# cosdata/cosdata

Hardware: AMD Instinct MI355X
Metric: QPS at recall@10≥0.95, 1024-dim dense cosine, 1/2/4/8 MI355X (higher is better)
Workload: dtype u8

## Files before the change

cosdata_amd/_lib.py:

```python
from __future__ import annotations

import ctypes as C
import os
import subprocess

_PKG = os.path.dirname(os.path.abspath(__file__))
SO_PATH = os.path.join(_PKG, "libcosdata_hip.so")
CSRC = os.path.join(_PKG, "csrc")

OK, ERR_STORAGE_MISMATCH, ERR_CALCULATION, ERR_INVALID, ERR_UNIMPLEMENTED, ERR_HIP, ERR_NOT_READY, ERR_NO_DEVICE = range(8)
STATUS_NAMES = {
    0: "OK", 1: "StorageMismatch", 2: "CalculationError", 3: "Invalid", 4: "Unimplemented", 5: "HipError",
    6: "NotReady", 7: "NoDevice",
}
ABI_VERSION = 1


class CosdataError(RuntimeError):

    def __init__(self, status: int, message: str):
        super().__init__(f"[{STATUS_NAMES.get(status, status)}] {message}")
        self.status = status


class CosParams(C.Structure):
    _fields_ = [
        ("struct_size", C.c_uint32), ("abi_version", C.c_uint32), ("dim", C.c_uint32), ("metric", C.c_uint32),
        ("storage", C.c_uint32), ("resolution", C.c_uint32), ("range_lo", C.c_float), ("range_hi", C.c_float),
        ("num_layers", C.c_uint32), ("neighbors_count", C.c_uint32), ("level0_neighbors_count", C.c_uint32),
        ("ef_construction", C.c_uint32), ("ef_search", C.c_uint32), ("shortlist_size", C.c_uint32),
        ("visited_mode", C.c_uint32), ("device", C.c_int32), ("id_base", C.c_uint32), ("reserved", C.c_uint32),
        ("seed", C.c_uint64),
    ]


class CosSearchStats(C.Structure):
    _fields_ = [
        ("evals", C.c_uint64), ("expansions", C.c_uint64), ("adj_bytes", C.c_uint64), ("rerank_rows", C.c_uint64),
        ("walk_ms", C.c_float), ("finalize_ms", C.c_float), ("prep_ms", C.c_float), ("reserved", C.c_uint32),
    ]


class CosWalkSplit(C.Structure):
    _fields_ = [
        ("struct_size", C.c_uint32), ("queries", C.c_uint32), ("table_level_min", C.c_uint32), ("table_cols", C.c_uint32),
        ("cut_after_level", C.c_uint32), ("reserved", C.c_uint32),
        ("table_ms", C.c_float), ("upper_ms", C.c_float), ("sort_ms", C.c_float), ("lower_ms", C.c_float),
        ("table_int8_ops", C.c_double), ("table_evals", C.c_uint64),
        ("upper_evals", C.c_uint64), ("upper_expansions", C.c_uint64), ("upper_adj_bytes", C.c_uint64),
        ("lower_evals", C.c_uint64), ("lower_expansions", C.c_uint64), ("lower_adj_bytes", C.c_uint64),
    ]


class CosTimingSummary(C.Structure):
    _fields_ = [("launches", C.c_uint32), ("prep_ms_sum", C.c_float), ("walk_ms_sum", C.c_float), ("finalize_ms_sum", C.c_float),
                ("walk_ms_min", C.c_float), ("walk_ms_max", C.c_float)]


class CosCoalescingStats(C.Structure):
    _fields_ = [("launches", C.c_uint64), ("queries", C.c_uint64), ("requests", C.c_uint64), ("closed_full", C.c_uint64),
                ("closed_quiet", C.c_uint64), ("closed_deadline", C.c_uint64), ("solo_calls", C.c_uint64)]


class CosSparseStats(C.Structure):
    _fields_ = [("kernel_ms", C.c_float), ("blocks", C.c_uint32), ("postings_visited", C.c_uint64), ("posting_bytes", C.c_uint64)]


class CosFlatStats(C.Structure):
    _fields_ = [("gemm_ms", C.c_float), ("gemm_launches", C.c_uint32), ("int8_ops", C.c_double), ("code_bytes", C.c_double)]


class CosBM25Stats(C.Structure):
    _fields_ = [("struct_size", C.c_uint32), ("documents_count", C.c_uint32), ("n_terms", C.c_uint32), ("largest_doc_id", C.c_uint32),
                ("dir_rows", C.c_uint32), ("dir_tiles", C.c_uint32), ("reserved", C.c_uint32),
                ("postings", C.c_uint64), ("tombstones", C.c_uint64), ("device_bytes", C.c_uint64)]


class CosSparseIndexStats(C.Structure):
    _fields_ = [("struct_size", C.c_uint32), ("n_vectors", C.c_uint32), ("n_dims", C.c_uint32), ("dir_rows", C.c_uint32),
                ("dir_tiles", C.c_uint32), ("packed", C.c_uint32), ("have_raw", C.c_uint32), ("reserved", C.c_uint32),
                ("postings", C.c_uint64), ("removed", C.c_uint64), ("raw_pairs", C.c_uint64), ("device_bytes", C.c_uint64)]


def build(force: bool = False, verbose: bool = False) -> str:
    srcs = [os.path.join(CSRC, f) for f in os.listdir(CSRC) if f.endswith((".hip", ".h"))]
    srcs.append(os.path.join(_PKG, "..", "include", "cosdata_hip.h"))
    stale = force or not os.path.exists(SO_PATH) or any(os.path.getmtime(s) > os.path.getmtime(SO_PATH) for s in srcs)
    if force:
        subprocess.check_call(["make", "-C", CSRC, "-s", "clean"])
    if stale:
        cmd = ["make", "-C", CSRC, "-j", str(max(2, min(16, 2 * (os.cpu_count() or 1))))]
        if not verbose:
            cmd.append("-s")
        subprocess.check_call(cmd)
    return SO_PATH


_lib = None

ABI_SYMBOLS = [
    "cos_index_create", "cos_index_destroy", "cos_last_error_string", "cos_device_count",
    "cos_index_upload_vectors", "cos_index_set_root", "cos_index_upload_graph_level", "cos_index_level_count",
    "cos_index_download_graph_level", "cos_index_download_codes", "cos_index_download_root", "cos_index_build", "cos_index_append", "cos_index_delete", "cos_index_restore_link_state", "cos_index_release_link_state", "cos_index_enable_metadata", "cos_index_upload_meta_nodes", "cos_index_upload_meta_graph_level", "cos_index_build_meta", "cos_index_meta_level_count", "cos_index_download_meta_graph_level", "cos_search_filtered_batch",
    "cos_ann_search_filtered_batch", "cos_index_load_reference_dir", "cos_reference_dir_level_counts", "cos_reference_dir_read_level",
    "cos_search_batch", "cos_search_batch_device", "cos_ann_search_batch", "cos_index_set_coalescing", "cos_index_coalescing_stats", "cos_index_set_ef_search",
    "cos_index_set_visited_mode", "cos_index_set_latency_mode", "cos_index_set_latency_waves", "cos_index_set_walk_order", "cos_index_walk_order_cuts", "cos_index_set_walk_table", "cos_index_walk_table_info", "cos_index_last_walk_split", "cos_index_enable_timing", "cos_index_last_stats", "cos_index_timing_summary", "cos_quantize_batch",
    "cos_code_bytes", "cos_sample_values_range", "cos_distance_batch", "cos_bruteforce_topk", "cos_flat_search_batch", "cos_bm25_create", "cos_bm25_destroy",
    "cos_bm25_insert", "cos_bm25_delete", "cos_bm25_stats", "cos_bm25_download",
    "cos_bm25_search_batch", "cos_bm25_search_batch_device", "cos_rrf_fuse_batch", "cos_hybrid_search_batch", "cos_text_process", "cos_text_count_tokens", "cos_bm25_term_frequency", "cos_xxhash32", "cos_stem_english", "cos_sparse_create", "cos_sparse_build_csr", "cos_sparse_create_from_vectors", "cos_sparse_destroy", "cos_sparse_search_batch", "cos_sparse_last_stats", "cos_sparse_layout",
    "cos_sparse_set_max_candidates", "cos_sparse_max_candidates",
    "cos_sparse_insert", "cos_sparse_delete", "cos_sparse_stats", "cos_sparse_download", "cos_merge_topk_device", "cos_merge_topk_packed_device", "cos_hbm_probe",
    "cos_shardset_unique_id", "cos_shardset_create", "cos_shardset_destroy", "cos_shardset_search_batch", "cos_shardset_exchange_device",
    "cos_tuning_set", "cos_tuning_clear", "cos_tuning_get",
]


def lib():
    global _lib
    if _lib is not None:
        return _lib
    if not os.path.exists(SO_PATH):
        raise CosdataError(ERR_NO_DEVICE, f"{SO_PATH} is missing: build it with `python -c 'import __graft_entry__ as g; g.build()'` "
                                          "(the HIP extension is mandatory; there is no CPU path)")
    try:
        import torch
    except ImportError:
        pass
    L = C.CDLL(SO_PATH)
    vp, i32, u32, f32 = C.c_void_p, C.c_int32, C.c_uint32, C.c_float
    sig = {
        "cos_index_create": [C.POINTER(CosParams), C.POINTER(vp)],
        "cos_index_destroy": [vp],
        "cos_device_count": [C.POINTER(i32)],
        "cos_index_upload_vectors": [vp, vp, u32, u32],
        "cos_index_set_root": [vp, vp],
        "cos_index_upload_graph_level": [vp, u32, u32, vp, vp],
        "cos_index_level_count": [vp, u32, C.POINTER(u32)],
        "cos_index_download_graph_level": [vp, u32, vp, vp],
        "cos_index_download_codes": [vp, vp, vp],
        "cos_index_download_root": [vp, vp],
        "cos_index_build": [vp, u32],
        "cos_index_append": [vp, vp, u32, u32, u32],
        "cos_index_release_link_state": [vp],
        "cos_index_restore_link_state": [vp],
        "cos_index_delete": [vp, vp, u32],
        "cos_index_load_reference_dir": [vp, C.c_char_p, u32, u32],
        "cos_index_enable_metadata": [vp, u32, u32],
        "cos_index_upload_meta_nodes": [vp, u32, vp, vp],
        "cos_index_upload_meta_graph_level": [vp, u32, u32, vp, vp],
        "cos_search_filtered_batch": [vp, vp, u32, vp, vp, u32, vp, vp, vp, vp],
        "cos_ann_search_filtered_batch": [vp, vp, u32, vp, vp, vp, vp, vp, vp],
        "cos_reference_dir_level_counts": [C.c_char_p, u32, u32, u32, vp],
        "cos_reference_dir_read_level": [C.c_char_p, u32, u32, u32, u32, vp, vp],
        "cos_search_batch": [vp, vp, u32, u32, vp, vp, vp, vp],
        "cos_search_batch_device": [vp, vp, u32, u32, vp, vp, vp, vp, vp],
        "cos_ann_search_batch": [vp, vp, u32, vp, vp, vp, vp],
        "cos_index_set_ef_search": [vp, u32],
        "cos_index_set_coalescing": [vp, u32, u32],
        "cos_index_coalescing_stats": [vp, C.POINTER(CosCoalescingStats)],
        "cos_index_set_visited_mode": [vp, u32],
        "cos_index_build_meta": [vp, u32, vp, vp, vp, u32],
        "cos_index_meta_level_count": [vp, u32, C.POINTER(u32)],
        "cos_index_download_meta_graph_level": [vp, u32, vp, vp],
        "cos_index_set_latency_mode": [vp, u32],
        "cos_index_set_latency_waves": [vp, u32],
        "cos_index_set_walk_order": [vp, u32],
        "cos_index_walk_order_cuts": [vp, C.POINTER(u32), u32, C.POINTER(u32)],
        "cos_index_enable_timing": [vp, i32],
        "cos_index_last_stats": [vp, vp, C.POINTER(CosSearchStats)],
        "cos_index_set_walk_table": [vp, u32, u32],
        "cos_index_walk_table_info": [vp, C.POINTER(u32), C.POINTER(u32)],
        "cos_index_last_walk_split": [vp, vp, C.POINTER(CosWalkSplit)],
        "cos_index_timing_summary": [vp, vp, C.POINTER(CosTimingSummary)],
        "cos_quantize_batch": [u32, u32, u32, f32, f32, vp, u32, vp, vp],
        "cos_sample_values_range": [vp, u32, u32, f32, C.POINTER(f32), C.POINTER(f32)],
        "cos_distance_batch": [u32, u32, u32, u32, vp, vp, u32, vp, vp, u32, vp, vp, u32, vp, vp],
        "cos_bruteforce_topk": [vp, vp, u32, u32, vp, vp],
        "cos_flat_search_batch": [vp, vp, u32, u32, vp, vp, vp, C.POINTER(CosFlatStats)],
        "cos_bm25_create": [i32, vp, vp, u32, vp, vp, u32, C.POINTER(vp)],
        "cos_bm25_destroy": [vp],
        "cos_bm25_insert": [vp, vp, vp, u32, vp, vp],
        "cos_bm25_delete": [vp, vp, vp, u32, vp],
        "cos_bm25_stats": [vp, C.POINTER(CosBM25Stats)],
        "cos_bm25_download": [vp, C.POINTER(u32), C.POINTER(C.c_uint64), vp, vp, vp, vp, vp],
        "cos_bm25_search_batch": [vp, vp, vp, u32, u32, vp, vp, vp],
        "cos_bm25_search_batch_device": [vp, vp, vp, u32, u32, vp, vp, vp, vp],
        "cos_rrf_fuse_batch": [vp, vp, u32, vp, vp, u32, u32, f32, u32, vp, vp, vp],
        "cos_hybrid_search_batch": [vp, vp, vp, vp, vp, u32, u32, f32, vp, vp, vp],
        "cos_sparse_create": [i32, u32, f32, vp, u32, vp, vp, u32, vp, vp, vp, C.POINTER(vp)],
        "cos_sparse_build_csr": [u32, f32, u32, vp, vp, vp, vp, vp, vp, C.POINTER(u32)],
        "cos_sparse_create_from_vectors": [i32, u32, f32, u32, vp, vp, vp, i32, C.POINTER(vp)],
        "cos_sparse_destroy": [vp],
        "cos_sparse_search_batch": [vp, vp, vp, vp, u32, u32, f32, u32, vp, vp, vp],
        "cos_sparse_last_stats": [vp, vp],
        "cos_sparse_layout": [vp, C.POINTER(u32)],
        "cos_sparse_set_max_candidates": [vp, u32],
        "cos_sparse_max_candidates": [vp, C.POINTER(u32)],
        "cos_sparse_insert": [vp, u32, vp, vp, vp, C.POINTER(u32)],
        "cos_sparse_delete": [vp, vp, vp, u32, vp, vp, C.POINTER(C.c_uint64)],
        "cos_sparse_stats": [vp, C.POINTER(CosSparseIndexStats)],
        "cos_sparse_download": [vp, C.POINTER(u32), C.POINTER(C.c_uint64), vp, vp, vp],
        "cos_merge_topk_device": [vp, vp, vp, u32, u32, u32, vp, vp, vp, i32, vp],
        "cos_merge_topk_packed_device": [vp, u32, u32, u32, vp, vp, vp, i32, vp],
        "cos_hbm_probe": [i32, u32, C.c_uint64, u32, u32, C.POINTER(C.c_double)],
        "cos_shardset_unique_id": [vp],
        "cos_shardset_create": [vp, u32, u32, u32, vp, C.POINTER(vp)],
        "cos_shardset_destroy": [vp],
        "cos_shardset_search_batch": [vp, vp, u32, u32, vp, vp, vp],
        "cos_shardset_exchange_device": [vp, vp, u32, u32, vp, vp, vp, vp, vp],
        "cos_tuning_set": [C.c_char_p, C.c_int64],
        "cos_tuning_clear": [C.c_char_p],
        "cos_tuning_get": [C.c_char_p, C.POINTER(C.c_int64), C.POINTER(i32)],
    }
    for name, args in sig.items():
        fn = getattr(L, name)
        fn.restype = i32
        fn.argtypes = args
    L.cos_last_error_string.restype = C.c_char_p
    L.cos_last_error_string.argtypes = []
    L.cos_stem_english.restype = C.c_size_t
    L.cos_stem_english.argtypes = [vp, C.c_char_p, C.c_size_t, C.c_char_p, C.c_size_t]
    L.cos_text_process.restype = i32
    L.cos_text_process.argtypes = [C.c_char_p, C.c_size_t, u32, f32, f32, f32, vp, vp, vp, vp, u32, C.POINTER(u32)]
    L.cos_text_count_tokens.restype = u32
    L.cos_text_count_tokens.argtypes = [C.c_char_p, C.c_size_t, u32]
    L.cos_bm25_term_frequency.restype = f32
    L.cos_bm25_term_frequency.argtypes = [u32, u32, f32, f32, f32]
    L.cos_xxhash32.restype = u32
    L.cos_xxhash32.argtypes = [C.c_char_p, C.c_size_t, u32]
    L.cos_code_bytes.restype = C.c_size_t
    L.cos_code_bytes.argtypes = [u32, u32, u32]
    _lib = L
    return L


def check(rc: int):
    if rc != OK:
        raise CosdataError(rc, lib().cos_last_error_string().decode("utf-8", "replace"))


def tuning_set(name: str, value: int):
    check(lib().cos_tuning_set(name.encode(), int(value)))


def tuning_clear(name: str | None = None):
    check(lib().cos_tuning_clear(name.encode() if name is not None else None))


def tuning_get(name: str):
    v, isset = C.c_int64(), C.c_int32()
    check(lib().cos_tuning_get(name.encode(), C.byref(v), C.byref(isset)))
    return int(v.value) if isset.value else None


# ... 25 lines not shown
```

cosdata_amd/csrc/engine.hip:

```cpp
#include <hip/hip_runtime.h>

#include <algorithm>
#include <cstdarg>
#include <cstdio>
#include <cstdlib>
#include <chrono>
#include <cmath>
#include <condition_variable>
#include <cstring>
#include <map>
#include <mutex>
#include <string>
#include <thread>
#include <vector>

#include "engine_internal.h"

using namespace cosdev;

static thread_local std::string g_err;
int32_t cos_fail(int32_t code, const char *fmt, ...) {
    char buf[512];
    va_list ap;
    va_start(ap, fmt);
    vsnprintf(buf, sizeof(buf), fmt, ap);
    va_end(ap);
    g_err = buf;
    return code;
}

extern "C" const char *cos_last_error_string(void) { return g_err.c_str(); }

extern "C" int32_t cos_device_count(int32_t *out) {
    if (!out) return cos_fail(COS_ERR_INVALID, "null argument");
    int n = 0;
    hipError_t e = hipGetDeviceCount(&n);
    if (e != hipSuccess) { *out = 0; return cos_fail(COS_ERR_NO_DEVICE, "hipGetDeviceCount: %s", hipGetErrorString(e)); }
    *out = n;
    return COS_OK;
}

static u32 pow2ceil(u32 v) { u32 p = 1; while (p < v) p <<= 1; return p; }

int32_t cos_set_device(const cos_index *ix) {
    HIP_TRY(hipSetDevice(ix->p.device));
    return COS_OK;
}

static bool graph_ready(const cos_index *ix) {
    if (!ix->have_vectors || !ix->have_root) return false;
    for (auto &l : ix->lv) if (l.n == 0) return false;
    return true;
}

IndexDev cos_make_index_dev(const cos_index *ix) {
    IndexDev d;
    memset(&d, 0, sizeof(d));
    d.codes = ix->d_codes;
    d.mags = ix->d_mags;
    d.raw = ix->d_raw;
    d.raw_mags = ix->d_raw_mags;
    d.row_stride = ix->row_stride;
    d.raw_stride = ix->p.dim;
    d.n = ix->n;
    d.dim = ix->p.dim;
    d.metric = ix->p.metric;
    d.storage = ix->p.storage;
    d.num_layers = ix->p.num_layers;
    d.shortlist = ix->p.shortlist_size;
    d.visited_mode = ix->p.visited_mode;
    d.nchunks = ix->nchunks;
    d.G = ix->G;
    d.id_base = ix->p.id_base;
    d.id_stride = ix->id_stride;
    d.mbits = ix->meta.d_mbits;
    d.mmags = ix->meta.d_mmags;
    d.mdim = ix->meta.mdim;
    for (u32 l = 0; l <= ix->p.num_layers; l++) {
        const LevelHost &h = ix->lv[l];
        d.lv[l].adj_vec = h.d_adj_vec;
        d.lv[l].adj_node = l == 0 ? h.d_adj_vec : h.d_adj_node;
        d.lv[l].node_vec = l == 0 ? nullptr : h.d_node_vec;
        d.lv[l].child = l == 0 ? nullptr : h.d_child;
        d.lv[l].n = h.n;
        d.lv[l].M = h.M;
        d.lv[l].root_idx = h.n ? h.n - 1 : 0;
        d.lv[l].adj_mag = (ix->adj_mag_valid && cosdev::tune_or(cosdev::TUNE_WALK_ADJ_MAG, 1) != 0) ? h.d_adj_mag : nullptr;
        d.lv[l].mag_stride = std::min(h.M, ix->p.shortlist_size);
    }
    return d;
}

extern "C" int32_t cos_index_create(const cos_params *p, cos_index **out) {
    if (!p || !out) return cos_fail(COS_ERR_INVALID, "null argument");
    *out = nullptr;
    if (p->struct_size != sizeof(cos_params) || p->abi_version != COS_ABI_VERSION)
        return cos_fail(COS_ERR_INVALID, "cos_params size/version mismatch (%u/%u, expected %zu/%u)", p->struct_size, p->abi_version,
                    sizeof(cos_params), COS_ABI_VERSION);
    if (p->dim == 0) return cos_fail(COS_ERR_INVALID, "dim == 0");
// ... 485 lines not shown
    const u64 log_cap = (u64)ef * M + 2;
    u32 max_nodes = 0;
    for (const LevelHost &l : ix->lv) max_nodes = std::max(max_nodes, l.n);
    const u32 words = (max_nodes + 31) / 32 + 1;
    if (log_cap > 0xFFFFFFFFull) return cos_fail(COS_ERR_INVALID, "ef too large");
    const size_t need_bits = (size_t)B * words, need_log = (size_t)B * log_cap;
    if (need_bits > vt.bits.cap || need_log > vt.log.cap) {
        HIP_TRY(hipStreamSynchronize(st));
        if (need_bits > vt.bits.cap) vt.zeroed = false;
        HIP_TRY(vt.bits.grow(need_bits));
        HIP_TRY(vt.log.grow(need_log));
    }
    if (!vt.zeroed) {
        HIP_TRY(hipMemsetAsync(vt.bits, 0, vt.bits.cap * 4, st));
        vt.zeroed = true;
    }
    wa.vis_bits = vt.bits;
    wa.vis_log = vt.log;
    wa.vis_words_per_query = words;
    wa.vis_log_cap = (u32)log_cap;
    return COS_OK;
}

static int32_t ensure_order_rank(cos_index *ix) {
    if (ix->order_rank_valid) return COS_OK;
    for (u32 l = 0; l < cosdev::MAX_LEVELS; l++) {
        ix->d_order_rank[l].reset();
        ix->order_rank_n[l] = 0;
    }
    ix->order_levels.clear();
    const u32 Ltop = ix->p.num_layers;
    auto usable = [&](u32 l) { return l >= 1 && l <= Ltop && ix->lv[l].n > 1 && ix->lv[l].n <= (1u << 20) && ix->lv[l].d_adj_node; };
    std::vector<u32> want;
    if (const long long mask = cosdev::tune(cosdev::TUNE_WALK_SPLIT_LEVELS); mask != cosdev::TUNE_UNSET) {
        for (u32 l = Ltop; l >= 1; l--)
            if ((mask >> l) & 1) want.push_back(l);
    } else {
        for (u32 l = 1; l <= Ltop; l++)
            if (usable(l) && (size_t)ix->lv[l].n * ix->row_stride <= ((size_t)64 << 20)) { want.push_back(l); break; }
    }
    u32 prev = Ltop + 1;
    for (u32 l : want) {
        if (!usable(l) || l >= prev) continue;
        ix->order_levels.push_back(l);
        prev = l;
    }
    if (!ix->order_levels.empty()) HIP_TRY(hipDeviceSynchronize());
    for (u32 kl : ix->order_levels) {
        const LevelHost &H = ix->lv[kl];
        const u32 n = H.n, M = H.M;
        std::vector<u32> adj((size_t)n * M), rank(n, 0u), stack;
        HIP_TRY(hipMemcpy(adj.data(), H.d_adj_node, adj.size() * 4, hipMemcpyDeviceToHost));
        std::vector<uint8_t> seen(n, 0);
        u32 next = 0;
        auto dfs_from = [&](u32 start) {
            stack.push_back(start);
            while (!stack.empty()) {
                const u32 v = stack.back();
                stack.pop_back();
                if (seen[v]) continue;
                seen[v] = 1;
                rank[v] = next++;
                const u32 *row = &adj[(size_t)v * M];
                for (u32 j = M; j-- > 0;) {
                    const u32 u = row[j];
                    if (u != cosdev::ROW_EMPTY && u < n && !seen[u]) stack.push_back(u);
                }
            }
        };
        dfs_from(n - 1);
        for (u32 v = 0; v < n; v++) if (!seen[v]) dfs_from(v);
        HIP_TRY(ix->d_order_rank[kl].alloc(n));
        HIP_TRY(hipMemcpy(ix->d_order_rank[kl], rank.data(), (size_t)n * 4, hipMemcpyHostToDevice));
        ix->order_rank_n[kl] = n;
    }
    ix->order_rank_valid = true;
    return COS_OK;
}

static void clear_current_table(cos_index *ix) {
    ix->d_tcodes = nullptr;
    ix->d_tmags = nullptr;
    ix->d_tcsums = nullptr;
    ix->table_cols = 0;
    ix->table_level_min = 0;
    ix->table_stride = 0;
}
static u32 walk_table_max_cols(const cos_index *ix) {
    const long long env = cosdev::tune_or(cosdev::TUNE_WALK_TABLE_COLS, -1);
    return env >= 0 ? (u32)std::min<long long>(env, 1ll << 20) : ix->walk_table_max_cols;
}
static u32 walk_table_min_B(const cos_index *ix) {
    const long long env = cosdev::tune_or(cosdev::TUNE_WALK_TABLE_MIN_B, -1);
    return env >= 0 ? (u32)std::min<long long>(env, 0xFFFFFFFFll) : ix->walk_table_min_B;
}
cosdev::WalkPlanIn cos_walk_plan_in(const cos_index *ix, u32 B, u32 ef) {
    cosdev::WalkPlanIn in{};
    in.eng = ix->eng;
    in.storage = ix->p.storage;
    in.nchunks = ix->nchunks;
    in.G = ix->G;
    in.num_layers = ix->p.num_layers;
    for (u32 l = 0; l <= ix->p.num_layers; l++) in.M[l] = ix->lv[l].M;
    in.shortlist = ix->p.shortlist_size;
    in.visited_mode = ix->p.visited_mode;
    in.mdim = ix->meta.mdim;
    in.B = B;
    in.ef = ef;
    in.chain = true;
    const long long lat = cosdev::tune_or(cosdev::TUNE_WALK_LAT, -1), lat4 = cosdev::tune_or(cosdev::TUNE_WALK_LAT4, -1);
    in.lat_max_B = lat >= 0 ? (u32)std::min(lat, 0xFFFFFFFFll) : ix->lat_max_B;
    in.lat4_max_B = lat4 >= 0 ? (u32)std::min(lat4, 0xFFFFFFFFll) : ix->lat4_max_B;
    in.small_table_tk = cosdev::tune_or(cosdev::TUNE_WALK_SMALL_TABLE_TK, 1) != 0;
    in.adj_mag_mode = (u32)cosdev::tune_or(cosdev::TUNE_WALK_ADJ_MAG, 1);
    in.table_min_B = walk_table_min_B(ix);
    in.order_min_B = ix->walk_order_min_B;
    in.chain_min_B = ix->chain_min_B;
    in.side_min_B = ix->walk_side_min_B;
    in.table_after_sort = cosdev::tune_or(cosdev::TUNE_WALK_TABLE_AFTER_SORT, 1);
    in.table_supported = cosdev::level_table_eng_supported(ix->eng, ix->row_stride);
    in.adj_mag_valid = ix->adj_mag_valid;
    return in;
}
static int32_t ensure_level_table(cos_index *ix) {
    const u32 max_cols = walk_table_max_cols(ix);
    const bool automatic = max_cols == COS_WALK_TABLE_AUTO;
    const u32 efs = ix->p.ef_search, Mup = ix->p.neighbors_count;
    const u64 c_rule = (u64)cosdev::tune_or(cosdev::TUNE_WALK_TABLE_RULE_C, 2u * efs <= 3u * Mup ? 10 : (efs <= 2u * Mup ? 8 : 6));
    const u64 per_level = automatic ? std::min<u64>(c_rule * ix->p.ef_search * ix->p.neighbors_count, 1u << 20) : (u64)(1u << 20);
    const u64 total_cap = automatic ? (u64)(1u << 20) : (u64)max_cols;
    const u64 key = automatic ? (0x8000000000000000ull | per_level) : (u64)max_cols;
    if (ix->level_table_valid && ix->table_built_for_key == key) return COS_OK;
    if (!ix->level_table_valid) {
        HIP_TRY(hipDeviceSynchronize());
        ix->table_sets.clear();
    }
    ix->level_table_valid = true;
    ix->table_built_for_key = key;
    clear_current_table(ix);
    for (const auto &t : ix->table_sets)
        if (t.key == key) {
            ix->table_level_min = t.level_min;
            ix->table_cols = t.cols;
            ix->table_stride = t.stride;
            memcpy(ix->table_col0, t.col0, sizeof(t.col0));
            ix->d_tcodes = t.tcodes;
            ix->d_tmags = t.tmags;
            ix->d_tcsums = t.tcsums;
            return COS_OK;
        }
    if (!cosdev::level_table_eng_supported(ix->eng, ix->row_stride) || max_cols == 0) return COS_OK;
    const u32 Ltop = ix->p.num_layers;
    u32 cols = 0, lmin = 0;
    for (u32 l = Ltop; l >= 1; l--) {
        if (!ix->lv[l].d_node_vec || ix->lv[l].n == 0 || ix->lv[l].n > per_level || (u64)cols + ix->lv[l].n > total_cap) break;
        cols += ix->lv[l].n;
        lmin = l;
    }
    if (lmin == 0) return COS_OK;
    HIP_TRY(hipDeviceSynchronize());
    cos_index::TableSet t;
    auto build = [&]() -> hipError_t {
        hipError_t e = t.tcodes.alloc((size_t)cols * ix->row_stride);
        if (e == hipSuccess) e = t.tmags.alloc(cols);
        if (e == hipSuccess) e = t.tcsums.alloc(cols);
        u32 c0 = 0;
        for (u32 l = Ltop; l >= lmin && e == hipSuccess; l--) {
            ix->table_col0[l] = c0;
            e = cosdev::launch_level_table_gather(ix->d_codes, ix->d_mags, ix->row_stride, ix->lv[l].d_node_vec, ix->lv[l].n, c0, t.tcodes, t.tmags, nullptr);
            c0 += ix->lv[l].n;
        }
        if (e == hipSuccess) e = cosdev::launch_code_sums(t.tcodes, ix->row_stride, cols, t.tcsums, nullptr);
        if (e == hipSuccess) e = hipDeviceSynchronize();
        return e;
    };
    if (const hipError_t e = build(); e != hipSuccess) {
        (void)hipDeviceSynchronize();
        if (e == hipErrorOutOfMemory) {
            (void)hipGetLastError();
            return COS_OK;
        }
        ix->level_table_valid = false;
        HIP_TRY(e);
    }
    ix->d_tcodes = t.tcodes;
    ix->d_tmags = t.tmags;
    ix->d_tcsums = t.tcsums;
    ix->table_cols = cols;
    ix->table_level_min = lmin;
    ix->table_stride = ((u64)cols + 31) / 32 * 32;
    t.key = key;
    t.level_min = lmin;
    t.cols = cols;
    t.stride = ix->table_stride;
    memcpy(t.col0, ix->table_col0, sizeof(t.col0));
    ix->table_sets.push_back(std::move(t));
    return COS_OK;
}

extern "C" int32_t cos_index_set_walk_table(cos_index *ix, uint32_t max_cols, uint32_t min_queries) {
    if (!ix) return cos_fail(COS_ERR_INVALID, "null argument");
    if (max_cols > (1u << 20) && max_cols != COS_WALK_TABLE_AUTO) return cos_fail(COS_ERR_INVALID, "max_cols must be <= 2^20 (or COS_WALK_TABLE_AUTO)");
    std::lock_guard<std::mutex> g(ix->mu);
    ix->walk_table_max_cols = max_cols;
    ix->walk_table_min_B = min_queries;
    return COS_OK;
}

extern "C" int32_t cos_index_walk_table_info(cos_index *ix, uint32_t *out_level_min, uint32_t *out_cols) {
    if (!ix || !out_level_min || !out_cols) return cos_fail(COS_ERR_INVALID, "null argument");
    *out_level_min = *out_cols = 0;
    if (!graph_ready(ix)) return cos_fail(COS_ERR_NOT_READY, "index needs vectors, root and every graph level");
    int32_t rc = cos_set_device(ix);
    if (rc) return rc;
    std::lock_guard<std::mutex> g(ix->mu);
    if (walk_table_min_B(ix) == 0) return COS_OK;
    if ((rc = ensure_level_table(ix))) return rc;
    *out_level_min = ix->table_level_min;
    *out_cols = ix->table_cols;
    return COS_OK;
}

static int32_t ensure_adj_mags(cos_index *ix) {
    if (ix->adj_mag_valid) return COS_OK;
    if (!graph_ready(ix) || ix->meta.mdim != 0u) return COS_OK;
    if (cosdev::walk_rows_over_64_slots(cos_walk_plan_in(ix, 0, 0))) return COS_OK;
    HIP_TRY(hipDeviceSynchronize());
    for (u32 l = 0; l <= ix->p.num_layers; l++) {
        ix->lv[l].d_adj_mag.reset();
    }
    for (u32 l = 0; l <= ix->p.num_layers; l++) {
        LevelHost &H = ix->lv[l];
        const u32 slots = std::min(H.M, ix->p.shortlist_size);
        const hipError_t e = H.d_adj_mag.alloc((size_t)H.n * slots);
        if (e == hipErrorOutOfMemory) {
            (void)hipGetLastError();
            for (u32 k = 0; k < l; k++) ix->lv[k].d_adj_mag.reset();
            return COS_OK;
        }
        HIP_TRY(e);
        HIP_TRY(cosdev::launch_fill_adj_mag(H.d_adj_vec, ix->d_mags, H.d_adj_mag, H.n, H.M, slots, ix->own_stream));
    }
    HIP_TRY(hipStreamSynchronize(ix->own_stream));
    ix->adj_mag_valid = true;
    return COS_OK;
}

int32_t cos_prepare_walk_plans(cos_index *ix) {
    std::lock_guard<std::mutex> g(ix->mu);
    if (int32_t rc = ensure_adj_mags(ix)) return rc;
    if (ix->walk_order_min_B)
        if (int32_t rc = ensure_order_rank(ix)) return rc;
    if (walk_table_min_B(ix))
        if (int32_t rc = ensure_level_table(ix)) return rc;
    return COS_OK;
}

extern "C" int32_t cos_index_walk_order_cuts(cos_index *ix, uint32_t *out_levels, uint32_t cap, uint32_t *out_n) {
    if (!ix || !out_n || (cap && !out_levels)) return cos_fail(COS_ERR_INVALID, "null argument");
    *out_n = 0;
    if (!graph_ready(ix)) return cos_fail(COS_ERR_NOT_READY, "index needs vectors, root and every graph level");
    int32_t rc = cos_set_device(ix);
    if (rc) return rc;
    std::lock_guard<std::mutex> g(ix->mu);
    if ((rc = ensure_order_rank(ix))) return rc;
    for (u32 l : ix->order_levels) {
        if (*out_n < cap) out_levels[*out_n] = l;
        (*out_n)++;
    }
    return COS_OK;
}

struct SearchLaunch {
    cosdev::WalkPlan plan;
    u32 ef = 0, visited_mode = 0;
    bool timed = false;
    u64 tab_stride = 0;
    u32 tab_col0[cosdev::MAX_LEVELS] = {};
    const uint8_t *tcodes = nullptr;
    const float *tmags = nullptr;
    const u32 *tcsums = nullptr;
    u32 n_keys = 0, key_level[cosdev::MAX_LEVELS], key_n[cosdev::MAX_LEVELS];
    const u32 *order_rank[cosdev::MAX_LEVELS];
};

static int32_t get_workspace(cos_index *ix, void *key, hipStream_t st, u32 B, u32 top_k, bool host_api, Workspace **out, SearchLaunch *L,
                             bool chain = true) {
    std::lock_guard<std::mutex> g(ix->mu);
    std::unique_ptr<Workspace> &slot = ix->ws[key];
    if (!slot) slot.reset(new Workspace());
    Workspace *w = slot.get();
    const u32 L1 = ix->p.num_layers + 1;
    if (B > w->capB) {
        u32 cap = std::max(B, 64u);
        HIP_TRY(hipStreamSynchronize(st));
        w->capB = 0;
        w->cap_topk = 0;
        HIP_TRY(w->q_codes.alloc((size_t)cap * ix->row_stride));
        HIP_TRY(w->q_mags.alloc(cap));
        HIP_TRY(w->q_raw_mags.alloc(cap));
        HIP_TRY(w->walk_ids.alloc((size_t)cap * L1 * KEEP_SEARCH));
        HIP_TRY(w->walk_sims.alloc((size_t)cap * L1 * KEEP_SEARCH));
        HIP_TRY(w->walk_counts.alloc((size_t)cap * L1));
        HIP_TRY(w->walk_status.alloc(cap));
        HIP_TRY(w->stats.alloc((size_t)cap * 4));
        HIP_TRY(w->stats2.alloc((size_t)cap * 4));
        HIP_TRY(w->qsums.alloc(cap));
        if (ix->eng == ENG_Q2) HIP_TRY(w->qdig.alloc((size_t)cap * (ix->row_stride / 16) * 64));
        HIP_TRY(w->fin_flags.alloc((size_t)cap + 1));
        HIP_TRY(w->rerank_rows.alloc(cap));
        HIP_TRY(w->d_queries.alloc((size_t)cap * ix->p.dim));
        HIP_TRY(w->d_out_counts.alloc(cap));
        HIP_TRY(w->d_out_status.alloc(cap));
        w->capB = cap;
    }
    L->ef = ix->p.ef_search;
    L->visited_mode = ix->p.visited_mode;
    L->timed = ix->timing;
    cosdev::WalkPlanIn in = cos_walk_plan_in(ix, B, L->ef);
    in.chain = chain;
    const cosdev::WalkPlan want = cosdev::walk_plan(in);
    cosdev::WalkHave have{};
    if (want.refill_adj_mag) {
        if (int32_t rc = ensure_adj_mags(ix)) return rc;
        in.adj_mag_valid = ix->adj_mag_valid;
    }
    if (want.prepare_order) {
        if (w->order.cap < w->capB) {
            HIP_TRY(hipStreamSynchronize(st));
            HIP_TRY(cosdev::walk_order_reserve(w->order, w->capB));
        }
        if (int32_t rc = ensure_order_rank(ix)) return rc;
        have.order_buffers = w->order.cap >= B;
        have.n_order_keys = (u32)ix->order_levels.size();
        have.order_level0 = have.n_order_keys ? ix->order_levels[0] : 0u;
    }
    if (want.prepare_table) {
        if (int32_t rc = ensure_level_table(ix)) return rc;
        const size_t need = (size_t)w->capB * ix->table_stride;
        if (need > w->tab.cap) {
            const size_t budget = (size_t)cosdev::tune_or(cosdev::TUNE_WALK_TABLE_MAX_BYTES, (long long)48 << 30);
            HIP_TRY(hipStreamSynchronize(st));
            ix->table_bytes_total -= w->tab.cap * 4;
            w->tab.reset();
            if (ix->table_bytes_total + need * 4 <= budget) {
                if (const hipError_t e = w->tab.alloc(need); e == hipSuccess)
                    ix->table_bytes_total += need * 4;
                else if (e == hipErrorOutOfMemory)
                    (void)hipGetLastError();
                else
                    HIP_TRY(e);
            }
        }
        have.table_level_min = ix->level_table_valid ? ix->table_level_min : 0u;
        have.table_cols = ix->table_cols;
        have.table_buffer = w->tab && (size_t)B * ix->table_stride <= w->tab.cap;
    }
    L->plan = cosdev::walk_plan(in, &have);
    if (L->plan.use_table) {
        L->tab_stride = ix->table_stride;
        memcpy(L->tab_col0, ix->table_col0, sizeof(L->tab_col0));
        L->tcodes = ix->d_tcodes;
        L->tmags = ix->d_tmags;
        L->tcsums = ix->d_tcsums;
    }
    if (L->plan.ordered)
        for (u32 l : ix->order_levels) {
            L->key_level[L->n_keys] = l;
            L->key_n[L->n_keys] = ix->order_rank_n[l];
            L->order_rank[L->n_keys++] = ix->d_order_rank[l];
        }
    if (host_api && (size_t)top_k * w->capB > (size_t)w->cap_topk * w->capB) {
        w->cap_topk = 0;
        HIP_TRY(w->d_out_ids.alloc((size_t)w->capB * top_k));
        HIP_TRY(w->d_out_scores.alloc((size_t)w->capB * top_k));
        w->cap_topk = top_k;
    }
    if (w->ev.empty()) {
        w->ev.assign((size_t)Workspace::EV_RING * Workspace::EV_PER, nullptr);
        for (auto &e : w->ev) HIP_TRY(hipEventCreate(&e));
    }
    if (!w->walk_done) HIP_TRY(hipEventCreateWithFlags(&w->walk_done, hipEventDisableTiming));
    if (!w->walk_fin) HIP_TRY(hipEventCreateWithFlags(&w->walk_fin, hipEventDisableTiming));
    if (!w->last_range) HIP_TRY(hipEventCreateWithFlags(&w->last_range, hipEventDisableTiming));
    *out = w;
    return COS_OK;
}

static int32_t run_search(cos_index *ix, Workspace *w, const SearchLaunch &L, const float *d_queries, u32 B, u32 top_k, u32 *d_out_ids,
                          float *d_out_scores, u32 *d_out_counts, int32_t *d_out_status, bool do_finalize, hipStream_t st,
                          hipStream_t st_fin = nullptr, hipEvent_t walk_ev = nullptr) {
    const cosdev::WalkPlan &plan = L.plan;
    const bool timed = L.timed, ordered = plan.ordered, chained = plan.chained;
    const u32 ef = L.ef, n_keys = L.n_keys;
    IndexDev dev = cos_make_index_dev(ix);
    dev.visited_mode = L.visited_mode;
    for (u32 l = 0; l <= dev.num_layers; l++)
        if (!((plan.use_adj_mag >> l) & 1u)) dev.lv[l].adj_mag = nullptr;
    WalkArgs wa;
    memset(&wa, 0, sizeof(wa));
    if (dev.visited_mode == COS_VISITED_EXACT) {
        int32_t rc = vis_tab_prepare(w->vis, ix, B, ef, st, wa);
        if (rc) return rc;
    }
    hipEvent_t *ev = &w->ev[(size_t)(w->ev_count % Workspace::EV_RING) * Workspace::EV_PER];
    if (timed) HIP_TRY(hipEventRecord(ev[0], st));
    HIP_TRY(launch_quantize_rows(ix->eng, d_queries, ix->p.dim, B, ix->p.dim, ix->p.range_lo, ix->p.range_hi, w->q_codes, ix->row_stride,
                                 w->q_mags, w->q_raw_mags, st));
    if (plan.use_table) {
        if (plan.table_waits_for_sort) {
            std::lock_guard<std::mutex> g(ix->chain_mu);
            if (ix->chain_last_range_ev && ix->chain_last_range_ev != w->last_range) HIP_TRY(hipStreamWaitEvent(st, ix->chain_last_range_ev, 0));
        }
        if (timed) HIP_TRY(hipEventRecord(ev[4], st));
        HIP_TRY(cosdev::launch_level_table(ix->eng, w->q_codes, w->q_mags, w->qsums, w->qdig, B, L.tcodes, L.tmags, L.tcsums, ix->row_stride, plan.table_cols,
                                           w->tab, L.tab_stride, ix->n_cus, st));
        if (timed) HIP_TRY(hipEventRecord(ev[5], st));
    }
    if (timed) HIP_TRY(hipEventRecord(ev[1], st));
    wa.qcodes = w->q_codes;
    wa.qmags = w->q_mags;
    wa.B = B;
    wa.ef = ef;
    wa.keep = KEEP_SEARCH;
    wa.out_ids = w->walk_ids;
    wa.out_sims = w->walk_sims;
    wa.out_counts = w->walk_counts;
    wa.out_status = w->walk_status;
    wa.out_stats = w->stats;
    wa.out_stats2 = w->stats2;
    HIP_TRY(hipMemsetAsync(w->stats2, 0, (size_t)B * 32, st));
    if (plan.use_table) {
        wa.tab = w->tab;
        wa.tab_mags = L.tmags;
        wa.tab_stride = L.tab_stride;
        wa.tab_level_min = plan.table_level_min;
        memcpy(wa.tab_col0, L.tab_col0, sizeof(L.tab_col0));
    }
    hipStream_t sw = st;
    if (plan.side_stream) {
        if (!w->walk_stream) {
            int lo = 0, hi = 0;
            HIP_TRY(hipDeviceGetStreamPriorityRange(&lo, &hi));
            HIP_TRY(hipStreamCreateWithPriority(&w->walk_stream, hipStreamNonBlocking, lo));
            HIP_TRY(hipEventCreateWithFlags(&w->prep_done, hipEventDisableTiming));
        }
        sw = w->walk_stream;
        HIP_TRY(hipEventRecord(w->prep_done, st));
        HIP_TRY(hipStreamWaitEvent(sw, w->prep_done, 0));
    }
    auto walk = [&](hipStream_t s) -> int32_t {
        if (!ordered) {
            if (chained) HIP_TRY(hipEventRecord(w->last_range, s));
            HIP_TRY(launch_walk(ix->eng, dev, wa, plan.kernel, s));
            return COS_OK;
        }
        wa.phase = 1;
        wa.entry0 = w->order.entry0;
        wa.order_key = w->order.order_key;
        wa.order_iota = w->order.iota;
        u32 first = dev.num_layers;
        for (u32 i = 0; i <= n_keys; i++) {
            const bool last = i == n_keys;
            wa.level_first = first;
            wa.level_last = last ? 0u : L.key_level[i];
            wa.key_n = last ? 0u : L.key_n[i];
            wa.order_rank = last ? nullptr : L.order_rank[i];
            if (last && chained) HIP_TRY(hipEventRecord(w->last_range, s));
            HIP_TRY(launch_walk(ix->eng, dev, wa, plan.kernel, s));
            if (last) break;
            if (timed && i == 0) HIP_TRY(hipEventRecord(ev[6], s));
            HIP_TRY(cosdev::launch_walk_order(w->order, B, L.key_n[i], ix->num_xcd, s));
            if (timed && i == 0) HIP_TRY(hipEventRecord(ev[7], s));
            wa.q_order = w->order.q_order;
            first = L.key_level[i] - 1;
        }
        return COS_OK;
    };
    if (chained) {
        std::lock_guard<std::mutex> g(ix->chain_mu);
        if (ix->chain_ev && ix->chain_ev != w->walk_done) HIP_TRY(hipStreamWaitEvent(sw, ix->chain_ev, 0));
        if (timed) HIP_TRY(hipEventRecord(ev[1], sw));
        if (int32_t rc = walk(sw)) return rc;
        HIP_TRY(hipEventRecord(w->walk_done, sw));
        ix->chain_ev = w->walk_done;
        ix->chain_last_range_ev = w->last_range;
    } else {
        if (timed && sw != st) HIP_TRY(hipEventRecord(ev[1], sw));
        if (int32_t rc = walk(sw)) return rc;
    }
    if (timed) HIP_TRY(hipEventRecord(ev[2], sw));
    hipStream_t sf = st_fin ? st_fin : st;
    if (sf != sw) {
        hipEvent_t we = walk_ev ? walk_ev : w->walk_fin;
        HIP_TRY(hipEventRecord(we, sw));
        HIP_TRY(hipStreamWaitEvent(sf, we, 0));
    }
    if (do_finalize) {
        HIP_TRY(launch_finalize(dev, d_queries, ix->p.dim, w->q_raw_mags, w->walk_ids, w->walk_sims, w->walk_counts, w->walk_status, B, top_k,
                                d_out_ids, d_out_scores, d_out_counts, d_out_status, w->rerank_rows, sf, ordered ? w->order.q_order : nullptr, w->fin_flags));
    }
    if (timed) { HIP_TRY(hipEventRecord(ev[3], sf)); w->ev_count++; }
    w->lastB = B;
    w->timed = timed;
    w->last_plan = plan;
    { std::lock_guard<std::mutex> g(ix->mu); ix->last_ws = w; }
    return COS_OK;
}

static int32_t check_search_args(cos_index *ix, const void *q, u32 B, u32 top_k) {
    if (!ix || !q) return cos_fail(COS_ERR_INVALID, "null argument");
    if (!graph_ready(ix)) return cos_fail(COS_ERR_NOT_READY, "index needs vectors, root and every graph level before search");
    if (top_k == 0 || top_k > 1024) return cos_fail(COS_ERR_INVALID, "top_k must be in [1, 1024]");
    if (B == 0) return cos_fail(COS_ERR_INVALID, "empty batch");
    return cos_set_device(ix);
}

extern "C" int32_t cos_search_batch_device(cos_index *ix, const float *d_queries, uint32_t B, uint32_t top_k, uint32_t *d_out_ids,
                                           float *d_out_scores, uint32_t *d_out_counts, int32_t *d_out_status, void *stream) {
    int32_t rc = check_search_args(ix, d_queries, B, top_k);
    if (rc) return rc;
    if (!d_out_ids || !d_out_scores || !d_out_counts || !d_out_status) return cos_fail(COS_ERR_INVALID, "null output");
    Workspace *w;
    SearchLaunch L;
    rc = get_workspace(ix, stream, (hipStream_t)stream, B, top_k, false, &w, &L);
    if (rc) return rc;
    return run_search(ix, w, L, d_queries, B, top_k, d_out_ids, d_out_scores, d_out_counts, d_out_status, true, (hipStream_t)stream);
}

struct PipeLease {
    cos_index *ix;
    HostPipe *hp = nullptr;
    explicit PipeLease(cos_index *ix_) : ix(ix_) {}
    PipeLease(const PipeLease &) = delete;
    PipeLease &operator=(const PipeLease &) = delete;
    int32_t acquire() {
        std::unique_lock<std::mutex> lk(ix->pipe_mu);
        for (;;) {
            if (!ix->pipes_free.empty()) { hp = ix->pipes_free.back(); ix->pipes_free.pop_back(); break; }
            if (ix->pipes_all.size() < COS_MAX_HOST_PIPES) {
                std::unique_ptr<HostPipe> n(new HostPipe());
                hipError_t e = hipStreamCreateWithFlags(&n->s[0], hipStreamNonBlocking);
                if (e != hipSuccess) return cos_fail(COS_ERR_HIP, "hipStreamCreateWithFlags: %s", hipGetErrorString(e));
                hp = n.get();
                ix->pipes_all.push_back(std::move(n));
                break;
            }
            ix->pipe_cv.wait(lk);
        }
        ix->host_calls_active.fetch_add(1);
        return COS_OK;
    }
    ~PipeLease() {
        if (!hp) return;
        ix->host_calls_active.fetch_sub(1);
        { std::lock_guard<std::mutex> g(ix->pipe_mu); ix->pipes_free.push_back(hp); }
        ix->pipe_cv.notify_one();
    }
};

static int32_t report_status(const int32_t *status, u32 B) {
    for (u32 b = 0; b < B; b++)
        if (status[b] != COS_OK) return cos_fail(status[b], "query %u failed with status %d (zero-norm vector -> DistanceError::CalculationError)", b, status[b]);
    return COS_OK;
}

static int32_t search_host_simple(cos_index *ix, HostPipe *hp, const float *queries, uint32_t B, uint32_t top_k, uint32_t *out_ids, float *out_scores,
                                  uint32_t *out_counts, int32_t *out_status) {
    hipStream_t st = hp->s[0];
    Workspace *w;
    SearchLaunch L;
    int32_t rc = get_workspace(ix, (void *)st, st, B, top_k, true, &w, &L);
    if (rc) return rc;
    HIP_TRY(hipMemcpyAsync(w->d_queries, queries, (size_t)B * ix->p.dim * 4, hipMemcpyHostToDevice, st));
    rc = run_search(ix, w, L, w->d_queries, B, top_k, w->d_out_ids, w->d_out_scores, w->d_out_counts, w->d_out_status, true, st);
    if (rc) { (void)hipDeviceSynchronize(); return rc; }
    std::vector<int32_t> status(B);
    hipError_t e = hipMemcpyAsync(out_ids, w->d_out_ids, (size_t)B * top_k * 4, hipMemcpyDeviceToHost, st);
    if (e == hipSuccess) e = hipMemcpyAsync(out_scores, w->d_out_scores, (size_t)B * top_k * 4, hipMemcpyDeviceToHost, st);
    if (e == hipSuccess) e = hipMemcpyAsync(out_counts, w->d_out_counts, (size_t)B * 4, hipMemcpyDeviceToHost, st);
    if (e == hipSuccess) e = hipMemcpyAsync(status.data(), w->d_out_status, (size_t)B * 4, hipMemcpyDeviceToHost, st);
    const hipError_t es = hipStreamSynchronize(st);
    HIP_TRY(e);
    HIP_TRY(es);
    if (out_status) memcpy(out_status, status.data(), (size_t)B * 4);
    return report_status(status.data(), B);
// ... 284 lines not shown
    int32_t rc = check_search_args(ix, queries, B, 1);
    if (rc) return rc;
    if (!out_ids || !out_sims || !out_counts) return cos_fail(COS_ERR_INVALID, "null output");
    PipeLease lease(ix);
    rc = lease.acquire();
    if (rc) return rc;
    hipStream_t st = lease.hp->s[0];
    Workspace *w;
    SearchLaunch L;
    rc = get_workspace(ix, (void *)st, st, B, 1, true, &w, &L);
    if (rc) return rc;
    const u32 L1 = ix->p.num_layers + 1;
    HIP_TRY(hipMemcpyAsync(w->d_queries, queries, (size_t)B * ix->p.dim * 4, hipMemcpyHostToDevice, st));
    rc = run_search(ix, w, L, w->d_queries, B, 1, nullptr, nullptr, nullptr, nullptr, false, st);
    if (rc) return rc;
    std::vector<int32_t> status(B);
    HIP_TRY(hipMemcpyAsync(out_ids, w->walk_ids, (size_t)B * L1 * KEEP_SEARCH * 4, hipMemcpyDeviceToHost, st));
    HIP_TRY(hipMemcpyAsync(out_sims, w->walk_sims, (size_t)B * L1 * KEEP_SEARCH * 4, hipMemcpyDeviceToHost, st));
    HIP_TRY(hipMemcpyAsync(out_counts, w->walk_counts, (size_t)B * L1 * 4, hipMemcpyDeviceToHost, st));
    HIP_TRY(hipMemcpyAsync(status.data(), w->walk_status, (size_t)B * 4, hipMemcpyDeviceToHost, st));
    HIP_TRY(hipStreamSynchronize(st));
    if (out_status) memcpy(out_status, status.data(), (size_t)B * 4);
    for (u32 b = 0; b < B; b++)
        if (status[b] != COS_OK) return cos_fail(status[b], "query %u failed with status %d", b, status[b]);
    return COS_OK;
}

static Workspace *find_workspace(cos_index *ix, void *stream, bool null_is_last) {
    std::lock_guard<std::mutex> g(ix->mu);
    if (!stream && null_is_last) return ix->last_ws;
    auto it = ix->ws.find(stream);
    return it != ix->ws.end() ? it->second.get() : nullptr;
}
static int32_t sum_launch_stats(const u64 *d_stats, u32 B, u64 sum[4]) {
    std::vector<u64> st((size_t)B * 4);
    HIP_TRY(hipMemcpy(st.data(), d_stats, st.size() * 8, hipMemcpyDeviceToHost));
    sum[0] = sum[1] = sum[2] = sum[3] = 0;
    for (u32 b = 0; b < B; b++)
        for (int k = 0; k < 4; k++) sum[k] += st[(size_t)b * 4 + k];
    return COS_OK;
}

extern "C" int32_t cos_index_last_stats(cos_index *ix, void *stream, cos_search_stats *out) {
    if (!ix || !out) return cos_fail(COS_ERR_INVALID, "null argument");
    memset(out, 0, sizeof(*out));
    int32_t rc = cos_set_device(ix);
    if (rc) return rc;
    Workspace *w = find_workspace(ix, stream, true);
    if (!w || w->lastB == 0) return cos_fail(COS_ERR_NOT_READY, "no batch has run on this stream");
    if (w->timed && w->ev_count) {
        hipEvent_t *ev = &w->ev[(size_t)((w->ev_count - 1) % Workspace::EV_RING) * Workspace::EV_PER];
        HIP_TRY(hipEventSynchronize(ev[3]));
        HIP_TRY(hipEventElapsedTime(&out->prep_ms, ev[0], ev[1]));
        HIP_TRY(hipEventElapsedTime(&out->walk_ms, ev[1], ev[2]));
        HIP_TRY(hipEventElapsedTime(&out->finalize_ms, ev[2], ev[3]));
    } else {
        HIP_TRY(hipDeviceSynchronize());
    }
    u64 st[4];
    if ((rc = sum_launch_stats(w->stats, w->lastB, st))) return rc;
    out->evals = st[0];
    out->expansions = st[1];
    out->adj_bytes = st[2];
    out->reserved = (uint32_t)st[3];
    std::vector<u64> rr(w->lastB);
    HIP_TRY(hipMemcpy(rr.data(), w->rerank_rows, rr.size() * 8, hipMemcpyDeviceToHost));
    for (u32 b = 0; b < w->lastB; b++) out->rerank_rows += rr[b];
    return COS_OK;
}

extern "C" int32_t cos_index_last_walk_split(cos_index *ix, void *stream, cos_walk_split *out) {
    if (!ix || !out) return cos_fail(COS_ERR_INVALID, "null argument");
    if (out->struct_size != sizeof(cos_walk_split)) return cos_fail(COS_ERR_INVALID, "cos_walk_split.struct_size mismatch");
    memset(out, 0, sizeof(*out));
    out->struct_size = sizeof(cos_walk_split);
    int32_t rc = cos_set_device(ix);
    if (rc) return rc;
    Workspace *w = find_workspace(ix, stream, true);
    if (!w || w->lastB == 0) return cos_fail(COS_ERR_NOT_READY, "no batch has run on this stream");
    const cosdev::WalkPlan &plan = w->last_plan;
    out->queries = w->lastB;
    out->table_level_min = plan.table_level_min;
    out->table_cols = plan.table_cols;
    out->cut_after_level = plan.cut_after_level;
    if (w->timed && w->ev_count) {
        hipEvent_t *ev = &w->ev[(size_t)((w->ev_count - 1) % Workspace::EV_RING) * Workspace::EV_PER];
        HIP_TRY(hipEventSynchronize(ev[3]));
        if (plan.use_table) HIP_TRY(hipEventElapsedTime(&out->table_ms, ev[4], ev[5]));
        if (plan.ordered) {
            HIP_TRY(hipEventElapsedTime(&out->upper_ms, ev[1], ev[6]));
            HIP_TRY(hipEventElapsedTime(&out->sort_ms, ev[6], ev[7]));
            HIP_TRY(hipEventElapsedTime(&out->lower_ms, ev[7], ev[2]));
        } else
            HIP_TRY(hipEventElapsedTime(&out->lower_ms, ev[1], ev[2]));
    } else {
        HIP_TRY(hipDeviceSynchronize());
    }
    const u32 kdims = (u32)((ix->row_stride + 63) / 64 * 64);
    out->table_int8_ops = 2.0 * (double)w->lastB * (double)out->table_cols * (double)kdims;
    u64 st[4], s2[4];
    if ((rc = sum_launch_stats(w->stats, w->lastB, st)) || (rc = sum_launch_stats(w->stats2, w->lastB, s2))) return rc;
    out->lower_evals = s2[0];
    out->lower_expansions = s2[1];
    out->lower_adj_bytes = s2[2];
    out->table_evals = s2[3];
    out->upper_evals = st[0] - s2[0];
    out->upper_expansions = st[1] - s2[1];
    out->upper_adj_bytes = st[2] - s2[2];
    return COS_OK;
}

extern "C" int32_t cos_index_timing_summary(cos_index *ix, void *stream, cos_timing_summary *out) {
    if (!ix || !out) return cos_fail(COS_ERR_INVALID, "null argument");
    memset(out, 0, sizeof(*out));
    int32_t rc = cos_set_device(ix);
    if (rc) return rc;
    Workspace *w = find_workspace(ix, stream, false);
    if (!w || w->ev_count == 0) return cos_fail(COS_ERR_NOT_READY, "no timed batch has run on this stream");
    const u32 n = std::min(w->ev_count, Workspace::EV_RING);
    out->launches = n;
    out->walk_ms_min = 1e30f;
    for (u32 i = 0; i < n; i++) {
        hipEvent_t *ev = &w->ev[(size_t)((w->ev_count - 1 - i) % Workspace::EV_RING) * Workspace::EV_PER];
        float a = 0, b = 0, c = 0;
        HIP_TRY(hipEventSynchronize(ev[3]));
        HIP_TRY(hipEventElapsedTime(&a, ev[0], ev[1]));
        HIP_TRY(hipEventElapsedTime(&b, ev[1], ev[2]));
        HIP_TRY(hipEventElapsedTime(&c, ev[2], ev[3]));
        out->prep_ms_sum += a;
        out->walk_ms_sum += b;
        out->finalize_ms_sum += c;
        out->walk_ms_min = std::min(out->walk_ms_min, b);
        out->walk_ms_max = std::max(out->walk_ms_max, b);
    }
    return COS_OK;
}

static constexpr u32 PSEUDO_LO = 0xFFFFFEFEu, PSEUDO_HI = 0xFFFFFFFDu;

extern "C" int32_t cos_index_enable_metadata(cos_index *ix, uint32_t mdim, uint32_t max_replicas_per_node) {
    if (!ix || mdim == 0 || mdim > 64 || max_replicas_per_node == 0) return cos_fail(COS_ERR_INVALID, "metadata dimensions must be in [1, 64] and max_replicas_per_node >= 1");
    if (!ix->have_vectors) return cos_fail(COS_ERR_NOT_READY, "upload vectors before enabling the metadata component");
    if (ix->p.ef_construction > cosdev::WALK_FAST_MAX_EF || std::min(ix->p.neighbors_count, ix->p.shortlist_size) > 64u ||
        std::min(ix->p.level0_neighbors_count, ix->p.shortlist_size) > 64u ||
        (ix->nchunks != 0u && (ix->nchunks + ix->G - 1u) / ix->G > (ix->eng == ENG_U8 ? 2u : 1u)))
        return cos_fail(COS_ERR_UNIMPLEMENTED, "metadata collections: ef_construction <= %u, at most 64 scanned neighbour slots per node, u8 rows of at most 2048 / SubByte rows of at most 64 x 16 bytes", cosdev::WALK_FAST_MAX_EF);
    if ((u64)ix->n * max_replicas_per_node >= PSEUDO_LO) return cos_fail(COS_ERR_INVALID, "replica ids would run into the reserved id range");
    if (ix->p.id_base % max_replicas_per_node != 0)
        return cos_fail(COS_ERR_INVALID, "id_base %u of a metadata collection's shard must be a multiple of max_replicas_per_node %u (first embedding x replicas)", ix->p.id_base, max_replicas_per_node);
    if ((u64)ix->p.id_base + (u64)ix->n * max_replicas_per_node >= PSEUDO_LO) return cos_fail(COS_ERR_INVALID, "replica ids would run into the reserved id range");
    for (auto &l : ix->lv)
        if (l.n) return cos_fail(COS_ERR_INVALID, "enable the metadata component before uploading / building the base graph: it changes the id of every vector (row x max_replicas)");
    int32_t rc = cos_set_device(ix);
    if (rc) return rc;
    ix->id_stride = max_replicas_per_node;
    ix->meta.mdim = mdim;
    ix->meta.lv.resize(ix->p.num_layers + 1);
    for (u32 l = 0; l <= ix->p.num_layers; l++) ix->meta.lv[l].M = l == 0 ? ix->p.level0_neighbors_count : ix->p.neighbors_count;
    DevBuf z;
    HIP_TRY(z.alloc(((size_t)ix->p.dim + 1) * 4));
    HIP_TRY(hipMemsetAsync(z.p, 0, ((size_t)ix->p.dim + 1) * 4, ix->own_stream));
    HIP_TRY(launch_quantize_rows(ix->eng, z.as<float>(), ix->p.dim, 1, ix->p.dim, ix->p.range_lo, ix->p.range_hi,
                                 ix->d_codes + ((size_t)ix->n + 1) * ix->row_stride, ix->row_stride, ix->d_mags + ix->n + 1, z.as<float>() + ix->p.dim, ix->own_stream));
    HIP_TRY(hipStreamSynchronize(ix->own_stream));
    return COS_OK;
}

extern "C" int32_t cos_index_upload_meta_nodes(cos_index *ix, uint32_t n_nodes, const uint32_t *node_ids, const int32_t *mbits) {
    if (!ix || !node_ids || !mbits || n_nodes == 0) return cos_fail(COS_ERR_INVALID, "null/empty node table");
    if (!ix->meta.mdim || !ix->have_vectors) return cos_fail(COS_ERR_NOT_READY, "cos_index_enable_metadata first");
    int32_t rc = cos_set_device(ix);
    if (rc) return rc;
    const u32 md = ix->meta.mdim;
    for (u32 i = 0; i < n_nodes; i++) {
        if (i && node_ids[i] <= node_ids[i - 1]) return cos_fail(COS_ERR_INVALID, "node ids must be strictly ascending");
        const bool pseudo = node_ids[i] >= PSEUDO_LO && node_ids[i] <= PSEUDO_HI;
        if (!pseudo && node_ids[i] / ix->id_stride >= ix->n) return cos_fail(COS_ERR_INVALID, "replica id %u has no resident vector", node_ids[i]);
    }
    std::vector<float> mags(n_nodes);
    for (u32 i = 0; i < n_nodes; i++) {
        float acc = -0.0f;
        for (u32 j = 0; j < md; j++) { const float x = (float)mbits[(size_t)i * md + j]; acc = acc + x * x; }
// ... 228 lines not shown
```

cosdata_amd/csrc/engine_internal.h:

```cpp
#pragma once
#include <hip/hip_runtime.h>

#include <atomic>
#include <condition_variable>
#include <map>
#include <memory>
#include <mutex>
#include <string>
#include <thread>
#include <vector>

#include "../../include/cosdata_hip.h"
#include "engine_types.h"
#include "tuning.h"
#include "link_types.h"
#include "dev_mem.h"
#include "walk_plan.h"

namespace cosdev {
hipError_t launch_fill_i32(int32_t *p, u64 n, int32_t v, hipStream_t st);
hipError_t launch_edge_pairs(const u32 *adj_vec, const u32 *node_vec, u32 node0, u32 cn, u32 M, u32 *px, u32 *py, hipStream_t st);
hipError_t launch_edge_keys(const u32 *adj_vec, const float *sims, const int32_t *st_in, u32 node0, u32 cn, u32 M, u32 metric, int32_t *key, int32_t *fail, hipStream_t st);
hipError_t launch_low_cache(const u32 *adj_vec, const int32_t *key, u32 n, u32 M, int32_t kmin, int32_t kmax, uint8_t *low_idx, int32_t *low_key, hipStream_t st);
hipError_t launch_unlink(const LinkArgs &a, const u32 *dn, u32 *status, hipStream_t st);
hipError_t launch_index_pair_distances(int eng, const uint8_t *codes, const float *mags, u64 row_stride, u32 nchunks, u32 dim, u32 metric, const u32 *d_pair_x,
                                       const u32 *d_pair_y, u32 n_pairs, float *d_out, int32_t *d_status, hipStream_t st);
hipError_t launch_grow_rows(const u32 *src, u32 *dst, u32 old_n, u32 new_n, u32 M, u32 remap_from, u32 remap_to, u32 fill, hipStream_t st);
hipError_t launch_grow_bytes(const uint8_t *src, uint8_t *dst, u32 old_n, u32 new_n, hipStream_t st);
hipError_t launch_fill_adj_mag(const u32 *adj_vec, const float *mags, float *adj_mag, u32 n, u32 M, u32 slots, hipStream_t st);
hipError_t launch_link_round(const LinkArgs &a, u32 maxM, const u32 *pend, const u32 *pcount, u32 *next, u32 *next_count, u32 *evq, u32 *evq_count,
                             u32 count_ub, u32 round, hipStream_t st);
hipError_t launch_quantize_rows(int eng, const float *x, u64 x_stride, u32 n, u32 dim, float lo, float hi, uint8_t *codes,
                                u64 row_stride, float *mags, float *raw_mags, hipStream_t st);
hipError_t launch_walk(int eng, const IndexDev &ix, const WalkArgs &wa, WalkKernel kernel, hipStream_t st);
static_assert(WALK_PLAN_MAX_LEVELS == MAX_LEVELS && WALK_PLAN_ENG_U8 == ENG_U8 && WALK_PLAN_ENG_Q2 == ENG_Q2 && WALK_PLAN_FAST_MAX_EF == WALK_FAST_MAX_EF &&
              COS_STORAGE_U8 == 0u && COS_VISITED_REF == 0u, "walk_plan.h restates these");
hipError_t launch_walk_meta(int eng, const IndexDev &ix, const WalkArgs &wa, hipStream_t st);
hipError_t launch_walk_meta_index(int eng, const IndexDev &ix, const WalkArgs &wa, hipStream_t st);
hipError_t launch_finalize(const IndexDev &ix, const float *queries, u64 q_stride, const float *q_raw_mags, const u32 *walk_ids,
                           const float *walk_sims, const u32 *walk_counts, const int32_t *walk_status, u32 B, u32 top_k,
                           u32 *out_ids, float *out_scores, u32 *out_counts, int32_t *out_status, u64 *out_rerank_rows,
                           hipStream_t st, const u32 *q_order = nullptr, u32 *slow_list = nullptr);
struct WalkOrder {
    u32 cap = 0;
    DevArr<u32> entry0;
    DevArr<u32> order_key;
    DevArr<u32> keys_sorted;
    DevArr<u32> iota, vals_sorted, q_order;
    DevBuf tmp;
};
hipError_t walk_order_reserve(WalkOrder &o, u32 B);
hipError_t launch_walk_order(WalkOrder &o, u32 B, u32 key_max, u32 num_xcd, hipStream_t st);
hipError_t launch_level_table_gather(const uint8_t *codes, const float *mags, u64 row_stride, const u32 *node_vec, u32 n, u32 col0,
                                     uint8_t *tcodes, float *tmags, hipStream_t st);
hipError_t launch_code_sums(const uint8_t *codes, u64 row_stride, u32 n, u32 *sums, hipStream_t st);
hipError_t launch_level_table(int eng, const uint8_t *qcodes, const float *qmags, u32 *qsums, uint8_t *qdig, u32 B, const uint8_t *tcodes, const float *tmags,
                              const u32 *tcsums, u64 row_stride, u32 ncols, float *tab, u64 tab_stride, u32 n_cus, hipStream_t st);
bool level_table_eng_supported(int eng, u64 row_stride);
int32_t quantize_ref_layout(uint32_t storage, uint32_t res, uint32_t dim, const float *x, uint32_t n, void *codes, float *mags);
int32_t distance_ref_layout(uint32_t metric, uint32_t storage, uint32_t res, uint32_t dim, const void *x_codes, const float *x_mags, uint32_t nx,
                            const void *y_codes, const float *y_mags, uint32_t ny, const uint32_t *pair_x, const uint32_t *pair_y, uint32_t n_pairs,
                            float *out, int32_t *status);
}

using cosdev::u32;
using cosdev::u64;

int32_t cos_fail(int32_t code, const char *fmt, ...);
#define HIP_TRY(expr)                                                                                  \
    do {                                                                                               \
        hipError_t _e = (expr);                                                                        \
        if (_e != hipSuccess) return cos_fail(COS_ERR_HIP, "%s: %s (%s:%d)", #expr, hipGetErrorString(_e), __FILE__, __LINE__); \
    } while (0)

struct LevelHost {
    std::vector<u32> node_ids;
    std::vector<u32> nbr_ids;
    DevArr<u32> d_adj_vec, d_adj_node, d_node_vec, d_child;
    DevArr<u32> d_node_id, d_node_meta;
    DevArr<float> d_adj_mag;
    u32 n = 0, M = 0;
    u32 root_idx = 0;
    bool host_valid = false;
    void release() {
        d_adj_vec.reset(); d_adj_node.reset(); d_node_vec.reset(); d_child.reset();
        d_node_id.reset(); d_node_meta.reset(); d_adj_mag.reset();
        n = 0;
        node_ids.clear();
        nbr_ids.clear();
        host_valid = false;
    }
};

struct LinkState {
    DevBuf key[cosdev::MAX_LEVELS], low_idx[cosdev::MAX_LEVELS], low_key[cosdev::MAX_LEVELS], owner[cosdev::MAX_LEVELS];
    uint64_t rng = 0;
    u32 n_built = 0;
    bool valid = false;
    void release() {
        for (int l = 0; l < cosdev::MAX_LEVELS; l++) { key[l].reset(); low_idx[l].reset(); low_key[l].reset(); owner[l].reset(); }
        valid = false;
    }
};

struct VisTab {
    DevArr<u32> bits, log;
    bool zeroed = false;
};
int32_t vis_tab_prepare(VisTab &vt, const cos_index *ix, u32 B, u32 ef, hipStream_t st, cosdev::WalkArgs &wa);

struct Workspace {
    u32 capB = 0, cap_topk = 0;
    DevArr<uint8_t> q_codes;
    DevArr<float> q_mags, q_raw_mags;
    DevArr<u32> walk_ids, walk_counts;
    DevArr<float> walk_sims;
    DevArr<int32_t> walk_status;
    DevArr<u64> stats;
    DevArr<u64> stats2;
    DevArr<float> tab;
    DevArr<u32> qsums;
    DevArr<uint8_t> qdig;
    DevArr<u32> fin_flags;
    DevArr<u64> rerank_rows;
    VisTab vis;
    cosdev::WalkOrder order;
    DevArr<float> d_queries;
    DevArr<u32> d_out_ids, d_out_counts;
    DevArr<float> d_out_scores;
    DevArr<int32_t> d_out_status;
    DevArr<u32> f_buf;
    static constexpr u32 EV_RING = 128;
    static constexpr u32 EV_PER = 8;
    std::vector<hipEvent_t> ev;
    u32 ev_count = 0;
    hipEvent_t walk_done = nullptr;
    hipEvent_t last_range = nullptr;
    hipStream_t walk_stream = nullptr;
    hipEvent_t prep_done = nullptr, walk_fin = nullptr;
    u32 lastB = 0;
    bool timed = false;
    cosdev::WalkPlan last_plan{};
    Workspace() = default;
    Workspace(const Workspace &) = delete;
    ~Workspace() {
        for (hipEvent_t e : {walk_done, walk_fin, last_range, prep_done}) if (e) (void)hipEventDestroy(e);
        for (hipEvent_t e : ev) if (e) (void)hipEventDestroy(e);
        if (walk_stream) (void)hipStreamDestroy(walk_stream);
    }
};

struct MetaGraph {
    u32 mdim = 0;
    std::vector<u32> node_ids;
    DevArr<int32_t> d_mbits;
    DevArr<float> d_mmags;
    std::vector<LevelHost> lv;
};

struct HostPipe {
    static constexpr u32 MAX_CHUNKS = 4;
    hipStream_t s[2] = {nullptr, nullptr}, sc = nullptr, sf = nullptr;
    hipEvent_t ev_in[MAX_CHUNKS] = {}, ev_walk[MAX_CHUNKS] = {};
    char wkey[MAX_CHUNKS] = {};
    DevArr<float> d_q;
    DevArr<u32> d_ids, d_counts;
    DevArr<float> d_scores;
    DevArr<int32_t> d_status;
    HostPipe() = default;
    HostPipe(const HostPipe &) = delete;
    ~HostPipe() {
        for (hipEvent_t e : ev_in) if (e) (void)hipEventDestroy(e);
        for (hipEvent_t e : ev_walk) if (e) (void)hipEventDestroy(e);
        for (hipStream_t st : {s[0], s[1], sc, sf}) if (st) (void)hipStreamDestroy(st);
    }
};
static constexpr u32 COS_MAX_HOST_PIPES = 32;

struct cos_index {
    cos_params p;
    int eng = -1;
    u32 n = 0;
    bool have_vectors = false, have_root = false;
    const float *d_raw = nullptr;
    DevArr<float> raw_own;
    DevArr<float> d_raw_mags;
    DevArr<uint8_t> d_codes;
    DevArr<float> d_mags;
    u64 row_stride = 0;
    u32 nchunks = 0, G = 1;
    std::vector<float> root_raw;
    std::vector<LevelHost> lv;
    u32 id_stride = 1;
    MetaGraph meta;
    hipStream_t own_stream = nullptr;
    std::mutex mu;
    std::map<void *, std::unique_ptr<Workspace>> ws;
    std::mutex pipe_mu;
    std::condition_variable pipe_cv;
    std::vector<std::unique_ptr<HostPipe>> pipes_all;
    std::vector<HostPipe *> pipes_free;
    std::atomic<int> host_calls_active{0};
    Workspace *last_ws = nullptr;
    std::mutex co_mu;
    std::condition_variable co_cv;
    std::vector<struct CoSlot *> co_slots;
    struct CoSlot *co_open = nullptr;
    u32 co_max_queries = 0, co_window_us = 0;
    u32 co_inflight = 0;
    cos_coalescing_stats co_stats{};
    bool timing = false;
    std::mutex chain_mu;
    hipEvent_t chain_ev = nullptr;
    hipEvent_t chain_last_range_ev = nullptr;
    u32 chain_min_B = 16384;
    u32 walk_order_min_B = COS_WALK_ORDER_DEFAULT_MIN_B;
    u32 n_cus = 256;
    u32 num_xcd = 8;
    DevArr<u32> d_order_rank[cosdev::MAX_LEVELS];
    u32 order_rank_n[cosdev::MAX_LEVELS] = {};
    std::vector<u32> order_levels;
    bool order_rank_valid = false;
    u32 walk_table_max_cols = COS_WALK_TABLE_AUTO, walk_table_min_B = COS_WALK_TABLE_DEFAULT_MIN_B;
    size_t table_bytes_total = 0;
    bool adj_mag_valid = false;
    LinkState link;
    bool level_table_valid = false;
    u32 table_level_min = 0, table_cols = 0;
    u64 table_built_for_key = 0;
    u64 table_stride = 0;
    u32 table_col0[cosdev::MAX_LEVELS] = {};
    const uint8_t *d_tcodes = nullptr;
    const float *d_tmags = nullptr;
    const u32 *d_tcsums = nullptr;
    struct TableSet { u64 key; u32 level_min, cols; u64 stride; u32 col0[cosdev::MAX_LEVELS]; DevArr<uint8_t> tcodes; DevArr<float> tmags; DevArr<u32> tcsums; };
    std::vector<TableSet> table_sets;
    u32 walk_side_min_B = 4096;
    u32 lat_max_B = COS_LATENCY_MODE_DEFAULT_MAX_B;
    u32 lat4_max_B = COS_LATENCY_WAVES_DEFAULT_MAX_B;
    struct FlatWs *flat_ws = nullptr;
};


struct FlatWs;
void cos_flat_ws_release(cos_index *ix);
void cos_coalesce_release(cos_index *ix);
cosdev::IndexDev cos_make_index_dev(const cos_index *ix);
cosdev::IndexDev cos_make_meta_dev(const cos_index *ix);
int32_t cos_set_device(const cos_index *ix);
cosdev::WalkPlanIn cos_walk_plan_in(const cos_index *ix, u32 B, u32 ef);
int32_t cos_prepare_walk_plans(cos_index *ix);
void cos_meta_free_levels(cos_index *ix);
```

cosdata_amd/csrc/engine_types.h:

```cpp
#pragma once
#include <stdint.h>
#include "device_common.h"

namespace cosdev {

struct LevelDev {
    const u32 *adj_vec;
    const u32 *adj_node;
    const u32 *node_vec;
    const u32 *child;
    u32 n;
    u32 M;
    u32 root_idx;
    const float *adj_mag;
    u32 mag_stride;
    const u32 *node_id;
    const u32 *node_meta;
};

struct IndexDev {
    const uint8_t *codes;
    const float *mags;
    const float *raw;
    const float *raw_mags;
    u64 row_stride;
    u64 raw_stride;
    u32 n;
    u32 dim;
    u32 metric;
    u32 storage;
    u32 num_layers;
    u32 shortlist;
    u32 visited_mode;
    u32 nchunks;
    u32 G;
    u32 id_base;
    u32 id_stride;
    const int32_t *mbits;
    const float *mmags;
    u32 mdim;
    LevelDev lv[MAX_LEVELS];
};

struct WalkArgs {
    const uint8_t *qcodes;
    const float *qmags;
    const u32 *q_rows;
    const u32 *self_ids;
    u32 *vis_bits;
    u32 *vis_log;
    u32 vis_words_per_query;
    u32 vis_log_cap;
    u32 B;
    u32 ef;
    u32 keep;
    u32 *out_ids;
    float *out_sims;
    u32 *out_nodes;
    u32 *out_counts;
    int32_t *out_status;
    const int32_t *f_dims;
    const float *f_mags;
    const u32 *f_off;
    u64 *out_stats;
    u64 *out_stats2;
    const float *tab;
    const float *tab_mags;
    u64 tab_stride;
    u32 tab_level_min;
    u32 tab_col0[MAX_LEVELS];
    u32 no_self_seed;
    u32 smem_mmax;
    u32 smem_win_bytes;
    u32 merge_min;
    u32 phase;
    u32 level_first, level_last;
    u32 key_n;
    const u32 *order_rank;
    const u32 *q_order;
    u32 *entry0;
    u32 *order_key;
    u32 *order_iota;
};

constexpr u32 WALK_FAST_MAX_EF = 1024u;
constexpr u32 WALK_GENERAL_MAX_EF = 16384u;

}
```

cosdata_amd/csrc/kernels_flat.hip:

```cpp
#include <hip/hip_runtime.h>

#include <algorithm>
#include <cstdlib>
#include <cstring>
#include <type_traits>
#include <vector>

#include "dot_engines.h"
#include "engine_internal.h"
#include "flat_scan.h"
#include "topk_select.h"

using namespace cosdev;

namespace {

typedef float f32x16 __attribute__((ext_vector_type(16)));

constexpr int BM = 128, BN = 128, BK = 32, LDT = BK + 4;
constexpr int SEL = 64;
constexpr size_t GEMM_SMEM = 2ull * (BM + BN) * LDT * sizeof(float);

template <bool VEC, bool FUSED>
__global__ __launch_bounds__(256) void flat_gemm_f32(const float *__restrict__ Q, u64 q_stride, const float *__restrict__ qmags, u32 B,
// ... 751 lines not shown
                if (use_fused) FLAT_LAUNCH_PF(ENG_U8, true); else FLAT_LAUNCH_PF(ENG_U8, false);
            } else {
                if (use_fused) FLAT_LAUNCH_PF(ENG_Q2, true); else FLAT_LAUNCH_PF(ENG_Q2, false);
            }
#undef FLAT_LAUNCH_PF
#undef FLAT_LAUNCH
#undef FLAT_ARGS
            e = hipGetLastError();
            if (e == hipSuccess) e = hipEventRecord(ev1, st);
            if (e == hipSuccess) {
                if (use_fused && R == 1) {
                    hipLaunchKernelGGL(flat_select_append, dim3(B), dim3(64), 0, st, (const u64 *)d_app, d_appcnt, APP_CAP, B, d_pool, d_thr, d_zero + 1);
                    e = hipGetLastError();
                } else if (use_fused)
                    e = launch_flat_append_wide(R, d_app, d_appcnt, APP_CAP, B, d_pool, d_thr, d_zero + 1, st);
                else if (R == 1)
                    e = launch_select(d_scores, s_stride, B, n0, nc, d_part, S, d_pool, st, d_thr);
                else
                    e = launch_flat_select_wide(R, d_scores, s_stride, B, n0, nc, d_part, S, d_pool, d_thr, st);
            }
            launches++;
            streamed += (double)nc * (double)ix->row_stride * (double)((B + CM - 1) / CM);
            n0 += nc;
            seen += nc;
        }
        const size_t nk = (size_t)B * top_k, out_words = 2 * nk + B + 2;
        if (e == hipSuccess) e = W->out.grow(out_words);
        if (e == hipSuccess) e = W->h_out.grow(out_words);
        if (e != hipSuccess) break;
        if (R == 1) {
            hipLaunchKernelGGL(flat_rerank_top5k, dim3(B), dim3(64), (((size_t)dim * 4 + 15) & ~(size_t)15), st, d_q, (u64)dim, d_qrm, B, ix->d_raw, (u64)dim,
                               ix->d_raw_mags, dim, d_pool, 5 * top_k, top_k, ix->p.id_base, d_oi, d_os, d_oc);
        } else {
            e = launch_flat_rerank_wide(R, false, d_q, (u64)dim, d_qrm, B, ix->d_raw, (u64)dim, ix->d_raw_mags, dim, d_pool, 5 * top_k, top_k, ix->p.id_base,
                                        d_oi, d_os, d_oc, st);
            if (e != hipSuccess) break;
        }
        hipLaunchKernelGGL(flat_pack_out_kernel, dim3((u32)((std::max<size_t>(nk, B) + 255) / 256)), dim3(256), 0, st, d_oi, d_os, d_oc, d_zero, B, top_k, W->out.p);
        e = hipGetLastError();
        if (e == hipSuccess) e = hipMemcpyAsync(W->h_out, W->out.p, out_words * 4, hipMemcpyDeviceToHost, st);
        if (e == hipSuccess) e = hipStreamSynchronize(st);
        if (e != hipSuccess) break;
        const u32 *ho = W->h_out;
        zero = ho[2 * nk + B] != 0;
        const u32 hover = ho[2 * nk + B + 1];
        if (zero) break;
        if (fused && hover != 0) continue;
        memcpy(out_ids, ho, nk * 4);
        memcpy(out_scores, ho + nk, nk * 4);
        memcpy(out_counts, ho + 2 * nk, (size_t)B * 4);
        break;
    }
    if (e == hipSuccess && !zero) {
        for (size_t i = 0; i + 1 < n_ev && e == hipSuccess; i += 2) {
            float ms = 0.f;
            e = hipEventElapsedTime(&ms, W->evs[i], W->evs[i + 1]);
            gemm_ms += ms;
        }
    }
    if (stats) {
        stats->gemm_ms = gemm_ms;
        stats->gemm_launches = launches;
        stats->int8_ops = 2.0 * (double)B * (double)n * (double)kdims;
        stats->code_bytes = streamed;
    }
    HIP_TRY(e);
    if (zero) return cos_fail(COS_ERR_CALCULATION, "zero-norm query or stored vector: DistanceError::CalculationError (cosine.rs:228-232)");
    return COS_OK;
}

namespace {
__global__ __launch_bounds__(256) void level_table_gather_kernel(const uint8_t *__restrict__ codes, const float *__restrict__ mags, u64 row_stride,
                                                                 const u32 *__restrict__ node_vec, u32 n, u32 col0, uint8_t *__restrict__ tcodes,
                                                                 float *__restrict__ tmags) {
    const int lane = threadIdx.x & 63;
    const u32 node = blockIdx.x * 4 + (threadIdx.x >> 6);
    if (node >= n) return;
    const u32 row = node_vec[node];
    const uint4 *src = (const uint4 *)(codes + (u64)row * row_stride);
    uint4 *dst = (uint4 *)(tcodes + (u64)(col0 + node) * row_stride);
    for (u32 c = lane; c < (u32)(row_stride / 16); c += 64) dst[c] = src[c];
    if (lane == 0) tmags[col0 + node] = mags[row];
}
}

namespace cosdev {

hipError_t launch_level_table_gather(const uint8_t *codes, const float *mags, u64 row_stride, const u32 *node_vec, u32 n, u32 col0,
                                     uint8_t *tcodes, float *tmags, hipStream_t st) {
    if (n == 0) return hipSuccess;
    hipLaunchKernelGGL(level_table_gather_kernel, dim3((n + 3) / 4), dim3(256), 0, st, codes, mags, row_stride, node_vec, n, col0, tcodes, tmags);
    return hipGetLastError();
}

hipError_t launch_code_sums(const uint8_t *codes, u64 row_stride, u32 n, u32 *sums, hipStream_t st) {
    if (n == 0) return hipSuccess;
    hipLaunchKernelGGL(code_sums_kernel, dim3((n + 3) / 4), dim3(256), 0, st, codes, row_stride, n, sums);
    return hipGetLastError();
}

bool level_table_eng_supported(int eng, u64 row_stride) {
    return eng == ENG_U8 || (eng == ENG_Q2 && level_table_areg_supported(ENG_Q2, row_stride));
}

hipError_t launch_level_table(int eng, const uint8_t *qcodes, const float *qmags, u32 *qsums , uint8_t *qdig ,
                              u32 B, const uint8_t *tcodes, const float *tmags, const u32 *tcsums, u64 row_stride, u32 ncols, float *tab, u64 tab_stride,
                              u32 n_cus, hipStream_t st) {
    if (B == 0 || ncols == 0) return hipSuccess;
    const bool q2 = eng == ENG_Q2;
    const u32 kdims = q2 ? (u32)(row_stride / 16) * 64 : (u32)((row_stride + 63) / 64 * 64);
    hipError_t e = hipSuccess;
    if (!q2) e = launch_code_sums(qcodes, row_stride, B, qsums, st);
    if (e != hipSuccess) return e;
    if (level_table_areg_supported(eng, row_stride) && tune_or(TUNE_WALK_TABLE_GEMM, 1) != 0) {
        if (q2) {
            e = launch_flat_scan_expand_queries(qcodes, row_stride, B, kdims, qdig, st, false);
            if (e != hipSuccess) return e;
        }
        return launch_level_table_areg(eng, n_cus ? n_cus : 256u, st, q2 ? qdig : qcodes, (const u32 *)qsums, B, tcodes, tcsums, row_stride, ncols, tab, tab_stride);
    }
    const u32 metric = 1u;
    dim3 grid((ncols + CN - 1) / CN, (B + CM - 1) / CM);
    FusedOut fo{nullptr, nullptr, nullptr, 0u, nullptr};
    if (q2)
        hipLaunchKernelGGL((flat_codes_gemm_i8<ENG_Q2, false, 2>), grid, dim3(512), 0, st, qcodes, qmags, (const u32 *)qsums, B, tcodes, tmags, tcsums, row_stride, 0u,
                           ncols, kdims, metric, tab, tab_stride, fo);
    else
        hipLaunchKernelGGL((flat_codes_gemm_i8<ENG_U8, false, 2>), grid, dim3(512), 0, st, qcodes, qmags, (const u32 *)qsums, B, tcodes, tmags, tcsums, row_stride, 0u,
                           ncols, kdims, metric, tab, tab_stride, fo);
    return hipGetLastError();
}

}
```

cosdata_amd/csrc/kernels_walk.hip:

```cpp
#include <hip/hip_runtime.h>

#include <algorithm>
#include <cstdlib>

#include "engine_types.h"
#include "tuning.h"
#include "walk_common.h"
#include "walk_plan.h"

using namespace cosdev;

namespace {

template <int ENG>
__global__ __launch_bounds__(256) void quantize_rows_kernel(const float *__restrict__ x, u64 x_stride, u32 n, u32 dim, float lo,
                                                            float hi, uint8_t *__restrict__ codes, u64 row_stride,
                                                            float *__restrict__ mags, float *__restrict__ raw_mags) {
    const int lane = threadIdx.x & 63;
    const u32 row = blockIdx.x * (blockDim.x >> 6) + (threadIdx.x >> 6);
    if (row >= n) return;
    const float *xr = x + (u64)row * x_stride;
    uint8_t *cr = codes + (u64)row * row_stride;
    float rn = 0.0f;
    const bool need_seq = (raw_mags != nullptr) || (ENG != ENG_U8);
    if (need_seq) rn = seq_norm_wave(xr, dim, lane);
    if (raw_mags && lane == 0) raw_mags[row] = rn;
    if constexpr (ENG == ENG_U8) {
        u32 ss = 0;
        for (u32 i = lane; i < (u32)row_stride; i += 64) {
            uint8_t q = 0;
            if (i < dim) {
                float c = rust_min(rust_max(xr[i], lo), hi);
                float v = __fmul_rn(__fdiv_rn(__fsub_rn(c, lo), __fsub_rn(hi, lo)), 255.0f);
                q = rust_f32_as_u8(v);
            }
            cr[i] = q;
            ss += (u32)q * (u32)q;
        }
#pragma unroll
        for (int m = 32; m > 0; m >>= 1) ss += (u32)__shfl_xor((int)ss, m, 64);
        if (lane == 0) mags[row] = sqrtf((float)ss);
    } else if constexpr (ENG == ENG_Q2) {
        const u32 nch = (u32)(row_stride / 16);
        for (u32 c = 0; c < nch; c++) {
            u32 i = c * 64 + lane;
            u32 lvl = 0;
            if (i < dim) lvl = rust_f32_as_usize_low2(floorf(__fdiv_rn(__fadd_rn(xr[i], 1.0f), 0.5f)));
            u64 p0 = __ballot((lvl >> 1) & 1u);
            u64 p1 = __ballot(lvl & 1u);
            if (lane == 0) {
                *(u64 *)(cr + (u64)c * 16) = p0;
                *(u64 *)(cr + (u64)c * 16 + 8) = p1;
            }
        }
        if (lane == 0) mags[row] = rn;
    } else if constexpr (ENG == ENG_Q1) {
        const u32 nch = (u32)(row_stride / 16);
        for (u32 c = 0; c < 2 * nch; c++) {
            const u32 i = c * 64 + lane;
            u32 lvl = 0;
            if (i < dim) lvl = rust_f32_as_usize_low(floorf(__fdiv_rn(__fadd_rn(xr[i], 1.0f), 1.0f)), 1u);
            const u64 p0 = __ballot(lvl & 1u);
            if (lane == 0) *(u64 *)(cr + (u64)c * 8) = p0;
        }
        if (lane == 0) mags[row] = rn;
    } else if constexpr (ENG == ENG_Q3) {
        const u32 nch = (u32)(row_stride / 16);
        for (u32 c = 0; c < nch; c += 2) {
            const u32 i = c * 32 + lane;
            u32 lvl = 0;
            if (i < dim) lvl = rust_f32_as_usize_low(floorf(__fdiv_rn(__fadd_rn(xr[i], 1.0f), 0.25f)), 7u);
            const u64 p0 = __ballot((lvl >> 2) & 1u), p1 = __ballot((lvl >> 1) & 1u), p2 = __ballot(lvl & 1u);
            if (lane == 0) {
                *(uint4 *)(cr + (u64)c * 16) = make_uint4((u32)p0, (u32)p1, (u32)p2, 0u);
                if (c + 1 < nch) *(uint4 *)(cr + (u64)(c + 1) * 16) = make_uint4((u32)(p0 >> 32), (u32)(p1 >> 32), (u32)(p2 >> 32), 0u);
            }
        }
        if (lane == 0) mags[row] = rn;
    } else if constexpr (ENG == ENG_F16) {
        __half *ch = (__half *)cr;
        for (u32 i = lane; i < (u32)(row_stride / 2); i += 64) ch[i] = i < dim ? __float2half_rn(xr[i]) : __float2half_rn(0.0f);
        if (lane == 0) mags[row] = rn;
    } else {
        float *cf = (float *)cr;
        for (u32 i = lane; i < (u32)(row_stride / 4); i += 64) cf[i] = i < dim ? xr[i] : 0.0f;
        if (lane == 0) mags[row] = rn;
    }
}

#include "walk_kernel.inc"

struct FinalizeArgs {
    const float *queries;
    u64 q_stride;
    const float *q_raw_mags;
    const u32 *walk_ids;
    const float *walk_sims;
    const u32 *walk_counts;
    const int32_t *walk_status;
    u32 B, top_k;
    u32 *out_ids;
    float *out_scores;
    u32 *out_counts;
    int32_t *out_status;
    u64 *out_rerank_rows;
    const u32 *q_order;
    u32 *slow_list;
    u32 *slow_count;
};

template <int NWV>
__device__ __forceinline__ void finalize_sync() {
    if constexpr (NWV > 1) __syncthreads();
    else { __builtin_amdgcn_s_waitcnt(0); __builtin_amdgcn_wave_barrier(); }
}
template <int NWV>
__device__ __forceinline__ void rerank_wide(const IndexDev &ix, const float *qf, const u32 *cand, u32 ncand, float mag_query, u64 *keys, int lane, int wave) {
    for (u32 base = (u32)wave * 8u; base < ncand; base += 8u * (u32)NWV) {
        const u32 my = base + (u32)(lane >> 3);
        const u32 id = my < ncand ? cand[my] : 0u;
        const u32 rrow = id / ix.id_stride;
        const float dp = f32_oct_dot(ix.raw + (u64)rrow * ix.raw_stride, qf, ix.dim, lane & 7);
        const float cs = x86_div(dp, __fmul_rn(mag_query, ix.raw_mags[rrow]));
        if ((lane & 7) == 0 && my < ncand) keys[my] = pack_key(simkey(cs), id);
// ... 248 lines not shown
            const u64 key = pack_key(metric_key(metric, smv[u]), id);
            const u64 keep = ballot64((u32)lane < cc[u] && !drop && key >= T);
            const u32 nk = (u32)__popcll(keep);
            if (n + nk > (u32)FAST_CAP) { overflow = true; break; }
            if (__builtin_amdgcn_inverse_ballot_w64(keep)) surv[n + (u32)__popcll(keep & ((1ull << lane) - 1ull))] = key;
            n += nk;
        }
        if (overflow) break;
    }
    if (overflow) {
        if (lane == 0) fa.slow_list[atomicAdd(fa.slow_count, 1u)] = qi;
        if constexpr (NWV > 1) {
            if (lane == 0) cand[64] = 0xFFFFFFFFu;
            __syncthreads();
            __syncthreads();
        }
        return;
    }
    __builtin_amdgcn_s_waitcnt(0);
    __builtin_amdgcn_wave_barrier();
    u64 k[2];
#pragma unroll
    for (int r = 0; r < 2; r++) {
        const u32 e = (u32)lane * 2u + (u32)r;
        k[r] = e < n ? surv[e] : 0ull;
    }
    bitonic_sort_desc<2>(k, lane);
    const u64 prev_last = shfl_up1_u64(k[1]);
    const bool keep0 = k[0] != 0ull && (lane == 0 || k[0] != prev_last), keep1 = k[1] != 0ull && k[1] != k[0];
    const u32 mine = (keep0 ? 1u : 0u) + (keep1 ? 1u : 0u);
    u32 incl = mine;
#pragma unroll
    for (int d = 1; d < 64; d <<= 1) {
        const u32 t = (u32)__shfl_up((int)incl, d, 64);
        if (lane >= d) incl += t;
    }
    u32 pos = incl - mine;
    const u32 total = readlane_u32(incl, 63);
    const u32 ncand = total < want ? total : want;
    if (keep0) { if (pos < ncand) cand[pos] = (u32)k[0]; pos++; }
    if (keep1) { if (pos < ncand) cand[pos] = (u32)k[1]; }
    const u32 nout = ncand < fa.top_k ? ncand : fa.top_k;
    u64 res[1] = {0ull};
    if constexpr (NWV > 1) {
        if (lane == 0) cand[64] = ncand;
        __syncthreads();
        rerank_wide<NWV>(ix, qf, cand, ncand, mag_query, surv, lane, 0);
        __syncthreads();
        res[0] = (u32)lane < ncand ? surv[lane] : 0ull;
    } else {
    __builtin_amdgcn_s_waitcnt(0);
    __builtin_amdgcn_wave_barrier();

    const int pair = lane >> 1;
    for (u32 base = 0; base < ncand; base += 32) {
        const u32 my = base + (u32)pair;
        const u32 id = my < ncand ? cand[my] : 0u;
        const u32 rrow = id / ix.id_stride;
        const float dp = f32_pair_dot(ix.raw + (u64)rrow * ix.raw_stride, qf, ix.dim, lane & 1);
        const float cs = x86_div(dp, __fmul_rn(mag_query, ix.raw_mags[rrow]));
        const u64 key = my < ncand ? pack_key(simkey(cs), id) : 0ull;
        const int from = (2 * (lane - (int)base)) & 63;
        const u32 klo = (u32)__shfl((int)(u32)key, from, 64), khi = (u32)__shfl((int)(u32)(key >> 32), from, 64);
        if ((u32)lane >= base && (u32)lane < base + 32) res[0] = ((u64)khi << 32) | klo;
    }
    }
    bitonic_sort_desc<1>(res, lane);
    if ((u32)lane < nout) {
        fa.out_ids[(u64)qi * fa.top_k + lane] = (u32)res[0] + ix.id_base;
        fa.out_scores[(u64)qi * fa.top_k + lane] = simkey_inv((u32)(res[0] >> 32));
    }
    if (lane == 0) {
        fa.out_counts[qi] = nout;
        fa.out_status[qi] = COS_OK;
        if (fa.out_rerank_rows) fa.out_rerank_rows[qi] = ncand;
    }
}

}

namespace cosdev {

hipError_t launch_quantize_rows(int eng, const float *x, u64 x_stride, u32 n, u32 dim, float lo, float hi, uint8_t *codes,
                                u64 row_stride, float *mags, float *raw_mags, hipStream_t st) {
    if (n == 0) return hipSuccess;
    dim3 block(256), grid((n + 3) / 4);
    switch (eng) {
    case ENG_U8: hipLaunchKernelGGL(quantize_rows_kernel<ENG_U8>, grid, block, 0, st, x, x_stride, n, dim, lo, hi, codes, row_stride, mags, raw_mags); break;
    case ENG_Q2: hipLaunchKernelGGL(quantize_rows_kernel<ENG_Q2>, grid, block, 0, st, x, x_stride, n, dim, lo, hi, codes, row_stride, mags, raw_mags); break;
    case ENG_F32: hipLaunchKernelGGL(quantize_rows_kernel<ENG_F32>, grid, block, 0, st, x, x_stride, n, dim, lo, hi, codes, row_stride, mags, raw_mags); break;
    case ENG_F16: hipLaunchKernelGGL(quantize_rows_kernel<ENG_F16>, grid, block, 0, st, x, x_stride, n, dim, lo, hi, codes, row_stride, mags, raw_mags); break;
    case ENG_Q1: hipLaunchKernelGGL(quantize_rows_kernel<ENG_Q1>, grid, block, 0, st, x, x_stride, n, dim, lo, hi, codes, row_stride, mags, raw_mags); break;
    case ENG_Q3: hipLaunchKernelGGL(quantize_rows_kernel<ENG_Q3>, grid, block, 0, st, x, x_stride, n, dim, lo, hi, codes, row_stride, mags, raw_mags); break;
    default: return hipErrorInvalidValue;
    }
    return hipGetLastError();
}

size_t walk_smem_bytes(const IndexDev &ix, u32 ef, int eng, u32 mmax, u32 win_bytes) {
    size_t b = (size_t)mmax * 8 + (size_t)ef * 8 + 64 * 4 * 2 + (size_t)win_bytes;
    b = (b + 15) & ~(size_t)15;
    if (eng == ENG_F32) b += (size_t)ix.row_stride;
    if (eng == ENG_F16) b += ((size_t)ix.dim * 4 + 15) & ~(size_t)15;
    return b + 16;
}

static int walk_pb_policy(u32 B, u32 ef, bool upper_range_of_a_split_walk) {
    const int forced = (int)tune_or(TUNE_WALK_PB, 0), forced_upper = (int)tune_or(TUNE_WALK_PB_UPPER, 0);
    if (upper_range_of_a_split_walk && (forced_upper == 4 || forced_upper == 8)) return forced_upper;
    if (forced == 4 || forced == 8) return forced;
    if (upper_range_of_a_split_walk && ef > 64u) return 4;
    return ef > 256u ? 4 : 8;
}

static u32 walk_merge_min_policy(u32 ef) {
    const long long forced = tune_or(TUNE_WALK_MERGE_MIN, -1);
    if (forced >= 0) return (u32)std::min<long long>(forced, 65);
    return ef <= 64u ? 4u : 3u;
}

template <int ENG, int CH, bool G64>
static hipError_t launch_walk_r(const IndexDev &ix, const WalkArgs &wa_in, hipStream_t st) {
    WalkArgs wa = wa_in;
    wa.merge_min = wa.tab != nullptr ? walk_merge_min_policy(wa.ef) : 0u;
    const u32 lf = wa.phase ? wa.level_first : ix.num_layers, ll = wa.phase ? wa.level_last : 0u;
    u32 mmax = 1;
    for (u32 l = ll; l <= lf; l++) mmax = std::max(mmax, ix.lv[l].M);
    constexpr bool TABLE_ENG = ENG == ENG_U8 || ENG == ENG_Q2;
    const bool all_tab = TABLE_ENG && wa.tab != nullptr && ll >= wa.tab_level_min && tune_or(TUNE_WALK_UPPER_LDS_PAD, 0) >= 0;
    wa.smem_mmax = mmax;
    size_t pad = 0;
    if (wa.phase != 0u && wa.level_last >= 1u) pad = (size_t)std::max<long long>(0, std::min<long long>(tune_or(TUNE_WALK_UPPER_LDS_PAD, 0), 48 << 10));
    dim3 grid(wa.B), block(64);
    const bool exact = ix.visited_mode != 0;
    constexpr bool HAS_PB8 = ENG == ENG_U8 && G64 && CH == 1;
    const bool pb8 = HAS_PB8 && walk_pb_policy(wa.B, wa.ef, wa.phase != 0u && wa.level_last >= 1u) == 8;
#define WALK(R_)                                                                                                          \
    do {                                                                                                                  \
        wa.smem_win_bytes = (all_tab && (R_) <= 4) ? (u32)(((64 * (R_) + 1) * 8 + 15) & ~15) : (u32)(LA * 64 * 4 * 3);         \
        const size_t smem = walk_smem_bytes(ix, wa.ef, ENG, mmax, wa.smem_win_bytes) + pad;                                \
        if constexpr (HAS_PB8) {                                                                                          \
            if (pb8) {                                                                                                    \
                if (exact) hipLaunchKernelGGL((walk_kernel<ENG, CH, R_, G64, true, 8>), grid, block, smem, st, ix, wa);   \
                else hipLaunchKernelGGL((walk_kernel<ENG, CH, R_, G64, false, 8>), grid, block, smem, st, ix, wa);        \
                break;                                                                                                    \
            }                                                                                                             \
        }                                                                                                                 \
        if (exact) hipLaunchKernelGGL((walk_kernel<ENG, CH, R_, G64, true>), grid, block, smem, st, ix, wa);              \
        else hipLaunchKernelGGL((walk_kernel<ENG, CH, R_, G64, false>), grid, block, smem, st, ix, wa);                   \
    } while (0)
    if (wa.ef <= 64) WALK(1);
    else if (wa.ef <= 128 && tune_or(TUNE_WALK_R2, 1) != 0) WALK(2);
    else if (wa.ef <= 256) WALK(4);
    else if (wa.ef <= 512) WALK(8);
    else if (wa.ef <= 1024) WALK(16);
    else return hipErrorInvalidValue;
#undef WALK
    return hipGetLastError();
}

hipError_t launch_walk_lat(int eng, const IndexDev &ix, const WalkArgs &wa, hipStream_t st);
hipError_t launch_walk_lat4(int eng, const IndexDev &ix, const WalkArgs &wa, hipStream_t st);
hipError_t launch_walk_general(int eng, const IndexDev &ix, const WalkArgs &wa, hipStream_t st);

hipError_t launch_walk(int eng, const IndexDev &ix, const WalkArgs &wa, WalkKernel kernel, hipStream_t st) {
    if (wa.B == 0) return hipSuccess;
    if (kernel == WalkKernel::General) return launch_walk_general(eng, ix, wa, st);
    if (kernel == WalkKernel::Lat4) return launch_walk_lat4(eng, ix, wa, st);
    if (kernel == WalkKernel::Lat1) return launch_walk_lat(eng, ix, wa, st);
    const u32 ch = (eng == ENG_F32 || eng == ENG_F16) ? 1 : (ix.nchunks + ix.G - 1) / ix.G;
    switch (eng) {
    case ENG_U8:
        if (ch == 1) return ix.G == 64 ? launch_walk_r<ENG_U8, 1, true>(ix, wa, st) : launch_walk_r<ENG_U8, 1, false>(ix, wa, st);
        if (ch == 2) return launch_walk_r<ENG_U8, 2, true>(ix, wa, st);
        if (ch == 3) return launch_walk_r<ENG_U8, 3, true>(ix, wa, st);
        if (ch == 4) return launch_walk_r<ENG_U8, 4, true>(ix, wa, st);
// ... 61 lines not shown
```

cosdata_amd/csrc/kernels_walk_lat4.hip:

```cpp
#include <hip/hip_runtime.h>

#include <cstdlib>

#include "engine_types.h"
#include "tuning.h"
#include "walk_common.h"

using namespace cosdev;

namespace {

constexpr int NW = 4;
constexpr int GL4 = LAT_ROW_LANES;
constexpr int PBL4 = 8;
constexpr u32 FREE = 0xFFFFFFFFu;

template <int ENG, int CH, int R, int E>
__global__ __launch_bounds__(256) void walk_lat4_kernel(const IndexDev ix, const WalkArgs wa) {
    extern __shared__ __attribute__((aligned(16))) unsigned char smem_raw[];
    constexpr u32 CAP = 64u * R;
    constexpr u32 LA = (u32)(NW * E);
    const int tid = threadIdx.x, lane = tid & 63, wave = __builtin_amdgcn_readfirstlane(tid >> 6);
    const u32 qi = blockIdx.x;
    if (qi >= wa.B) return;

    const u32 Mmax = walk_mmax(ix);
    u64 *s_pool, *s_res, *s_win, *s_cl, *s_spec;
    u32 *s_vis, *s_first, *s_flag, *s_misc;
    {
        unsigned char *p = smem_raw;
        s_pool = (u64 *)p;  p += (size_t)2 * CAP * 8;
        s_res = (u64 *)p;   p += (size_t)wa.ef * 8;
        s_win = (u64 *)p;   p += (size_t)LA * 64 * 8;
        s_cl = (u64 *)p;    p += (size_t)NW * E * 64 * 8;
        s_spec = (u64 *)p;  p += (size_t)NW * E * 64 * 8;
        s_first = (u32 *)p; p += (size_t)64 * Mmax * 4;
        s_vis = (u32 *)p;   p += (size_t)2 * Mmax * 4;
        s_flag = (u32 *)p;  p += (size_t)LA * 4;
        s_misc = (u32 *)p;
    }
    u64 *my_cl = s_cl + (size_t)wave * E * 64, *my_spec = s_spec + (size_t)wave * E * 64;

    const u32 qrow = wa.q_rows ? wa.q_rows[qi] : qi;
    const u32 self_id = wa.self_ids ? wa.self_ids[qi] * ix.id_stride : COS_QUERY_ID;
    const uint8_t *qcode = wa.qcodes + (u64)qrow * ix.row_stride;
    const float qmag = wa.qmags[qrow];
    const u32 N = ix.n;
    const u32 L = ix.num_layers;
    const u32 metric = ix.metric;

    const int lig = lane & (GL4 - 1);
    const int grp = lane / GL4;
    const u64 lt_mask = (1ull << lane) - 1ull;
    uint4 qreg[CH];
#pragma unroll
    for (int c = 0; c < CH; c++) {
        const u32 chunk = (u32)lig + (u32)c * (u32)GL4;
        qreg[c] = chunk < ix.nchunks ? *(const uint4 *)(qcode + (u64)chunk * 16) : make_uint4(0, 0, 0, 0);
    }

    for (u32 i = tid; i < 64u * Mmax; i += 256) s_first[i] = FREE;

    u64 n_evals = 0, n_exp = 0, adj_bytes = 0, n_rounds = 0;
    int32_t status = COS_OK;
    u32 entry = ix.lv[L].root_idx;

    auto single_distance = [&](u32 row, float &sim_out) -> bool {
        const u32 acc = int_row_dot_group0<ENG, CH>(qreg, ix.codes + (u64)row * ix.row_stride, ix.nchunks, lig, grp, GL4);
        bool bad;
        sim_out = cosine_or_dot(metric, (float)acc, qmag, uniform_f32(ix.mags[row]), bad);
        return !bad;
    };

    for (int level = (int)L; level >= 0; level--) {
        const LevelDev lv = ix.lv[level];
        const u32 M = lv.M;
        const u32 slots = M < ix.shortlist ? M : ix.shortlist;
        const u32 bitmask = 64u * M - 1u;
        const u32 out_slot = L - (u32)level;
        u32 cur = 0;
        const bool tab_level = ENG == ENG_U8 && wa.tab != nullptr && (u32)level >= wa.tab_level_min;
        const float *tabq = wa.tab + (u64)qi * wa.tab_stride + wa.tab_col0[level];
        const float *tabm = wa.tab_mags + wa.tab_col0[level];

        vis_clear<256>(s_vis, M, tid);
        __syncthreads();
        u32 npool = 0, npop = 0;
        if (wave == 0) {
            const u32 erow = uniform_u32(lv.node_vec ? lv.node_vec[entry] : entry);
            float s0 = 0.0f;
            bool ok;
            if (tab_level) {
                bool bad;
                s0 = cosine_or_dot(metric, uniform_f32(tabq[entry]), qmag, uniform_f32(tabm[entry]), bad);
                ok = !bad;
            } else
                ok = single_distance(erow, s0);
            if (lane == 0) {
                vis_set_bit(s_vis, self_id & bitmask);
                vis_set_bit(s_vis, vis_bit_of(erow, N, ix.id_stride, bitmask));
                s_pool[0] = pack_key(metric_key(metric, s0), entry);
                s_misc[1] = ok ? 0u : 1u;
            }
        }
        n_evals++;
        __syncthreads();
        if (uniform_u32(s_misc[1])) { status = COS_ERR_CALCULATION; break; }
        npool = 1;

        bool failed = false;
        while (npool > 0 && npop < wa.ef) {
            n_rounds++;
            u32 kwin = npool < LA ? npool : LA;
            if (kwin > wa.ef - npop) kwin = wa.ef - npop;
            const u64 *pool = s_pool + (size_t)cur * CAP;
            u64 *pool_nx = s_pool + (size_t)(cur ^ 1u) * CAP;

            u32 av[E], an[E], wnode[E];
            u64 wkey[E];
            const u32 slot_l = (u32)lane < slots ? (u32)lane : slots - 1u;
#pragma unroll
            for (int i = 0; i < E; i++) {
                const u32 e = (u32)(i * NW + wave);
                wkey[i] = pool[e < kwin ? e : 0u];
                wnode[i] = uniform_u32((u32)wkey[i]);
                av[i] = lv.adj_vec[(u64)wnode[i] * M + slot_l];
            }
            if (level != 0) {
#pragma unroll
                for (int i = 0; i < E; i++) an[i] = lv.adj_node[(u64)wnode[i] * M + slot_l];
            }
            const u64 last_key = pool[kwin - 1u];
            bool cnd[E];
            u32 bitv[E];
            u32 T = 0;
#pragma unroll
            for (int i = 0; i < E; i++) {
                const u32 e = (u32)(i * NW + wave);
                const bool live = e < kwin && (u32)lane < slots;
                av[i] = live ? av[i] : ROW_EMPTY;
                an[i] = live ? (level == 0 ? av[i] : an[i]) : ROW_EMPTY;
                bitv[i] = vis_bit_of(av[i], N, ix.id_stride, bitmask);
                const u32 vword = s_vis[bitv[i] >> 5];
                cnd[i] = av[i] != ROW_EMPTY && !(vword & (1u << (bitv[i] & 31u)));
                if (cnd[i]) atomicMin(&s_first[bitv[i]], e * 64u + (u32)lane);
                const u64 cm = ballot64(cnd[i]);
                if (cnd[i]) my_cl[T + (u32)__popcll(cm & lt_mask)] = (u64)av[i] | ((u64)(u32)(i * 64 + lane) << 32);
                T += (u32)__popcll(cm);
            }
            __builtin_amdgcn_wave_barrier();
            if (tab_level) {
#pragma unroll
                for (int i = 0; i < E; i++) {
                    float sim = 0.0f, magv = 1.0f;
                    if (cnd[i]) { sim = tabq[an[i]]; magv = tabm[an[i]]; }
                    bool bad;
                    sim = cosine_or_dot(metric, sim, qmag, magv, bad);
                    if (cnd[i]) my_spec[i * 64 + lane] = (u64)metric_key(metric, sim) | (bad ? (1ull << 32) : 0ull);
                }
                T = 0;
            }
            spec_row_dots<ENG, CH, GL4, PBL4>(my_cl, my_spec, T, qreg, ix, qmag, lig, grp);
            __syncthreads();

            bool win[E];
            u64 key[E];
            u64 wmask[E];
#pragma unroll
            for (int i = 0; i < E; i++) {
                const u32 e = (u32)(i * NW + wave);
                win[i] = cnd[i] && s_first[bitv[i]] == e * 64u + (u32)lane;
                const u64 sp = win[i] ? my_spec[i * 64 + lane] : 0ull;
                key[i] = pack_key((u32)sp, an[i]);
                wmask[i] = ballot64(win[i]);
                if (e < kwin) {
                    const bool stale = e + 1u < kwin && (wmask[i] & ballot64(key[i] > last_key)) != 0ull;
                    const bool bad = (wmask[i] & ballot64((sp >> 32) != 0ull)) != 0ull;
                    if (lane == 0) s_flag[e] = (stale ? 1u : 0u) | (bad ? 2u : 0u) | ((u32)__popcll(wmask[i]) << 8);
                }
            }
            __syncthreads();

            u32 j = kwin - 1u, n_valid = 0, my_base[E];
            {
                const u32 f = (u32)lane < kwin ? s_flag[lane] : 0u;
                bool found = false;
#pragma unroll
                for (int i = 0; i < E; i++) my_base[i] = 0;
#pragma unroll
                for (int e = 0; e < (int)LA; e++) {
                    const u32 fe = readlane_u32(f, e);
                    if ((u32)e < kwin && !found) {
#pragma unroll
                        for (int i = 0; i < E; i++)
                            if ((u32)(i * NW + wave) == (u32)e) my_base[i] = n_valid;
                        n_valid += fe >> 8;
                        if (fe & 2u) failed = true;
                        if (fe & 1u) { j = (u32)e; found = true; }
                    }
                }
            }
            if (failed) break;
#pragma unroll
            for (int i = 0; i < E; i++) {
                const u32 e = (u32)(i * NW + wave);
                if (win[i] && e <= j) {
                    atomicOr(&s_vis[bitv[i] >> 5], 1u << (bitv[i] & 31u));
                    s_win[my_base[i] + (u32)__popcll(wmask[i] & lt_mask)] = key[i];
                }
                if (cnd[i]) s_first[bitv[i]] = FREE;
            }
            if ((u32)tid <= j) s_res[npop + (u32)tid] = pool[tid];
            const u64 pk = (u32)tid < npool ? pool[tid] : 0ull;
            if (n_valid) __syncthreads();

            if (n_valid == 0u) {
                if ((u32)tid > j && (u32)tid < npool) pool_nx[(u32)tid - (j + 1u)] = pk;
            } else if (n_valid <= 64u && npool <= 64u) {
                if (wave == 0) {
                    const u64 kw_l = (u32)lane < n_valid ? s_win[lane] : 0ull;
                    const bool live_p = (u32)lane > j && (u32)lane < npool;
                    u32 pos_p = (u32)lane - (j + 1u), pos_w = 0;
                    for (u32 w = 0; w < n_valid; w++) {
                        const u64 kw = readlane_u64(kw_l, (int)w);
                        pos_p += kw > pk ? 1u : 0u;
                        pos_w += kw > kw_l ? 1u : 0u;
                        const u32 above = (u32)__popcll(ballot64(live_p && pk > kw));
                        if ((u32)lane == w) pos_w += above;
                    }
                    if (live_p && pos_p < CAP) pool_nx[pos_p] = pk;
                    if ((u32)lane < n_valid && pos_w < CAP) pool_nx[pos_w] = kw_l;
                }
            } else {
            constexpr int WR = (int)((LA * 64u + 63u) / 64u);
            u64 wreg[WR];
#pragma unroll
            for (int r = 0; r < WR; r++) wreg[r] = ((u32)(r * 64 + lane) < n_valid) ? s_win[r * 64 + lane] : 0ull;
            u32 pos_p = (u32)tid - (j + 1u);
// ... 113 lines not shown
```

cosdata_amd/csrc/walk_common.h:

```cpp
#pragma once
#include "engine_types.h"
#include "dot_engines.h"
#include "topk_select.h"

namespace cosdev {

constexpr int32_t COS_OK = 0, COS_ERR_CALCULATION = 2, COS_ERR_UNIMPLEMENTED = 4;
constexpr u32 COS_QUERY_ID = 0xFFFFFFFEu;
constexpr u32 COS_ROOT_ID = 0xFFFFFFFFu;
constexpr int LAT_ROW_LANES = 16;

__host__ __device__ __forceinline__ u32 walk_mmax(const IndexDev &ix) {
    return ix.lv[0].M > ix.lv[ix.num_layers].M ? ix.lv[0].M : ix.lv[ix.num_layers].M;
}

__device__ __forceinline__ u32 vis_bit_of(u32 row, u32 N, u32 id_stride, u32 bitmask) {
    const u32 id = row == N ? COS_ROOT_ID : row * id_stride;
    return id & bitmask;
}
template <int NT>
__device__ __forceinline__ void vis_clear(u32 *vis, u32 M, int tid) {
    for (u32 w = tid; w < 2 * M; w += NT) vis[w] = 0;
}
__device__ __forceinline__ void vis_set_bit(u32 *vis, u32 bit) { vis[bit >> 5] |= 1u << (bit & 31); }
__device__ __forceinline__ u64 vis_alias_winners(u64 cmask, u32 bit, u64 lostmask) {
    u64 wmask = cmask & ~lostmask;
    while (lostmask) {
        const int l = __ffsll((long long)lostmask) - 1;
        const u64 g = cmask & ballot64(bit == readlane_u32(bit, l));
        wmask = (wmask & ~g) | (g & (0ull - g));
        lostmask &= ~g;
    }
    return wmask;
}

template <bool UNSCALED = false>
__device__ __forceinline__ float cosine_or_dot(u32 metric, float dotf, float qmag, float mag, bool &bad) {
    bad = false;
    if (metric != 0u) return dotf;
    const float den = __fmul_rn(qmag, mag);
    bad = den == 0.0f;
    return UNSCALED ? div_rn_unscaled(dotf, den) : __fdiv_rn(dotf, den);
}

template <int ENG, int CH>
__device__ __forceinline__ u32 int_row_dot_group0(const uint4 (&qreg)[CH], const uint8_t *row_ptr, u32 nchunks, int lig, int grp, int G) {
    u32 acc = 0;
    if (grp == 0) {
#pragma unroll
        for (int c = 0; c < CH; c++) {
            const u32 chunk = (u32)lig + (u32)c * (u32)G;
            if (chunk < nchunks) acc = chunk_dot<ENG>(qreg[c], *(const uint4 *)(row_ptr + (u64)chunk * 16), acc);
        }
    }
    acc = group_reduce_add_u32(acc, G);
    return readlane_u32(acc, 0);
}

template <int ENG, int CH, int GL, int PB>
__device__ __forceinline__ void spec_row_dots(const u64 *cl, u64 *spec, u32 T, const uint4 (&qreg)[CH], const IndexDev &ix, float qmag, int lig, int grp) {
    constexpr int RP = 64 / GL;
    for (u32 b0 = 0; b0 < T; b0 += RP * PB) {
        uint4 buf[PB][CH];
        float pmag[PB];
        u32 ppos[PB], prow[PB];
#pragma unroll
        for (int p = 0; p < PB; p++) {
            if (b0 + (u32)(p * RP) >= T) break;
            const u32 my = b0 + (u32)(p * RP + grp);
            const bool v = my < T;
            const u64 e = cl[v ? my : b0];
            prow[p] = (u32)e;
            ppos[p] = v ? (u32)(e >> 32) : 0xFFFFFFFFu;
        }
#pragma unroll
        for (int p = 0; p < PB; p++) {
            if (b0 + (u32)(p * RP) >= T) break;
            pmag[p] = ix.mags[prow[p]];
            const uint8_t *rp = ix.codes + (u64)prow[p] * ix.row_stride;
#pragma unroll
            for (int c = 0; c < CH; c++) {
                u32 chunk = (u32)lig + (u32)c * (u32)GL;
                if (c == CH - 1) chunk = chunk < ix.nchunks ? chunk : ix.nchunks - 1u;
                buf[p][c] = *(const uint4 *)(rp + (u64)chunk * 16);
            }
        }
#pragma unroll
        for (int p = 0; p < PB; p++) {
            if (b0 + (u32)(p * RP) >= T) break;
            u32 part[CH];
#pragma unroll
            for (int c = 0; c < CH; c++) part[c] = chunk_dot<ENG>(qreg[c], buf[p][c], 0u);
            u32 acc = part[0];
#pragma unroll
            for (int c = 1; c < CH; c++) acc += part[c];
            acc = group_reduce_add_u32(acc, GL);
            bool bad;
            const float sim = cosine_or_dot(ix.metric, (float)acc, qmag, pmag[p], bad);
            if (lig == 0 && ppos[p] != 0xFFFFFFFFu) spec[ppos[p]] = (u64)metric_key(ix.metric, sim) | (bad ? (1ull << 32) : 0ull);
        }
    }
}

template <int R>
__device__ __forceinline__ void sort_popped_list(u64 (&rk)[R], const u64 *res, u32 npop, int lane) {
#pragma unroll
    for (int r = 0; r < R; r++) {
        const u32 e = (u32)lane * R + r;
        rk[r] = e < npop ? res[e] : 0ull;
    }
    bitonic_sort_desc<R>(rk, lane);
}
__device__ __forceinline__ void write_level_entry(u64 key, u64 pos, const IndexDev &ix, const LevelDev &lv, const WalkArgs &wa) {
    const u32 nd = (u32)key;
    const u32 vrow = lv.node_vec ? lv.node_vec[nd] : nd;
    wa.out_ids[pos] = vrow == ix.n ? COS_ROOT_ID : vrow * ix.id_stride;
// ... 26 lines not shown
```

cosdata_amd/csrc/walk_kernel.inc:

```
constexpr int PB = 4;
constexpr int LA = 4;

struct WalkSmem {
    u32 *vis;
    u64 *res;
    u32 *wl_vec;
    u32 *wl_node;
    u32 *win_vec;
    u32 *win_node;
    float *win_mag;
    float *qf;
};

template <int ENG, int CH, int R, bool G64, bool EXACT, int PB64 = 4>
__global__ __launch_bounds__(64) __attribute__((amdgpu_waves_per_eu(CH >= 3 ? (R <= 4 ? (CH == 3 ? 4 : 3) : (CH == 3 ? 3 : 2)) : (R == 1 ? ((ENG == ENG_U8 && CH == 1 && G64 && !EXACT) ? 7 : 6) : (R <= 4 ? 5 : 4)), 8))) void walk_kernel(const IndexDev ix, const WalkArgs wa) {
    extern __shared__ __attribute__((aligned(16))) unsigned char smem_raw[];
    const int lane = threadIdx.x;
    if (blockIdx.x >= wa.B) return;
    const u32 qi = wa.q_order ? wa.q_order[blockIdx.x] : blockIdx.x;
    const bool resume = wa.phase != 0u && wa.level_first < ix.num_layers;
    if (resume && wa.out_status[qi] != COS_OK) return;

    const u32 Mmax = wa.smem_mmax;
    WalkSmem sm;
// ... 7 lines not shown
        sm.win_node = (u32 *)(p + LA * 64 * 4);
        sm.win_mag = (float *)(p + 2 * LA * 64 * 4);
        p += wa.smem_win_bytes;
        p = (unsigned char *)(((size_t)p + 15) & ~(size_t)15);
        sm.qf = (float *)p;
    }

    const u32 qrow = wa.q_rows ? wa.q_rows[qi] : qi;
    const u32 self_id = wa.self_ids ? wa.self_ids[qi] * ix.id_stride : COS_QUERY_ID;
    const uint8_t *qcode = wa.qcodes + (u64)qrow * ix.row_stride;
    const float qmag = wa.qmags[qrow];
    const u32 N = ix.n;
    const u32 L = ix.num_layers;
    const u32 metric = ix.metric;
    constexpr bool exact = EXACT;
    u32 *vis = exact ? wa.vis_bits + (u64)qi * wa.vis_words_per_query : sm.vis;
    u32 *vlog = exact ? wa.vis_log + (u64)qi * wa.vis_log_cap : nullptr;

    constexpr bool FLOAT_ENG = ENG == ENG_F32 || ENG == ENG_F16;
    constexpr bool TABLE_OK = ENG == ENG_U8 || ENG == ENG_Q2;
    const int G = (ENG == ENG_F32) ? 8 : (ENG == ENG_F16 ? 1 : (int)ix.G);
    const int lig = lane & (G - 1);
    const int grp = lane / G;
    const int RP = 64 / G;
    uint4 qreg[CH];
    if constexpr (!FLOAT_ENG) {
#pragma unroll
        for (int c = 0; c < CH; c++) {
            u32 chunk = (u32)lig + (u32)c * (u32)G;
            qreg[c] = chunk < ix.nchunks ? *(const uint4 *)(qcode + (u64)chunk * 16) : make_uint4(0, 0, 0, 0);
        }
    } else if constexpr (ENG == ENG_F16) {
        const __half *qh = (const __half *)qcode;
        for (u32 i = lane; i < ix.dim; i += 64) sm.qf[i] = __half2float(qh[i]);
        __builtin_amdgcn_s_waitcnt(0);
#pragma unroll
        for (int c = 0; c < CH; c++) qreg[c] = make_uint4(0, 0, 0, 0);
    } else {
        const float *qg = (const float *)qcode;
        for (u32 i = lane; i < (u32)(ix.row_stride / 4); i += 64) sm.qf[i] = qg[i];
        __builtin_amdgcn_s_waitcnt(0);
#pragma unroll
        for (int c = 0; c < CH; c++) qreg[c] = make_uint4(0, 0, 0, 0);
    }

    u32 loff64[CH];
#pragma unroll
    for (int c = 0; c < CH; c++) {
        const u32 chunk = (u32)lane + (u32)c * 64u;
        loff64[c] = (chunk < ix.nchunks ? chunk : 0u) * 16u;
    }

    u64 n_evals = 0, n_exp = 0, adj_bytes = 0, n_rounds = 0, n_tab = 0;
    const u32 merge_min = uniform_u32(wa.merge_min);
    int32_t status = COS_OK;
    u32 entry = uniform_u32(resume ? wa.entry0[qi] : ix.lv[L].root_idx);
    const int level_first = wa.phase ? (int)wa.level_first : (int)L, level_last = wa.phase ? (int)wa.level_last : 0;
    u32 order_key = wa.key_n;

    auto single_distance = [&](u32 row, float &sim_out) -> bool {
        float dotf;
        if constexpr (!FLOAT_ENG) {
            dotf = (float)int_row_dot_group0<ENG, CH>(qreg, ix.codes + (u64)row * ix.row_stride, ix.nchunks, lig, grp, G);
        } else if constexpr (ENG == ENG_F16) {
            float d = f16_lane_dot(ix.codes + (u64)row * ix.row_stride, sm.qf, ix.dim);
            dotf = __uint_as_float(readlane_u32(__float_as_uint(d), 0));
        } else {
            float d = f32_oct_dot((const float *)(ix.codes + (u64)row * ix.row_stride), sm.qf, ix.dim, lane & 7);
            dotf = __uint_as_float(readlane_u32(__float_as_uint(d), 0));
        }
        bool bad;
        sim_out = cosine_or_dot(metric, dotf, qmag, uniform_f32(ix.mags[row]), bad);
        return !bad;
    };

    for (int level = level_first; level >= level_last; level--) {
        const LevelDev lv = ix.lv[level];
        const u32 M = lv.M;
        const u32 slots = M < ix.shortlist ? M : ix.shortlist;
        const u32 bitmask = 64u * M - 1u;
        const u32 out_slot = L - (u32)level;
        u32 nlog = 0;
        const bool tab_level = TABLE_OK && wa.tab != nullptr && (u32)level >= wa.tab_level_min;
        const float *tabq = wa.tab + (u64)qi * wa.tab_stride + wa.tab_col0[level];
        const float *tabm = wa.tab_mags + wa.tab_col0[level];

        if (!exact) {
            vis_clear<64>(sm.vis, M, lane);
            if (lane == 0 && wa.no_self_seed == 0u) vis_set_bit(sm.vis, self_id & bitmask);
        }

        Pool<R> pool;
        pool.clear();
        u32 npool = 0, npop = 0;
        u32 res_lo = 0, res_hi = 0;

        {
            const u32 erow = uniform_u32(lv.node_vec ? lv.node_vec[entry] : entry);
            float s0;
            if (tab_level) {
                bool bad;
                s0 = cosine_or_dot(metric, uniform_f32(tabq[entry]), qmag, uniform_f32(tabm[entry]), bad);
                if (bad) { status = COS_ERR_CALCULATION; break; }
            } else if (!single_distance(erow, s0)) { status = COS_ERR_CALCULATION; break; }
            if (lane == 0) {
                if (!exact) vis_set_bit(sm.vis, vis_bit_of(erow, N, ix.id_stride, bitmask));
                else {
                    atomicOr(&vis[entry >> 5], 1u << (entry & 31));
                    vlog[0] = entry >> 5;
                }
            }
            pool.insert_at(pack_key(metric_key(metric, s0), entry), 0, lane);
            npool = 1;
            if (exact) nlog = 1;
        }

        u32 failed = 0;
        u32 lev_evals = 1;
        const u32 log2M = (u32)__ffs((int)M) - 1u;
        const u64 slotmask = slots >= 64u ? ~0ull : ((1ull << slots) - 1ull);
        auto level_rounds = [&](auto tabc, auto cosc, auto amagc) __attribute__((always_inline)) {
        constexpr bool TAB = decltype(tabc)::value;
        constexpr bool COSINE = decltype(cosc)::value;
        constexpr bool AMAG = decltype(amagc)::value && G64 && !FLOAT_ENG;
        const u32 metric_t = COSINE ? 0u : metric;
        while (npool > 0 && npop < wa.ef) {
            n_rounds++;
            u32 kwin = npool < (u32)LA ? npool : (u32)LA;
            if (kwin > wa.ef - npop) kwin = wa.ef - npop;
            u32 wv_[LA], wn_[LA];
            {
                const u32 slot_l = (u32)lane < slots ? (u32)lane : slots - 1u;
                auto fetch_stage = [&](auto bothc) {
                    constexpr bool BOTH = decltype(bothc)::value;
                    float wm_[LA];
                    static_for<0, LA>([&](auto ic) {
                        constexpr int i = decltype(ic)::value;
                        const u32 nd = pool.template peek_node<i>();
                        const u64 off = ((u64)nd << log2M) + slot_l;
                        wv_[i] = lv.adj_vec[off];
                        if constexpr (BOTH) wn_[i] = lv.adj_node[off];
                        if constexpr (!TAB && AMAG) wm_[i] = lv.adj_mag[(u64)nd * lv.mag_stride + slot_l];
                    });
                    if constexpr (!TAB) {
                        static_for<0, LA>([&](auto ic) {
                            constexpr int i = decltype(ic)::value;
                            sm.win_vec[i * 64 + lane] = wv_[i];
                            sm.win_node[i * 64 + lane] = BOTH ? wn_[i] : wv_[i];
                            if constexpr (AMAG) sm.win_mag[i * 64 + lane] = wm_[i];
                        });
                    }
                };
                if (TAB || level != 0) fetch_stage(std::true_type{});
                else fetch_stage(std::false_type{});
            }
            u32 stop = 0;
            auto consume = [&](u32 wi, u32 nb_vec, u32 nb_node, float nb_mag) __attribute__((always_inline)) {
                if constexpr (R == 1) {
                    const u64 hd = pool.head();
                    res_lo = writelane_dyn(res_lo, (u32)hd, (int)npop);
                    res_hi = writelane_dyn(res_hi, (u32)(hd >> 32), (int)npop);
                } else if (lane == 0) sm.res[npop] = pool.e[0];
                pool.pop_head(lane);
                npool--;
                npop++;
                const int limit = (int)wa.ef - (int)npop;
                const int ahead = (int)kwin - 1 - (int)wi;
                u32 window_ok = 1;

                const u64 vmask = ballot64(nb_vec != ROW_EMPTY) & slotmask;
                u64 wmask;
                if (!exact) {
                    u32 bit = vis_bit_of(nb_vec, N, 1u, bitmask);
                    if (ix.id_stride != 1u) {
                        asm volatile("");
                        bit = vis_bit_of(nb_vec, N, ix.id_stride, bitmask);
                    }
                    const u32 word = bit >> 5, msk = 1u << (bit & 31);
                    u32 seen = sm.vis[word];
                    asm volatile("" : "+v"(seen));
                    const u64 cmask = vmask & ballot64((seen & msk) == 0u);
                    wmask = cmask;
                    if (cmask) {
                    u32 old = 0;
                    if (__builtin_amdgcn_inverse_ballot_w64(cmask)) old = atomicOr(&sm.vis[word], msk);
                    wmask = vis_alias_winners(cmask, bit, cmask & ballot64((old & msk) != 0u));
                    }
                } else {
                    u32 w = 0;
                    if (__builtin_amdgcn_inverse_ballot_w64(vmask)) w = __hip_atomic_load(&vis[nb_node >> 5], __ATOMIC_RELAXED, __HIP_MEMORY_SCOPE_AGENT);
                    wmask = vmask & ballot64(((w >> (nb_node & 31)) & 1u) == 0u);
                    if (__builtin_amdgcn_inverse_ballot_w64(wmask)) {
                        atomicOr(&vis[nb_node >> 5], 1u << (nb_node & 31));
                        vlog[nlog + (u32)__popcll(wmask & ((1ull << lane) - 1ull))] = nb_node >> 5;
                    }
                    nlog += (u32)__popcll(wmask);
                }
                if (wmask) {
                const bool win = __builtin_amdgcn_inverse_ballot_w64(wmask);
                const int W = __popcll(wmask);
                lev_evals += (u32)W;
                auto insert_serial = [&](u64 pm, u32 keyv, u32 nodev) {
                    while (pm) {
                        const int p = __ffsll((long long)pm) - 1;
                        pm = clear_bit_u64(pm, p);
                        const u64 kk = pack_key(readlane_u32(keyv, p), readlane_u32(nodev, p));
                        const int pos = pool.rank_of(kk);
                        if (pos < limit) {
                            pool.insert_at(kk, pos, lane);
                            npool = npool + 1u < (u32)(64 * R) ? npool + 1u : (u32)(64 * R);
                            window_ok = pos < ahead ? 0u : window_ok;
                        }
                    }
                };
                auto commit = [&](u64 leadmask, u32 keyv, u32 nodev) {
                    const u64 bar = limit > 0 ? pool.peek_dyn((u32)(limit - 1)) : ~0ull;
                    insert_serial(leadmask & ballot64(pack_key(keyv, nodev) > bar), keyv, nodev);
                };
                auto commit_merge = [&](u64 leadmask, u32 keyv, u32 nodev) {
                    const u64 bar = limit > 0 ? pool.peek_dyn((u32)(limit - 1)) : ~0ull;
                    const u64 mykey = pack_key(keyv, nodev);
                    const u64 pm = leadmask & ballot64(mykey > bar);
                    const u32 Wp = (u32)__popcll(pm);
                    if (Wp < merge_min) { insert_serial(pm, keyv, nodev); return; }
                    u32 below[R];
#pragma unroll
                    for (int r = 0; r < R; r++) below[r] = 0u;
                    u32 posv = 0u;
                    u32 abovev = 0u;
                    u32 minrank = ~0u;
                    u64 m = pm;
                    while (m) {
                        const int p = __ffsll((long long)m) - 1;
                        m = clear_bit_u64(m, p);
                        const u64 kk = pack_key(readlane_u32(keyv, p), readlane_u32(nodev, p));
                        u32 rank = 0;
#pragma unroll
                        for (int r = 0; r < R; r++) {
                            const bool gt = pool.e[r] > kk;
                            rank += (u32)__popcll(ballot64(gt));
                            below[r] += gt ? 1u : 0u;
                        }
                        minrank = rank < minrank ? rank : minrank;
                        abovev += kk > mykey ? 1u : 0u;
                        posv = writelane_dyn(posv, rank, p);
                    }
                    window_ok = (int)minrank < ahead ? 0u : window_ok;
                    u64 *mg = (u64 *)sm.win_vec;
#pragma unroll
                    for (int r = 0; r < R; r++) {
                        u32 np = (u32)lane * R + r + (Wp - below[r]);
                        np = np < (u32)(64 * R) ? np : (u32)(64 * R);
                        mg[np] = pool.e[r];
                    }
                    if (__builtin_amdgcn_inverse_ballot_w64(pm)) {
                        u32 np = posv + abovev;
                        np = np < (u32)(64 * R) ? np : (u32)(64 * R);
                        mg[np] = mykey;
                    }
                    __builtin_amdgcn_fence(__ATOMIC_RELEASE, "wavefront");
                    __builtin_amdgcn_wave_barrier();
                    __builtin_amdgcn_fence(__ATOMIC_ACQUIRE, "wavefront");
#pragma unroll
                    for (int r = 0; r < R; r++) pool.e[r] = mg[(u32)lane * R + r];
                    npool = npool + Wp < (u32)(64 * R) ? npool + Wp : (u32)(64 * R);
                };
                if constexpr (TAB) {
                    float simv = 0.0f, magv = 1.0f;
                    if (win) { simv = tabq[nb_node]; magv = tabm[nb_node]; }
                    bool badl;
                    simv = cosine_or_dot<ENG == ENG_U8>(metric_t, simv, qmag, magv, badl);
                    if (wmask & ballot64(badl)) failed = 1;
                    else if constexpr (R <= 4) {
                        if (merge_min != 0u) commit_merge(wmask, metric_key(metric_t, simv), nb_node);
                        else commit(wmask, metric_key(metric_t, simv), nb_node);
                    } else commit(wmask, metric_key(metric_t, simv), nb_node);
                } else if constexpr (G64 && !FLOAT_ENG) {
                    float magw = 1.0f;
                    if constexpr (AMAG) magw = nb_mag;
                    else if (win) magw = ix.mags[nb_vec];
                    u64 m = wmask;
                    while (m && !failed) {
                        u32 lsel = 0;
                        u32 tot = 0;
                        u64 leadmask = 0;
                        auto eval_block = [&](auto npc) {
                            constexpr int NP = decltype(npc)::value;
                            constexpr int LS = 64 / NP;
                            uint4 buf[NP][CH];
                            int cnt = 0;
                            static_for<0, NP>([&](auto pc) {
                                constexpr int p = decltype(pc)::value;
                                if (m) {
                                    const int l = __ffsll((long long)m) - 1;
                                    m = clear_bit_u64(m, l);
                                    const uint8_t *rp = row_ptr_scalar(ix.codes, readlane_u32(nb_vec, l), (u32)ix.row_stride);
                                    lsel = writelane_u32<p * LS>(lsel, (u32)l << 2);
#pragma unroll
                                    for (int c = 0; c < CH; c++) {
                                        u32 lo = loff64[c];
                                        asm("" : "+v"(lo));
                                        buf[p][c] = *(const uint4 *)(rp + lo);
                                    }
                                    cnt++;
                                }
                            });
                            u32 acc[NP];
                            static_for<0, NP>([&](auto pc) {
                                constexpr int p = decltype(pc)::value;
                                acc[p] = 0;
                                if (p < cnt) {
                                    asm volatile("");
#pragma unroll
                                    for (int c = 0; c < CH; c++) acc[p] = chunk_dot<ENG>(qreg[c], buf[p][c], acc[p]);
                                }
                            });
                            tot = wave_reduce_rows<NP>(acc);
                            constexpr u64 firsts = NP == 8 ? 0x0101010101010101ull : 0x0001000100010001ull;
                            leadmask = cnt == NP ? firsts : firsts & ((1ull << (cnt * LS)) - 1ull);
                        };
                        if constexpr (PB64 == 8) {
                            if (__popcll(m) > 4) eval_block(std::integral_constant<int, 8>{});
                            else eval_block(std::integral_constant<int, 4>{});
                        } else {
                            eval_block(std::integral_constant<int, 4>{});
                        }
                        const float magv = __uint_as_float((u32)__builtin_amdgcn_ds_bpermute((int)lsel, (int)__float_as_uint(magw)));
                        const u32 nodev = (u32)__builtin_amdgcn_ds_bpermute((int)lsel, (int)nb_node);
                        const float dotv = (float)tot;
                        bool badl;
                        const float sim = cosine_or_dot<ENG == ENG_U8>(metric, dotv, qmag, magv, badl);
                        if (leadmask & ballot64(badl)) { failed = 1; break; }
                        commit(leadmask, metric_key(metric, sim), nodev);
                    }
                } else {
                if (win) {
                    const int rank = __popcll(wmask & ((1ull << lane) - 1ull));
                    sm.wl_vec[rank] = nb_vec;
                    sm.wl_node[rank] = nb_node;
                }

                for (int base = 0; base < W; base += RP * PB) {
                    u32 prow[PB];
                    float pmag[PB];
                    uint4 buf[PB][CH];
                    float fdot[PB];
#pragma unroll
                    for (int p = 0; p < PB; p++) {
                        if (base + p * RP >= W) break;
                        const int my = base + p * RP + grp;
                        const bool v = my < W;
                        prow[p] = v ? sm.wl_vec[my] : 0u;
                        pmag[p] = 1.0f;
                        if (v) pmag[p] = ix.mags[prow[p]];
                        if constexpr (!FLOAT_ENG) {
#pragma unroll
                            for (int c = 0; c < CH; c++) {
                                u32 chunk = (u32)lig + (u32)c * (u32)G;
                                buf[p][c] = make_uint4(0, 0, 0, 0);
                                if (v && chunk < ix.nchunks) buf[p][c] = *(const uint4 *)(ix.codes + (u64)prow[p] * ix.row_stride + (u64)chunk * 16);
                            }
                        }
                    }
                    if constexpr (FLOAT_ENG) {
#pragma unroll
                        for (int p = 0; p < PB; p++) {
                            if (base + p * RP >= W) break;
                            if constexpr (ENG == ENG_F32)
                                fdot[p] = f32_oct_dot((const float *)(ix.codes + (u64)prow[p] * ix.row_stride), sm.qf, ix.dim, lane & 7);
                            else
                                fdot[p] = f16_lane_dot(ix.codes + (u64)prow[p] * ix.row_stride, sm.qf, ix.dim);
                        }
                    }
#pragma unroll
                    for (int p = 0; p < PB; p++) {
                        if (base + p * RP >= W) break;
                        float dotf;
                        if constexpr (!FLOAT_ENG) {
                            u32 acc = 0;
#pragma unroll
                            for (int c = 0; c < CH; c++) acc = chunk_dot<ENG>(qreg[c], buf[p][c], acc);
                            acc = group_reduce_add_u32(acc, G);
                            dotf = (float)acc;
                        } else {
                            dotf = fdot[p];
                        }
                        const int mine = base + p * RP + grp;
                        const bool leadg = lig == 0 && mine < W;
                        bool badl;
                        const float sim = cosine_or_dot(metric, dotf, qmag, pmag[p], badl);
                        if (ballot64(mine < W && badl)) { failed = 1; break; }
                        const u32 mynode = leadg ? sm.wl_node[mine] : 0u;
                        commit(ballot64(leadg), metric_key(metric, sim), mynode);
                    }
                    if (failed) break;
                }
                }
                stop = failed | (window_ok ^ 1u);
                }
            };
            if constexpr (TAB) {
                static_for<0, LA>([&](auto ic) __attribute__((always_inline)) {
                    constexpr int i = decltype(ic)::value;
                    if ((u32)i < kwin && !stop) consume((u32)i, wv_[i], wn_[i], 1.0f);
                });
            } else {
                for (u32 wi = 0; wi < kwin && !stop; wi++)
                    consume(wi, sm.win_vec[wi * 64 + lane], sm.win_node[wi * 64 + lane], AMAG ? sm.win_mag[wi * 64 + lane] : 1.0f);
            }
            if (failed) break;
        }
        };
        if (tab_level) {
            if (metric == 0u) level_rounds(std::true_type{}, std::true_type{}, std::false_type{});
            else level_rounds(std::true_type{}, std::false_type{}, std::false_type{});
        } else {
            bool done = false;
            if constexpr (G64 && !FLOAT_ENG) {
                if (lv.adj_mag != nullptr) {
                    level_rounds(std::false_type{}, std::false_type{}, std::true_type{});
                    done = true;
                }
            }
            if (!done) level_rounds(std::false_type{}, std::false_type{}, std::false_type{});
        }
        n_exp += npop;
        adj_bytes += (u64)npop * slots * 4;
        n_evals += lev_evals;
        if (tab_level) n_tab += lev_evals;
        if (exact) {
            __atomic_signal_fence(__ATOMIC_SEQ_CST);
            __builtin_amdgcn_s_waitcnt(0);
            for (u32 i = lane; i < nlog; i += 64) {
                const u32 w = __hip_atomic_load(&vlog[i], __ATOMIC_RELAXED, __HIP_MEMORY_SCOPE_AGENT);
                __hip_atomic_store(&vis[w], 0u, __ATOMIC_RELAXED, __HIP_MEMORY_SCOPE_AGENT);
            }
            __atomic_signal_fence(__ATOMIC_SEQ_CST);
            __builtin_amdgcn_s_waitcnt(0);
        }
        if (failed) { status = COS_ERR_CALCULATION; break; }

        u64 rk[R];
#pragma unroll
        for (int r = 0; r < R; r++) {
            const u32 e = (u32)lane * R + r;
            if constexpr (R == 1) rk[r] = e < npop ? pack_key(res_hi, res_lo) : 0ull;
            else rk[r] = e < npop ? sm.res[e] : 0ull;
        }
        bitonic_sort_desc<R>(rk, lane);
        u32 cnt = npop < wa.keep ? npop : wa.keep;
        if (npop == 0) {
            const u32 erow = uniform_u32(lv.node_vec ? lv.node_vec[entry] : entry);
            float s0;
            if (!single_distance(erow, s0)) { status = COS_ERR_CALCULATION; break; }
            rk[0] = lane == 0 ? pack_key(metric_key(metric, s0), entry) : 0ull;
            cnt = 1;
        }
        const u64 obase = level_list_base(ix, wa, qi, out_slot);
#pragma unroll
        for (int r = 0; r < R; r++) {
            const u32 e = (u32)lane * R + r;
            if (e < cnt) {
                const u32 nd = (u32)rk[r];
                const u32 vrow = lv.node_vec ? lv.node_vec[nd] : nd;
                wa.out_ids[obase + e] = vrow == N ? COS_ROOT_ID : vrow * ix.id_stride;
                wa.out_sims[obase + e] = metric_key_inv(metric, (u32)(rk[r] >> 32));
                if (wa.out_nodes) wa.out_nodes[obase + e] = nd;
            }
        }
        if (lane == 0) wa.out_counts[(u64)qi * (L + 1) + out_slot] = cnt;
        if (level > 0) {
            const u32 best = (u32)readlane_u64(rk[0], 0);
            entry = uniform_u32(lv.child[best]);
            if (wa.phase != 0u && level == level_last) order_key = uniform_u32(wa.order_rank[best]);
        }
    }

    if (lane == 0) {
        wa.out_status[qi] = status;
        if (wa.phase != 0u && level_last > 0) {
            wa.entry0[qi] = entry;
            wa.order_key[qi] = status == COS_OK ? order_key : wa.key_n;
            wa.order_iota[qi] = qi;
        }
        if (wa.out_stats) {
            const bool add = resume;
            wa.out_stats[(u64)qi * 4 + 0] = n_evals + (add ? wa.out_stats[(u64)qi * 4 + 0] : 0ull);
            wa.out_stats[(u64)qi * 4 + 1] = n_exp + (add ? wa.out_stats[(u64)qi * 4 + 1] : 0ull);
            wa.out_stats[(u64)qi * 4 + 2] = adj_bytes + (add ? wa.out_stats[(u64)qi * 4 + 2] : 0ull);
            wa.out_stats[(u64)qi * 4 + 3] = n_rounds + (add ? wa.out_stats[(u64)qi * 4 + 3] : 0ull);
        }
// ... 11 lines not shown
```

cosdata_amd/index.py:

```python
from __future__ import annotations

import ctypes as C
import enum
from dataclasses import dataclass
from typing import List, Optional, Sequence, Tuple

import numpy as np

from . import _lib
from ._lib import CosdataError, CosFlatStats, CosParams, CosSearchStats, CosTimingSummary, CosWalkSplit, check

ROOT_ID, QUERY_ID, SLOT_EMPTY = 0xFFFFFFFF, 0xFFFFFFFE, 0xFFFFFFFD
VISITED_REF, VISITED_EXACT = 0, 1


class DistanceMetric(enum.IntEnum):
    Cosine = 0
    Euclidean = 1
    Hamming = 2
    DotProduct = 3


class StorageKind(enum.IntEnum):
    UnsignedByte = 0
# ... 169 lines not shown
    def load_reference_dir(self, dense_hnsw_dir: str, root_ptr_offset: int, verify_codes: bool = False):
        check(_lib.lib().cos_index_load_reference_dir(self._h, dense_hnsw_dir.encode(), root_ptr_offset, 1 if verify_codes else 0))
        return self

    def build(self, batch_size: int = 0):
        check(_lib.lib().cos_index_build(self._h, batch_size))
        return self

    def append(self, raw_new, batch_size: int = 0):
        x = _c(np.atleast_2d(raw_new), np.float32)
        if x.ndim != 2 or x.shape[1] != self.dim or x.shape[0] == 0:
            raise CosdataError(_lib.ERR_INVALID, f"new vectors must be [m][{self.dim}] f32, got shape {tuple(x.shape)}")
        check(_lib.lib().cos_index_append(self._h, _p(x), x.shape[0], 0, batch_size))
        self.n += x.shape[0]
        return self

    def append_device(self, dev_ptr_all: int, m: int, batch_size: int = 0, keepalive=None):
        check(_lib.lib().cos_index_append(self._h, C.c_void_p(dev_ptr_all), m, 1, batch_size))
        self.n += m
        self._keepalive = keepalive
        return self

    def delete(self, ids):
        a = _c(np.atleast_1d(ids), np.uint32)
        check(_lib.lib().cos_index_delete(self._h, _p(a), a.size))
        return self

    def restore_link_state(self):
        check(_lib.lib().cos_index_restore_link_state(self._h))
        return self

    def release_link_state(self):
        check(_lib.lib().cos_index_release_link_state(self._h))
        return self

    def set_ef_search(self, ef: int):
        check(_lib.lib().cos_index_set_ef_search(self._h, ef))
        self.hnsw_params.ef_search = ef

    def set_coalescing(self, max_queries: int, window_us: int = 200):
        check(_lib.lib().cos_index_set_coalescing(self._h, max_queries, window_us))

    def coalescing_stats(self) -> dict:
        st = _lib.CosCoalescingStats()
        check(_lib.lib().cos_index_coalescing_stats(self._h, C.byref(st)))
        return {f: int(getattr(st, f)) for f, _ in st._fields_}

    def set_visited_mode(self, mode: int):
        check(_lib.lib().cos_index_set_visited_mode(self._h, mode))

    LATENCY_MODE_DEFAULT_MAX_B = 2048

    def set_latency_mode(self, max_queries: int):
        check(_lib.lib().cos_index_set_latency_mode(self._h, max_queries))

    LATENCY_WAVES_DEFAULT_MAX_B = 512

    def set_latency_waves(self, max_queries: int):
        check(_lib.lib().cos_index_set_latency_waves(self._h, max_queries))

    WALK_ORDER_DEFAULT_MIN_B = 8192

    def set_walk_order(self, min_queries: int):
        check(_lib.lib().cos_index_set_walk_order(self._h, min_queries))

    def walk_order_cuts(self):
        lv = (C.c_uint32 * 16)()
        n = C.c_uint32()
        check(_lib.lib().cos_index_walk_order_cuts(self._h, lv, 16, C.byref(n)))
        return [int(lv[i]) for i in range(min(n.value, 16))]

    WALK_TABLE_DEFAULT_MIN_B = 1
    WALK_TABLE_DEFAULT_MAX_COLS = 8192
    WALK_TABLE_AUTO = 0xFFFFFFFF

    def set_walk_table(self, max_cols: int = WALK_TABLE_AUTO, min_queries: int = WALK_TABLE_DEFAULT_MIN_B):
        check(_lib.lib().cos_index_set_walk_table(self._h, max_cols, min_queries))

    def walk_table_info(self):
        lv, cols = C.c_uint32(), C.c_uint32()
        check(_lib.lib().cos_index_walk_table_info(self._h, C.byref(lv), C.byref(cols)))
        return int(lv.value), int(cols.value)

    def last_walk_split(self, stream: int = 0) -> CosWalkSplit:
        st = CosWalkSplit()
        st.struct_size = C.sizeof(CosWalkSplit)
        check(_lib.lib().cos_index_last_walk_split(self._h, C.c_void_p(stream), C.byref(st)))
        return st

    def batch_search(self, queries, top_k: int, return_status: bool = False):
        q = self._queries(queries)
        B = q.shape[0]
        ids = np.full((B, top_k), 0xFFFFFFFF, np.uint32)
        scores = np.zeros((B, top_k), np.float32)
        counts = np.zeros(B, np.uint32)
        status = np.zeros(B, np.int32)
        rc = _lib.lib().cos_search_batch(self._h, _p(q), B, top_k, _p(ids), _p(scores), _p(counts), _p(status))
        if return_status:
            return ids, scores, counts, rc, status
        check(rc)
        return ids, scores, counts

    def search_internal(self, query, top_k: int):
        ids, scores, counts = self.batch_search(np.asarray(query, np.float32)[None, :], top_k)
        return [(int(ids[0, i]), float(scores[0, i])) for i in range(int(counts[0]))]

    def batch_search_device(self, q_ptr: int, B: int, top_k: int, out_ids_ptr: int, out_scores_ptr: int, out_counts_ptr: int,
                            out_status_ptr: int, stream: int = 0):
        check(_lib.lib().cos_search_batch_device(self._h, C.c_void_p(q_ptr), B, top_k, C.c_void_p(out_ids_ptr),
                                                 C.c_void_p(out_scores_ptr), C.c_void_p(out_counts_ptr),
                                                 C.c_void_p(out_status_ptr), C.c_void_p(stream)))

    def ann_search_batch(self, queries):
        q = self._queries(queries)
        B, L1 = q.shape[0], self.hnsw_params.num_layers + 1
        ids = np.zeros((B, L1, 100), np.uint32)
        sims = np.zeros((B, L1, 100), np.float32)
        counts = np.zeros((B, L1), np.uint32)
        status = np.zeros(B, np.int32)
        check(_lib.lib().cos_ann_search_batch(self._h, _p(q), B, _p(ids), _p(sims), _p(counts), _p(status)))
        return ids, sims, counts

    def enable_metadata(self, mdim: int, max_replicas_per_node: int):
        check(_lib.lib().cos_index_enable_metadata(self._h, mdim, max_replicas_per_node))
        self.mdim = mdim
        return self

    def upload_meta_graph(self, node_ids, mbits, levels):
        ids, mb = _c(node_ids, np.uint32), _c(mbits, np.int32)
        assert mb.shape == (ids.size, self.mdim)
        check(_lib.lib().cos_index_upload_meta_nodes(self._h, ids.size, _p(ids), _p(mb)))
        for l, (lid, nbr) in enumerate(levels):
            lid, nbr = _c(lid, np.uint32), _c(nbr, np.uint32)
            assert nbr.shape == (lid.size, self.level_M(l))
            check(_lib.lib().cos_index_upload_meta_graph_level(self._h, l, lid.size, _p(lid), _p(nbr)))
        return self

    def build_meta(self, node_ids, mbits, max_levels, batch_size: int = 0):
        ids, mb, ml = _c(node_ids, np.uint32), _c(mbits, np.int32), _c(max_levels, np.uint8)
        assert mb.shape == (ids.size, self.mdim) and ml.size == ids.size
        check(_lib.lib().cos_index_build_meta(self._h, ids.size, _p(ids), _p(mb), _p(ml), batch_size))
        return self

    def download_meta_graph(self):
        out = []
        for l in range(self.hnsw_params.num_layers + 1):
            n = C.c_uint32()
            check(_lib.lib().cos_index_meta_level_count(self._h, l, C.byref(n)))
            ids = np.zeros(n.value, np.uint32)
            nbr = np.zeros((n.value, self.level_M(l)), np.uint32)
            check(_lib.lib().cos_index_download_meta_graph_level(self._h, l, _p(ids), _p(nbr)))
            out.append((ids, nbr))
        return out

    def _filters(self, filter_offsets, filter_dims):
        off, fd = _c(filter_offsets, np.uint32), _c(np.atleast_2d(filter_dims), np.int8)
        if fd.shape[1] != self.mdim or off[-1] != fd.shape[0]:
            raise CosdataError(_lib.ERR_INVALID, f"filters must be [F][{self.mdim}] i8 with offsets ending at F")
        return off, fd

    def search_filtered(self, queries, filter_offsets, filter_dims, top_k: int, return_status: bool = False):
        q = self._queries(queries)
        off, fd = self._filters(filter_offsets, filter_dims)
        B = q.shape[0]
        ids = np.full((B, top_k), 0xFFFFFFFF, np.uint32)
        scores = np.zeros((B, top_k), np.float32)
# ... 49 lines not shown
```

include/cosdata_hip.h:

```cpp
#ifndef COSDATA_HIP_H
#define COSDATA_HIP_H

#include <stddef.h>
#include <stdint.h>

#ifdef __cplusplus
extern "C" {
#endif

#define COS_ABI_VERSION 1u

typedef enum { COS_METRIC_COSINE = 0, COS_METRIC_EUCLIDEAN = 1, COS_METRIC_HAMMING = 2, COS_METRIC_DOT = 3 } cos_metric;
typedef enum { COS_STORAGE_U8 = 0, COS_STORAGE_SUBBYTE = 1, COS_STORAGE_F16 = 2, COS_STORAGE_F32 = 3 } cos_storage;

typedef enum {
    COS_OK = 0,
    COS_ERR_STORAGE_MISMATCH = 1,
    COS_ERR_CALCULATION = 2,
    COS_ERR_INVALID = 3,
    COS_ERR_UNIMPLEMENTED = 4,
    COS_ERR_HIP = 5,
    COS_ERR_NOT_READY = 6,
    COS_ERR_NO_DEVICE = 7
} cos_status;
// ... 23 lines not shown
    uint32_t ef_search;
    uint32_t shortlist_size;
    uint32_t visited_mode;
    int32_t device;
    uint32_t id_base;
    uint32_t reserved;
    uint64_t seed;
} cos_params;

typedef struct cos_index cos_index;

typedef struct {
    uint64_t evals;
    uint64_t expansions;
    uint64_t adj_bytes;
    uint64_t rerank_rows;
    float walk_ms;
    float finalize_ms;
    float prep_ms;
    uint32_t reserved;
} cos_search_stats;

int32_t cos_index_create(const cos_params *params, cos_index **out);
int32_t cos_index_destroy(cos_index *ix);
const char *cos_last_error_string(void);
int32_t cos_device_count(int32_t *out);
int32_t cos_hbm_probe(int32_t device, uint32_t kind, uint64_t buffer_bytes, uint32_t row_bytes, uint32_t iters,
                      double *out_gbps);

int32_t cos_index_upload_vectors(cos_index *ix, const float *raw, uint32_t n, uint32_t flags);
int32_t cos_index_set_root(cos_index *ix, const float *root_raw);
int32_t cos_index_upload_graph_level(cos_index *ix, uint32_t level, uint32_t n_nodes, const uint32_t *node_ids,
                                     const uint32_t *nbr_ids);
int32_t cos_index_level_count(const cos_index *ix, uint32_t level, uint32_t *n_nodes);
int32_t cos_index_download_graph_level(const cos_index *ix, uint32_t level, uint32_t *node_ids, uint32_t *nbr_ids);
int32_t cos_index_download_codes(const cos_index *ix, void *codes, float *mags);
int32_t cos_index_download_root(const cos_index *ix, float *root_raw);

#define COS_LOAD_DEFAULT 0u
#define COS_LOAD_VERIFY_CODES 1u
int32_t cos_index_load_reference_dir(cos_index *ix, const char *dense_hnsw_dir, uint32_t root_ptr_offset, uint32_t flags);
int32_t cos_reference_dir_level_counts(const char *dense_hnsw_dir, uint32_t num_layers, uint32_t neighbors_count,
                                       uint32_t level0_neighbors_count, uint32_t *level_counts );
int32_t cos_reference_dir_read_level(const char *dense_hnsw_dir, uint32_t num_layers, uint32_t neighbors_count,
                                     uint32_t level0_neighbors_count, uint32_t level, uint32_t *node_ids, uint32_t *nbr_ids);

int32_t cos_index_build(cos_index *ix, uint32_t batch_size);
int32_t cos_index_append(cos_index *ix, const float *raw, uint32_t m, uint32_t flags, uint32_t batch_size );
int32_t cos_index_delete(cos_index *ix, const uint32_t *ids, uint32_t m);
int32_t cos_index_restore_link_state(cos_index *ix);
int32_t cos_index_release_link_state(cos_index *ix);

int32_t cos_search_batch(cos_index *ix, const float *queries, uint32_t B, uint32_t top_k, uint32_t *out_ids,
                         float *out_scores, uint32_t *out_counts, int32_t *out_status);
int32_t cos_search_batch_device(cos_index *ix, const float *d_queries, uint32_t B, uint32_t top_k, uint32_t *d_out_ids,
                                float *d_out_scores, uint32_t *d_out_counts, int32_t *d_out_status, void *stream);
int32_t cos_ann_search_batch(cos_index *ix, const float *queries, uint32_t B, uint32_t *out_ids, float *out_sims,
                             uint32_t *out_counts, int32_t *out_status);
int32_t cos_index_set_coalescing(cos_index *ix, uint32_t max_queries, uint32_t window_us);
typedef struct cos_coalescing_stats {
    uint64_t launches;
    uint64_t queries;
    uint64_t requests;
    uint64_t closed_full;
    uint64_t closed_quiet;
    uint64_t closed_deadline;
    uint64_t solo_calls;
} cos_coalescing_stats;
int32_t cos_index_coalescing_stats(cos_index *ix, cos_coalescing_stats *out);
int32_t cos_index_set_ef_search(cos_index *ix, uint32_t ef_search);
int32_t cos_index_set_visited_mode(cos_index *ix, uint32_t mode);
#define COS_LATENCY_MODE_DEFAULT_MAX_B 2048u
int32_t cos_index_set_latency_mode(cos_index *ix, uint32_t max_queries);
#define COS_LATENCY_WAVES_DEFAULT_MAX_B 512u
int32_t cos_index_set_latency_waves(cos_index *ix, uint32_t max_queries);
#define COS_WALK_ORDER_DEFAULT_MIN_B 8192u
int32_t cos_index_set_walk_order(cos_index *ix, uint32_t min_queries);
int32_t cos_index_walk_order_cuts(cos_index *ix, uint32_t *out_levels, uint32_t cap, uint32_t *out_n);
#define COS_WALK_TABLE_DEFAULT_MIN_B 1u
#define COS_WALK_TABLE_DEFAULT_MAX_COLS 8192u
#define COS_WALK_TABLE_AUTO 0xFFFFFFFFu
int32_t cos_index_set_walk_table(cos_index *ix, uint32_t max_cols, uint32_t min_queries);
int32_t cos_index_walk_table_info(cos_index *ix, uint32_t *out_level_min, uint32_t *out_cols);
typedef struct {
    uint32_t struct_size;
    uint32_t queries;
    uint32_t table_level_min;
    uint32_t table_cols;
    uint32_t cut_after_level;
    uint32_t reserved;
    float table_ms;
    float upper_ms, sort_ms, lower_ms;
    double table_int8_ops;
    uint64_t table_evals;
    uint64_t upper_evals, upper_expansions, upper_adj_bytes;
    uint64_t lower_evals, lower_expansions, lower_adj_bytes;
} cos_walk_split;
int32_t cos_index_last_walk_split(cos_index *ix, void *stream, cos_walk_split *out);
int32_t cos_index_enable_timing(cos_index *ix, int32_t on);
int32_t cos_index_last_stats(cos_index *ix, void *stream, cos_search_stats *out);
typedef struct {
    uint32_t launches;
    float prep_ms_sum, walk_ms_sum, finalize_ms_sum;
    float walk_ms_min, walk_ms_max;
} cos_timing_summary;
int32_t cos_index_timing_summary(cos_index *ix, void *stream, cos_timing_summary *out);

int32_t cos_index_enable_metadata(cos_index *ix, uint32_t mdim , uint32_t max_replicas_per_node);
int32_t cos_index_upload_meta_nodes(cos_index *ix, uint32_t n_nodes, const uint32_t *node_ids, const int32_t *mbits);
int32_t cos_index_upload_meta_graph_level(cos_index *ix, uint32_t level, uint32_t n_nodes, const uint32_t *node_ids,
                                          const uint32_t *nbr_ids);
int32_t cos_index_build_meta(cos_index *ix, uint32_t n_nodes, const uint32_t *node_ids, const int32_t *mbits, const uint8_t *max_levels,
                             uint32_t batch_size );
int32_t cos_index_meta_level_count(cos_index *ix, uint32_t level, uint32_t *out);
int32_t cos_index_download_meta_graph_level(cos_index *ix, uint32_t level, uint32_t *node_ids, uint32_t *nbr_ids);
int32_t cos_search_filtered_batch(cos_index *ix, const float *queries, uint32_t B, const uint32_t *filter_offsets,
                                  const int8_t *filter_dims, uint32_t top_k, uint32_t *out_ids, float *out_scores,
                                  uint32_t *out_counts, int32_t *out_status);
int32_t cos_ann_search_filtered_batch(cos_index *ix, const float *queries, uint32_t B, const uint32_t *filter_offsets,
                                      const int8_t *filter_dims, uint32_t *out_ids, float *out_sims, uint32_t *out_counts,
                                      int32_t *out_status);

int32_t cos_quantize_batch(uint32_t storage, uint32_t resolution, uint32_t dim, float range_lo, float range_hi,
                           const float *x, uint32_t n, void *codes, float *mags);
size_t cos_code_bytes(uint32_t storage, uint32_t resolution, uint32_t dim);
int32_t cos_sample_values_range(const float *x, uint32_t n, uint32_t dim, float clamp_margin_percent, float *range_lo,
                                float *range_hi);
int32_t cos_distance_batch(uint32_t metric, uint32_t storage, uint32_t resolution, uint32_t dim, const void *x_codes,
                           const float *x_mags, uint32_t nx, const void *y_codes, const float *y_mags, uint32_t ny,
                           const uint32_t *pair_x, const uint32_t *pair_y, uint32_t n_pairs, float *out,
                           int32_t *status);
int32_t cos_bruteforce_topk(cos_index *ix, const float *queries, uint32_t B, uint32_t k, uint32_t *out_ids,
                            float *out_scores);

typedef struct {
    float gemm_ms;
    uint32_t gemm_launches;
    double int8_ops;
    double code_bytes;
} cos_flat_stats;
int32_t cos_flat_search_batch(cos_index *ix, const float *queries, uint32_t B, uint32_t top_k, uint32_t *out_ids,
                              float *out_scores, uint32_t *out_counts, cos_flat_stats *stats );

typedef struct cos_bm25 cos_bm25;
int32_t cos_bm25_create(int32_t device, const uint32_t *term_hashes, const uint64_t *offsets, uint32_t n_terms,
                        const uint32_t *doc_ids, const float *tfs, uint32_t documents_count, cos_bm25 **out);
int32_t cos_bm25_destroy(cos_bm25 *b);
int32_t cos_bm25_insert(cos_bm25 *b, const uint32_t *doc_ids, const uint64_t *doc_offsets, uint32_t m, const uint32_t *term_hashes,
                        const float *tfs);
int32_t cos_bm25_delete(cos_bm25 *b, const uint32_t *doc_ids, const uint64_t *doc_offsets, uint32_t m, const uint32_t *term_hashes);
typedef struct {
    uint32_t struct_size;
    uint32_t documents_count;
    uint32_t n_terms;
    uint32_t largest_doc_id;
    uint32_t dir_rows;
    uint32_t dir_tiles;
    uint32_t reserved;
    uint64_t postings;
    uint64_t tombstones;
    uint64_t device_bytes;
} cos_bm25_index_stats;
int32_t cos_bm25_stats(cos_bm25 *b, cos_bm25_index_stats *out);
int32_t cos_bm25_download(cos_bm25 *b, uint32_t *n_terms, uint64_t *n_postings, uint32_t *term_hashes, uint64_t *offsets,
                          uint32_t *doc_ids, float *tfs, uint8_t *tombstones);
int32_t cos_bm25_search_batch(cos_bm25 *b, const uint32_t *q_terms, const uint32_t *q_offsets, uint32_t B,
                              uint32_t top_k, uint32_t *out_ids, float *out_scores, uint32_t *out_counts);
int32_t cos_bm25_search_batch_device(cos_bm25 *b, const uint32_t *q_terms, const uint32_t *q_offsets, uint32_t B, uint32_t top_k,
                                     uint32_t *d_out_ids, float *d_out_scores, uint32_t *d_out_counts, void *stream);
int32_t cos_rrf_fuse_batch(const uint32_t *dense_ids, const uint32_t *dense_counts, uint32_t dense_stride,
                           const uint32_t *sparse_ids, const uint32_t *sparse_counts, uint32_t sparse_stride, uint32_t B,
                           float fusion_constant_k, uint32_t top_k, uint32_t *out_ids, float *out_scores,
                           uint32_t *out_counts);
// ... 90 lines not shown
```

Measured before the change: 1.015 million.

## Deduplicate walk-table columns across HNSW levels and remap adjacency to column ids

The precomputed query-vs-upper-levels similarity table previously held one column per node per level, so a vector present on several levels was scored several times. Columns are now deduplicated by underlying vector row, with a per-level adjacency-to-column map used by the walk kernel to index the table. Query code sums are also filled during quantization, so the table kernel can skip recomputing them. The cost is one extra adjacency-column load per neighbour in the table path and extra device memory for the column maps.

```diff
diff --git a/cosdata_amd/_lib.py b/cosdata_amd/_lib.py
--- a/cosdata_amd/_lib.py
+++ b/cosdata_amd/_lib.py
@@ -44,7 +44,7 @@
 class CosWalkSplit(C.Structure):
     _fields_ = [
         ("struct_size", C.c_uint32), ("queries", C.c_uint32), ("table_level_min", C.c_uint32), ("table_cols", C.c_uint32),
-        ("cut_after_level", C.c_uint32), ("reserved", C.c_uint32),
+        ("cut_after_level", C.c_uint32), ("table_phys_cols", C.c_uint32),
         ("table_ms", C.c_float), ("upper_ms", C.c_float), ("sort_ms", C.c_float), ("lower_ms", C.c_float),
         ("table_int8_ops", C.c_double), ("table_evals", C.c_uint64),
         ("upper_evals", C.c_uint64), ("upper_expansions", C.c_uint64), ("upper_adj_bytes", C.c_uint64),
@@ -104,7 +104,7 @@
     "cos_index_download_graph_level", "cos_index_download_codes", "cos_index_download_root", "cos_index_build", "cos_index_append", "cos_index_delete", "cos_index_restore_link_state", "cos_index_release_link_state", "cos_index_enable_metadata", "cos_index_upload_meta_nodes", "cos_index_upload_meta_graph_level", "cos_index_build_meta", "cos_index_meta_level_count", "cos_index_download_meta_graph_level", "cos_search_filtered_batch",
     "cos_ann_search_filtered_batch", "cos_index_load_reference_dir", "cos_reference_dir_level_counts", "cos_reference_dir_read_level",
     "cos_search_batch", "cos_search_batch_device", "cos_ann_search_batch", "cos_index_set_coalescing", "cos_index_coalescing_stats", "cos_index_set_ef_search",
-    "cos_index_set_visited_mode", "cos_index_set_latency_mode", "cos_index_set_latency_waves", "cos_index_set_walk_order", "cos_index_walk_order_cuts", "cos_index_set_walk_table", "cos_index_walk_table_info", "cos_index_last_walk_split", "cos_index_enable_timing", "cos_index_last_stats", "cos_index_timing_summary", "cos_quantize_batch",
+    "cos_index_set_visited_mode", "cos_index_set_latency_mode", "cos_index_set_latency_waves", "cos_index_set_walk_order", "cos_index_walk_order_cuts", "cos_index_set_walk_table", "cos_index_walk_table_info", "cos_index_walk_table_phys_cols", "cos_index_last_walk_split", "cos_index_enable_timing", "cos_index_last_stats", "cos_index_timing_summary", "cos_quantize_batch",
     "cos_code_bytes", "cos_sample_values_range", "cos_distance_batch", "cos_bruteforce_topk", "cos_flat_search_batch", "cos_bm25_create", "cos_bm25_destroy",
     "cos_bm25_insert", "cos_bm25_delete", "cos_bm25_stats", "cos_bm25_download",
     "cos_bm25_search_batch", "cos_bm25_search_batch_device", "cos_rrf_fuse_batch", "cos_hybrid_search_batch", "cos_text_process", "cos_text_count_tokens", "cos_bm25_term_frequency", "cos_xxhash32", "cos_stem_english", "cos_sparse_create", "cos_sparse_build_csr", "cos_sparse_create_from_vectors", "cos_sparse_destroy", "cos_sparse_search_batch", "cos_sparse_last_stats", "cos_sparse_layout",
@@ -170,6 +170,7 @@
         "cos_index_last_stats": [vp, vp, C.POINTER(CosSearchStats)],
         "cos_index_set_walk_table": [vp, u32, u32],
         "cos_index_walk_table_info": [vp, C.POINTER(u32), C.POINTER(u32)],
+        "cos_index_walk_table_phys_cols": [vp, C.POINTER(u32)],
         "cos_index_last_walk_split": [vp, vp, C.POINTER(CosWalkSplit)],
         "cos_index_timing_summary": [vp, vp, C.POINTER(CosTimingSummary)],
         "cos_quantize_batch": [u32, u32, u32, f32, f32, vp, u32, vp, vp],
diff --git a/cosdata_amd/csrc/engine.hip b/cosdata_amd/csrc/engine.hip
--- a/cosdata_amd/csrc/engine.hip
+++ b/cosdata_amd/csrc/engine.hip
@@ -15,6 +15,7 @@
 #include <vector>
 
 #include "engine_internal.h"
+#include "table_columns.h"
 
 using namespace cosdev;
 
@@ -666,9 +667,21 @@
     ix->d_tcodes = nullptr;
     ix->d_tmags = nullptr;
     ix->d_tcsums = nullptr;
+    for (auto &a : ix->d_tadj_col) a = nullptr;
     ix->table_cols = 0;
+    ix->table_phys_cols = 0;
     ix->table_level_min = 0;
     ix->table_stride = 0;
+}
+void cos_index::view_table_set(const TableSet &t) {
+    table_level_min = t.level_min;
+    table_cols = t.cols;
+    table_phys_cols = t.phys_cols;
+    table_stride = t.stride;
+    d_tcodes = t.tcodes;
+    d_tmags = t.tmags;
+    d_tcsums = t.tcsums;
+    for (u32 l = 0; l < cosdev::MAX_LEVELS; l++) d_tadj_col[l] = l == t.level_min && l < lv.size() ? (const u32 *)lv[l].d_adj_node : (const u32 *)t.adj_col[l];
 }
 static u32 walk_table_max_cols(const cos_index *ix) {
     const long long env = cosdev::tune_or(cosdev::TUNE_WALK_TABLE_COLS, -1);
@@ -724,13 +737,7 @@
     clear_current_table(ix);
     for (const auto &t : ix->table_sets)
         if (t.key == key) {
-            ix->table_level_min = t.level_min;
-            ix->table_cols = t.cols;
-            ix->table_stride = t.stride;
-            memcpy(ix->table_col0, t.col0, sizeof(t.col0));
-            ix->d_tcodes = t.tcodes;
-            ix->d_tmags = t.tmags;
-            ix->d_tcsums = t.tcsums;
+            ix->view_table_set(t);
             return COS_OK;
         }
     if (!cosdev::level_table_eng_supported(ix->eng, ix->row_stride) || max_cols == 0) return COS_OK;
@@ -743,18 +750,37 @@
     }
     if (lmin == 0) return COS_OK;
     HIP_TRY(hipDeviceSynchronize());
+    std::vector<std::vector<u32>> h_child(Ltop + 1), h_node_vec(Ltop + 1);
+    cosdev::TableLevelIn lin[cosdev::MAX_LEVELS] = {};
+    for (u32 l = lmin; l <= Ltop; l++) {
+        const u32 n = ix->lv[l].n;
+        h_node_vec[l].resize(n);
+        HIP_TRY(hipMemcpy(h_node_vec[l].data(), ix->lv[l].d_node_vec, (size_t)n * 4, hipMemcpyDeviceToHost));
+        if (l > lmin && ix->lv[l].d_child) {
+            h_child[l].resize(n);
+            HIP_TRY(hipMemcpy(h_child[l].data(), ix->lv[l].d_child, (size_t)n * 4, hipMemcpyDeviceToHost));
+        }
+        lin[l] = cosdev::TableLevelIn{n, h_child[l].empty() ? nullptr : h_child[l].data(), h_node_vec[l].data()};
+    }
+    const cosdev::TableColumns tc = cosdev::table_columns(lin, lmin, Ltop);
+    const u32 phys = tc.phys_cols;
     cos_index::TableSet t;
     auto build = [&]() -> hipError_t {
-        hipError_t e = t.tcodes.alloc((size_t)cols * ix->row_stride);
-        if (e == hipSuccess) e = t.tmags.alloc(cols);
-        if (e == hipSuccess) e = t.tcsums.alloc(cols);
-        u32 c0 = 0;
-        for (u32 l = Ltop; l >= lmin && e == hipSuccess; l--) {
-            ix->table_col0[l] = c0;
-            e = cosdev::launch_level_table_gather(ix->d_codes, ix->d_mags, ix->row_stride, ix->lv[l].d_node_vec, ix->lv[l].n, c0, t.tcodes, t.tmags, nullptr);
-            c0 += ix->lv[l].n;
-        }
-        if (e == hipSuccess) e = cosdev::launch_code_sums(t.tcodes, ix->row_stride, cols, t.tcsums, nullptr);
+        DevArr<u32> col_row;
+        hipError_t e = t.tcodes.alloc((size_t)phys * ix->row_stride);
+        if (e == hipSuccess) e = t.tmags.alloc(phys);
+        if (e == hipSuccess) e = t.tcsums.alloc(phys);
+        if (e == hipSuccess) e = col_row.alloc(phys);
+        if (e == hipSuccess) e = hipMemcpy(col_row, tc.col_row.data(), (size_t)phys * 4, hipMemcpyHostToDevice);
+        if (e == hipSuccess) e = cosdev::launch_level_table_gather(ix->d_codes, ix->d_mags, ix->row_stride, col_row, phys, 0u, t.tcodes, t.tmags, nullptr);
+        if (e == hipSuccess) e = cosdev::launch_code_sums(t.tcodes, ix->row_stride, phys, t.tcsums, nullptr);
+        for (u32 l = Ltop; l > lmin && e == hipSuccess; l--) {
+            const u32 n = ix->lv[l].n;
+            const u64 n_slots = (u64)n * ix->lv[l].M;
+            e = t.adj_col[l].alloc(n_slots + n);
+            if (e == hipSuccess) e = hipMemcpy(t.adj_col[l].p + n_slots, tc.node_col[l - lmin].data(), (size_t)n * 4, hipMemcpyHostToDevice);
+            if (e == hipSuccess) e = cosdev::launch_level_table_adj_col(ix->lv[l].d_adj_node, t.adj_col[l].p + n_slots, n, n_slots, t.adj_col[l], nullptr);
+        }
         if (e == hipSuccess) e = hipDeviceSynchronize();
         return e;
     };
@@ -767,17 +793,12 @@
         ix->level_table_valid = false;
         HIP_TRY(e);
     }
-    ix->d_tcodes = t.tcodes;
-    ix->d_tmags = t.tmags;
-    ix->d_tcsums = t.tcsums;
-    ix->table_cols = cols;
-    ix->table_level_min = lmin;
-    ix->table_stride = ((u64)cols + 31) / 32 * 32;
     t.key = key;
     t.level_min = lmin;
     t.cols = cols;
-    t.stride = ix->table_stride;
-    memcpy(t.col0, ix->table_col0, sizeof(t.col0));
+    t.phys_cols = phys;
+    t.stride = ((u64)phys + 31) / 32 * 32;
+    ix->view_table_set(t);
     ix->table_sets.push_back(std::move(t));
     return COS_OK;
 }
@@ -791,9 +812,8 @@
     return COS_OK;
 }
 
-extern "C" int32_t cos_index_walk_table_info(cos_index *ix, uint32_t *out_level_min, uint32_t *out_cols) {
-    if (!ix || !out_level_min || !out_cols) return cos_fail(COS_ERR_INVALID, "null argument");
-    *out_level_min = *out_cols = 0;
+static int32_t walk_table_view(cos_index *ix, uint32_t *out_level_min, uint32_t *out_cols, uint32_t *out_phys_cols) {
+    *out_level_min = *out_cols = *out_phys_cols = 0;
     if (!graph_ready(ix)) return cos_fail(COS_ERR_NOT_READY, "index needs vectors, root and every graph level");
     int32_t rc = cos_set_device(ix);
     if (rc) return rc;
@@ -802,7 +822,20 @@
     if ((rc = ensure_level_table(ix))) return rc;
     *out_level_min = ix->table_level_min;
     *out_cols = ix->table_cols;
-    return COS_OK;
+    *out_phys_cols = ix->table_phys_cols;
+    return COS_OK;
+}
+
+extern "C" int32_t cos_index_walk_table_info(cos_index *ix, uint32_t *out_level_min, uint32_t *out_cols) {
+    if (!ix || !out_level_min || !out_cols) return cos_fail(COS_ERR_INVALID, "null argument");
+    uint32_t phys = 0;
+    return walk_table_view(ix, out_level_min, out_cols, &phys);
+}
+
+extern "C" int32_t cos_index_walk_table_phys_cols(cos_index *ix, uint32_t *out_phys_cols) {
+    if (!ix || !out_phys_cols) return cos_fail(COS_ERR_INVALID, "null argument");
+    uint32_t lmin = 0, cols = 0;
+    return walk_table_view(ix, &lmin, &cols, out_phys_cols);
 }
 
 static int32_t ensure_adj_mags(cos_index *ix) {
@@ -860,10 +893,11 @@
     u32 ef = 0, visited_mode = 0;
     bool timed = false;
     u64 tab_stride = 0;
-    u32 tab_col0[cosdev::MAX_LEVELS] = {};
+    u32 tab_phys_cols = 0;
     const uint8_t *tcodes = nullptr;
     const float *tmags = nullptr;
     const u32 *tcsums = nullptr;
+    const u32 *tadj_col[cosdev::MAX_LEVELS] = {};
     u32 n_keys = 0, key_level[cosdev::MAX_LEVELS], key_n[cosdev::MAX_LEVELS];
     const u32 *order_rank[cosdev::MAX_LEVELS];
 };
@@ -943,10 +977,11 @@
     L->plan = cosdev::walk_plan(in, &have);
     if (L->plan.use_table) {
         L->tab_stride = ix->table_stride;
-        memcpy(L->tab_col0, ix->table_col0, sizeof(L->tab_col0));
+        L->tab_phys_cols = ix->table_phys_cols;
         L->tcodes = ix->d_tcodes;
         L->tmags = ix->d_tmags;
         L->tcsums = ix->d_tcsums;
+        memcpy(L->tadj_col, ix->d_tadj_col, sizeof(L->tadj_col));
     }
     if (L->plan.ordered)
         for (u32 l : ix->order_levels) {
@@ -989,16 +1024,17 @@
     }
     hipEvent_t *ev = &w->ev[(size_t)(w->ev_count % Workspace::EV_RING) * Workspace::EV_PER];
     if (timed) HIP_TRY(hipEventRecord(ev[0], st));
+    const bool qsums_filled = plan.use_table && ix->eng == ENG_U8;
     HIP_TRY(launch_quantize_rows(ix->eng, d_queries, ix->p.dim, B, ix->p.dim, ix->p.range_lo, ix->p.range_hi, w->q_codes, ix->row_stride,
-                                 w->q_mags, w->q_raw_mags, st));
+                                 w->q_mags, w->q_raw_mags, st, qsums_filled ? w->qsums.p : nullptr));
     if (plan.use_table) {
         if (plan.table_waits_for_sort) {
             std::lock_guard<std::mutex> g(ix->chain_mu);
             if (ix->chain_last_range_ev && ix->chain_last_range_ev != w->last_range) HIP_TRY(hipStreamWaitEvent(st, ix->chain_last_range_ev, 0));
         }
         if (timed) HIP_TRY(hipEventRecord(ev[4], st));
-        HIP_TRY(cosdev::launch_level_table(ix->eng, w->q_codes, w->q_mags, w->qsums, w->qdig, B, L.tcodes, L.tmags, L.tcsums, ix->row_stride, plan.table_cols,
-                                           w->tab, L.tab_stride, ix->n_cus, st));
+        HIP_TRY(cosdev::launch_level_table(ix->eng, w->q_codes, w->q_mags, w->qsums, qsums_filled, w->qdig, B, L.tcodes, L.tmags, L.tcsums, ix->row_stride,
+                                           L.tab_phys_cols, w->tab, L.tab_stride, ix->n_cus, st));
         if (timed) HIP_TRY(hipEventRecord(ev[5], st));
     }
     if (timed) HIP_TRY(hipEventRecord(ev[1], st));
@@ -1019,7 +1055,7 @@
         wa.tab_mags = L.tmags;
         wa.tab_stride = L.tab_stride;
         wa.tab_level_min = plan.table_level_min;
-        memcpy(wa.tab_col0, L.tab_col0, sizeof(L.tab_col0));
+        memcpy(wa.tab_adj_col, L.tadj_col, sizeof(L.tadj_col));
     }
     hipStream_t sw = st;
     if (plan.side_stream) {
@@ -1086,6 +1122,7 @@
     }
     if (timed) { HIP_TRY(hipEventRecord(ev[3], sf)); w->ev_count++; }
     w->lastB = B;
+    w->last_table_phys_cols = plan.use_table ? L.tab_phys_cols : 0u;
     w->timed = timed;
     w->last_plan = plan;
     { std::lock_guard<std::mutex> g(ix->mu); ix->last_ws = w; }
@@ -1536,6 +1573,7 @@
     out->queries = w->lastB;
     out->table_level_min = plan.table_level_min;
     out->table_cols = plan.table_cols;
+    out->table_phys_cols = w->last_table_phys_cols;
     out->cut_after_level = plan.cut_after_level;
     if (w->timed && w->ev_count) {
         hipEvent_t *ev = &w->ev[(size_t)((w->ev_count - 1) % Workspace::EV_RING) * Workspace::EV_PER];
@@ -1551,7 +1589,7 @@
         HIP_TRY(hipDeviceSynchronize());
     }
     const u32 kdims = (u32)((ix->row_stride + 63) / 64 * 64);
-    out->table_int8_ops = 2.0 * (double)w->lastB * (double)out->table_cols * (double)kdims;
+    out->table_int8_ops = 2.0 * (double)w->lastB * (double)out->table_phys_cols * (double)kdims;
     u64 st[4], s2[4];
     if ((rc = sum_launch_stats(w->stats, w->lastB, st)) || (rc = sum_launch_stats(w->stats2, w->lastB, s2))) return rc;
     out->lower_evals = s2[0];
diff --git a/cosdata_amd/csrc/engine_internal.h b/cosdata_amd/csrc/engine_internal.h
--- a/cosdata_amd/csrc/engine_internal.h
+++ b/cosdata_amd/csrc/engine_internal.h
@@ -31,7 +31,7 @@
 hipError_t launch_link_round(const LinkArgs &a, u32 maxM, const u32 *pend, const u32 *pcount, u32 *next, u32 *next_count, u32 *evq, u32 *evq_count,
                              u32 count_ub, u32 round, hipStream_t st);
 hipError_t launch_quantize_rows(int eng, const float *x, u64 x_stride, u32 n, u32 dim, float lo, float hi, uint8_t *codes,
-                                u64 row_stride, float *mags, float *raw_mags, hipStream_t st);
+                                u64 row_stride, float *mags, float *raw_mags, hipStream_t st, u32 *qsums = nullptr );
 hipError_t launch_walk(int eng, const IndexDev &ix, const WalkArgs &wa, WalkKernel kernel, hipStream_t st);
 static_assert(WALK_PLAN_MAX_LEVELS == MAX_LEVELS && WALK_PLAN_ENG_U8 == ENG_U8 && WALK_PLAN_ENG_Q2 == ENG_Q2 && WALK_PLAN_FAST_MAX_EF == WALK_FAST_MAX_EF &&
               COS_STORAGE_U8 == 0u && COS_VISITED_REF == 0u, "walk_plan.h restates these");
@@ -53,9 +53,10 @@
 hipError_t launch_walk_order(WalkOrder &o, u32 B, u32 key_max, u32 num_xcd, hipStream_t st);
 hipError_t launch_level_table_gather(const uint8_t *codes, const float *mags, u64 row_stride, const u32 *node_vec, u32 n, u32 col0,
                                      uint8_t *tcodes, float *tmags, hipStream_t st);
+hipError_t launch_level_table_adj_col(const u32 *adj_node, const u32 *node_col, u32 n_nodes, u64 n_slots, u32 *adj_col, hipStream_t st);
 hipError_t launch_code_sums(const uint8_t *codes, u64 row_stride, u32 n, u32 *sums, hipStream_t st);
-hipError_t launch_level_table(int eng, const uint8_t *qcodes, const float *qmags, u32 *qsums, uint8_t *qdig, u32 B, const uint8_t *tcodes, const float *tmags,
-                              const u32 *tcsums, u64 row_stride, u32 ncols, float *tab, u64 tab_stride, u32 n_cus, hipStream_t st);
+hipError_t launch_level_table(int eng, const uint8_t *qcodes, const float *qmags, u32 *qsums, bool qsums_filled, uint8_t *qdig, u32 B, const uint8_t *tcodes,
+                              const float *tmags, const u32 *tcsums, u64 row_stride, u32 ncols, float *tab, u64 tab_stride, u32 n_cus, hipStream_t st);
 bool level_table_eng_supported(int eng, u64 row_stride);
 int32_t quantize_ref_layout(uint32_t storage, uint32_t res, uint32_t dim, const float *x, uint32_t n, void *codes, float *mags);
 int32_t distance_ref_layout(uint32_t metric, uint32_t storage, uint32_t res, uint32_t dim, const void *x_codes, const float *x_mags, uint32_t nx,
@@ -139,6 +140,7 @@
     hipStream_t walk_stream = nullptr;
     hipEvent_t prep_done = nullptr, walk_fin = nullptr;
     u32 lastB = 0;
+    u32 last_table_phys_cols = 0;
     bool timed = false;
     cosdev::WalkPlan last_plan{};
     Workspace() = default;
@@ -227,13 +229,19 @@
     LinkState link;
     bool level_table_valid = false;
     u32 table_level_min = 0, table_cols = 0;
+    u32 table_phys_cols = 0;
     u64 table_built_for_key = 0;
     u64 table_stride = 0;
-    u32 table_col0[cosdev::MAX_LEVELS] = {};
     const uint8_t *d_tcodes = nullptr;
     const float *d_tmags = nullptr;
     const u32 *d_tcsums = nullptr;
-    struct TableSet { u64 key; u32 level_min, cols; u64 stride; u32 col0[cosdev::MAX_LEVELS]; DevArr<uint8_t> tcodes; DevArr<float> tmags; DevArr<u32> tcsums; };
+    const u32 *d_tadj_col[cosdev::MAX_LEVELS] = {};
+    struct TableSet {
+        u64 key; u32 level_min, cols, phys_cols; u64 stride;
+        DevArr<uint8_t> tcodes; DevArr<float> tmags; DevArr<u32> tcsums;
+        DevArr<u32> adj_col[cosdev::MAX_LEVELS];
+    };
+    void view_table_set(const TableSet &t);
     std::vector<TableSet> table_sets;
     u32 walk_side_min_B = 4096;
     u32 lat_max_B = COS_LATENCY_MODE_DEFAULT_MAX_B;
diff --git a/cosdata_amd/csrc/engine_types.h b/cosdata_amd/csrc/engine_types.h
--- a/cosdata_amd/csrc/engine_types.h
+++ b/cosdata_amd/csrc/engine_types.h
@@ -68,7 +68,7 @@
     const float *tab_mags;
     u64 tab_stride;
     u32 tab_level_min;
-    u32 tab_col0[MAX_LEVELS];
+    const u32 *tab_adj_col[MAX_LEVELS];
     u32 no_self_seed;
     u32 smem_mmax;
     u32 smem_win_bytes;
diff --git a/cosdata_amd/csrc/kernels_flat.hip b/cosdata_amd/csrc/kernels_flat.hip
--- a/cosdata_amd/csrc/kernels_flat.hip
+++ b/cosdata_amd/csrc/kernels_flat.hip
@@ -857,9 +857,22 @@
     for (u32 c = lane; c < (u32)(row_stride / 16); c += 64) dst[c] = src[c];
     if (lane == 0) tmags[col0 + node] = mags[row];
 }
+__global__ __launch_bounds__(256) void level_table_adj_col_kernel(const u32 *__restrict__ adj_node, const u32 *__restrict__ node_col, u32 n_nodes, u64 n_slots,
+                                                                  u32 *__restrict__ adj_col) {
+    const u64 i = (u64)blockIdx.x * 256 + threadIdx.x;
+    if (i >= n_slots) return;
+    const u32 v = adj_node[i];
+    adj_col[i] = v < n_nodes ? node_col[v] : ROW_EMPTY;
+}
 }
 
 namespace cosdev {
+
+hipError_t launch_level_table_adj_col(const u32 *adj_node, const u32 *node_col, u32 n_nodes, u64 n_slots, u32 *adj_col, hipStream_t st) {
+    if (n_slots == 0) return hipSuccess;
+    hipLaunchKernelGGL(level_table_adj_col_kernel, dim3((unsigned)((n_slots + 255) / 256)), dim3(256), 0, st, adj_node, node_col, n_nodes, n_slots, adj_col);
+    return hipGetLastError();
+}
 
 hipError_t launch_level_table_gather(const uint8_t *codes, const float *mags, u64 row_stride, const u32 *node_vec, u32 n, u32 col0,
                                      uint8_t *tcodes, float *tmags, hipStream_t st) {
@@ -878,14 +891,14 @@
     return eng == ENG_U8 || (eng == ENG_Q2 && level_table_areg_supported(ENG_Q2, row_stride));
 }
 
-hipError_t launch_level_table(int eng, const uint8_t *qcodes, const float *qmags, u32 *qsums , uint8_t *qdig ,
+hipError_t launch_level_table(int eng, const uint8_t *qcodes, const float *qmags, u32 *qsums , bool qsums_filled, uint8_t *qdig ,
                               u32 B, const uint8_t *tcodes, const float *tmags, const u32 *tcsums, u64 row_stride, u32 ncols, float *tab, u64 tab_stride,
                               u32 n_cus, hipStream_t st) {
     if (B == 0 || ncols == 0) return hipSuccess;
     const bool q2 = eng == ENG_Q2;
     const u32 kdims = q2 ? (u32)(row_stride / 16) * 64 : (u32)((row_stride + 63) / 64 * 64);
     hipError_t e = hipSuccess;
-    if (!q2) e = launch_code_sums(qcodes, row_stride, B, qsums, st);
+    if (!q2 && !qsums_filled) e = launch_code_sums(qcodes, row_stride, B, qsums, st);
     if (e != hipSuccess) return e;
     if (level_table_areg_supported(eng, row_stride) && tune_or(TUNE_WALK_TABLE_GEMM, 1) != 0) {
         if (q2) {
diff --git a/cosdata_amd/csrc/kernels_walk.hip b/cosdata_amd/csrc/kernels_walk.hip
--- a/cosdata_amd/csrc/kernels_walk.hip
+++ b/cosdata_amd/csrc/kernels_walk.hip
@@ -15,7 +15,8 @@
 template <int ENG>
 __global__ __launch_bounds__(256) void quantize_rows_kernel(const float *__restrict__ x, u64 x_stride, u32 n, u32 dim, float lo,
                                                             float hi, uint8_t *__restrict__ codes, u64 row_stride,
-                                                            float *__restrict__ mags, float *__restrict__ raw_mags) {
+                                                            float *__restrict__ mags, float *__restrict__ raw_mags,
+                                                            u32 *__restrict__ qsums ) {
     const int lane = threadIdx.x & 63;
     const u32 row = blockIdx.x * (blockDim.x >> 6) + (threadIdx.x >> 6);
     if (row >= n) return;
@@ -26,7 +27,7 @@
     if (need_seq) rn = seq_norm_wave(xr, dim, lane);
     if (raw_mags && lane == 0) raw_mags[row] = rn;
     if constexpr (ENG == ENG_U8) {
-        u32 ss = 0;
+        u32 ss = 0, sq = 0;
         for (u32 i = lane; i < (u32)row_stride; i += 64) {
             uint8_t q = 0;
             if (i < dim) {
@@ -36,10 +37,16 @@
             }
             cr[i] = q;
             ss += (u32)q * (u32)q;
+            sq += (u32)q;
         }
 #pragma unroll
         for (int m = 32; m > 0; m >>= 1) ss += (u32)__shfl_xor((int)ss, m, 64);
         if (lane == 0) mags[row] = sqrtf((float)ss);
+        if (qsums) {
+#pragma unroll
+            for (int m = 32; m > 0; m >>= 1) sq += (u32)__shfl_xor((int)sq, m, 64);
+            if (lane == 0) qsums[row] = sq;
+        }
     } else if constexpr (ENG == ENG_Q2) {
         const u32 nch = (u32)(row_stride / 16);
         for (u32 c = 0; c < nch; c++) {
@@ -454,16 +461,17 @@
 namespace cosdev {
 
 hipError_t launch_quantize_rows(int eng, const float *x, u64 x_stride, u32 n, u32 dim, float lo, float hi, uint8_t *codes,
-                                u64 row_stride, float *mags, float *raw_mags, hipStream_t st) {
+                                u64 row_stride, float *mags, float *raw_mags, hipStream_t st, u32 *qsums) {
     if (n == 0) return hipSuccess;
+    if (qsums && eng != ENG_U8) return hipErrorInvalidValue;
     dim3 block(256), grid((n + 3) / 4);
     switch (eng) {
-    case ENG_U8: hipLaunchKernelGGL(quantize_rows_kernel<ENG_U8>, grid, block, 0, st, x, x_stride, n, dim, lo, hi, codes, row_stride, mags, raw_mags); break;
-    case ENG_Q2: hipLaunchKernelGGL(quantize_rows_kernel<ENG_Q2>, grid, block, 0, st, x, x_stride, n, dim, lo, hi, codes, row_stride, mags, raw_mags); break;
-    case ENG_F32: hipLaunchKernelGGL(quantize_rows_kernel<ENG_F32>, grid, block, 0, st, x, x_stride, n, dim, lo, hi, codes, row_stride, mags, raw_mags); break;
-    case ENG_F16: hipLaunchKernelGGL(quantize_rows_kernel<ENG_F16>, grid, block, 0, st, x, x_stride, n, dim, lo, hi, codes, row_stride, mags, raw_mags); break;
-    case ENG_Q1: hipLaunchKernelGGL(quantize_rows_kernel<ENG_Q1>, grid, block, 0, st, x, x_stride, n, dim, lo, hi, codes, row_stride, mags, raw_mags); break;
-    case ENG_Q3: hipLaunchKernelGGL(quantize_rows_kernel<ENG_Q3>, grid, block, 0, st, x, x_stride, n, dim, lo, hi, codes, row_stride, mags, raw_mags); break;
+    case ENG_U8: hipLaunchKernelGGL(quantize_rows_kernel<ENG_U8>, grid, block, 0, st, x, x_stride, n, dim, lo, hi, codes, row_stride, mags, raw_mags, qsums); break;
+    case ENG_Q2: hipLaunchKernelGGL(quantize_rows_kernel<ENG_Q2>, grid, block, 0, st, x, x_stride, n, dim, lo, hi, codes, row_stride, mags, raw_mags, qsums); break;
+    case ENG_F32: hipLaunchKernelGGL(quantize_rows_kernel<ENG_F32>, grid, block, 0, st, x, x_stride, n, dim, lo, hi, codes, row_stride, mags, raw_mags, qsums); break;
+    case ENG_F16: hipLaunchKernelGGL(quantize_rows_kernel<ENG_F16>, grid, block, 0, st, x, x_stride, n, dim, lo, hi, codes, row_stride, mags, raw_mags, qsums); break;
+    case ENG_Q1: hipLaunchKernelGGL(quantize_rows_kernel<ENG_Q1>, grid, block, 0, st, x, x_stride, n, dim, lo, hi, codes, row_stride, mags, raw_mags, qsums); break;
+    case ENG_Q3: hipLaunchKernelGGL(quantize_rows_kernel<ENG_Q3>, grid, block, 0, st, x, x_stride, n, dim, lo, hi, codes, row_stride, mags, raw_mags, qsums); break;
     default: return hipErrorInvalidValue;
     }
     return hipGetLastError();
diff --git a/cosdata_amd/csrc/kernels_walk_lat4.hip b/cosdata_amd/csrc/kernels_walk_lat4.hip
--- a/cosdata_amd/csrc/kernels_walk_lat4.hip
+++ b/cosdata_amd/csrc/kernels_walk_lat4.hip
@@ -80,8 +80,9 @@
         const u32 out_slot = L - (u32)level;
         u32 cur = 0;
         const bool tab_level = ENG == ENG_U8 && wa.tab != nullptr && (u32)level >= wa.tab_level_min;
-        const float *tabq = wa.tab + (u64)qi * wa.tab_stride + wa.tab_col0[level];
-        const float *tabm = wa.tab_mags + wa.tab_col0[level];
+        const float *tabq = tab_query_row(wa, qi);
+        const float *tabm = wa.tab_mags;
+        const u32 *adj_col = tab_level ? wa.tab_adj_col[level] : nullptr;
 
         vis_clear<256>(s_vis, M, tid);
         __syncthreads();
@@ -92,7 +93,8 @@
             bool ok;
             if (tab_level) {
                 bool bad;
-                s0 = cosine_or_dot(metric, uniform_f32(tabq[entry]), qmag, uniform_f32(tabm[entry]), bad);
+                const u32 ecol = tab_entry_col(wa, adj_col, lv, level, entry);
+                s0 = cosine_or_dot(metric, uniform_f32(tabq[ecol]), qmag, uniform_f32(tabm[ecol]), bad);
                 ok = !bad;
             } else
                 ok = single_distance(erow, s0);
@@ -116,7 +118,7 @@
             const u64 *pool = s_pool + (size_t)cur * CAP;
             u64 *pool_nx = s_pool + (size_t)(cur ^ 1u) * CAP;
 
-            u32 av[E], an[E], wnode[E];
+            u32 av[E], an[E], ac[E], wnode[E];
             u64 wkey[E];
             const u32 slot_l = (u32)lane < slots ? (u32)lane : slots - 1u;
 #pragma unroll
@@ -129,6 +131,12 @@
             if (level != 0) {
 #pragma unroll
                 for (int i = 0; i < E; i++) an[i] = lv.adj_node[(u64)wnode[i] * M + slot_l];
+            }
+#pragma unroll
+            for (int i = 0; i < E; i++) ac[i] = 0u;
+            if (tab_level) {
+#pragma unroll
+                for (int i = 0; i < E; i++) ac[i] = adj_col[(u64)wnode[i] * M + slot_l];
             }
             const u64 last_key = pool[kwin - 1u];
             bool cnd[E];
@@ -153,7 +161,7 @@
 #pragma unroll
                 for (int i = 0; i < E; i++) {
                     float sim = 0.0f, magv = 1.0f;
-                    if (cnd[i]) { sim = tabq[an[i]]; magv = tabm[an[i]]; }
+                    if (cnd[i]) { sim = tabq[ac[i]]; magv = tabm[ac[i]]; }
                     bool bad;
                     sim = cosine_or_dot(metric, sim, qmag, magv, bad);
                     if (cnd[i]) my_spec[i * 64 + lane] = (u64)metric_key(metric, sim) | (bad ? (1ull << 32) : 0ull);
diff --git a/cosdata_amd/csrc/table_columns.h b/cosdata_amd/csrc/table_columns.h
--- /dev/null
+++ b/cosdata_amd/csrc/table_columns.h
@@ -0,0 +1,62 @@
+#pragma once
+#include <cstdint>
+#include <unordered_map>
+#include <vector>
+
+namespace cosdev {
+
+struct TableLevelIn {
+    uint32_t n;
+    const uint32_t *child;
+    const uint32_t *node_vec;
+};
+
+struct TableColumns {
+    uint32_t phys_cols = 0;
+    uint32_t logical_cols = 0;
+    std::vector<std::vector<uint32_t>> node_col;
+    std::vector<uint32_t> col_row;
+};
+
+inline TableColumns table_columns(const TableLevelIn *lv, uint32_t lmin, uint32_t ltop) {
+    TableColumns t;
+    if (ltop < lmin) return t;
+    auto row_of = [&](uint32_t level, uint32_t x) { return lv[level].node_vec ? lv[level].node_vec[x] : x; };
+    t.node_col.resize(ltop - lmin + 1);
+    const uint32_t n0 = lv[lmin].n;
+    t.node_col[0].resize(n0);
+    t.col_row.resize(n0);
+    for (uint32_t x = 0; x < n0; x++) {
+        t.node_col[0][x] = x;
+        t.col_row[x] = row_of(lmin, x);
+    }
+    t.logical_cols = n0;
+    std::unordered_map<uint32_t, uint32_t> by_row;
+    bool by_row_built = false;
+    for (uint32_t l = lmin + 1; l <= ltop; l++) {
+        const uint32_t n = lv[l].n, nb = lv[l - 1].n;
+        std::vector<uint32_t> &col = t.node_col[l - lmin];
+        const std::vector<uint32_t> &below = t.node_col[l - 1 - lmin];
+        col.resize(n);
+        t.logical_cols += n;
+        for (uint32_t x = 0; x < n; x++) {
+            const uint32_t row = row_of(l, x);
+            const uint32_t c = lv[l].child ? lv[l].child[x] : 0xFFFFFFFFu;
+            if (c < nb && t.col_row[below[c]] == row) {
+                col[x] = below[c];
+                continue;
+            }
+            if (!by_row_built) {
+                for (uint32_t k = 0; k < (uint32_t)t.col_row.size(); k++) by_row.emplace(t.col_row[k], k);
+                by_row_built = true;
+            }
+            const auto ins = by_row.emplace(row, (uint32_t)t.col_row.size());
+            if (ins.second) t.col_row.push_back(row);
+            col[x] = ins.first->second;
+        }
+    }
+    t.phys_cols = (uint32_t)t.col_row.size();
+    return t;
+}
+
+}
diff --git a/cosdata_amd/csrc/walk_common.h b/cosdata_amd/csrc/walk_common.h
--- a/cosdata_amd/csrc/walk_common.h
+++ b/cosdata_amd/csrc/walk_common.h
@@ -32,6 +32,11 @@
         lostmask &= ~g;
     }
     return wmask;
+}
+
+__device__ __forceinline__ const float *tab_query_row(const WalkArgs &wa, u32 qi) { return wa.tab + (u64)qi * wa.tab_stride; }
+__device__ __forceinline__ u32 tab_entry_col(const WalkArgs &wa, const u32 *adj_col, const LevelDev &lv, int level, u32 entry) {
+    return (u32)level == wa.tab_level_min ? entry : uniform_u32(adj_col[(u64)lv.n * lv.M + entry]);
 }
 
 template <bool UNSCALED = false>
diff --git a/cosdata_amd/csrc/walk_kernel.inc b/cosdata_amd/csrc/walk_kernel.inc
--- a/cosdata_amd/csrc/walk_kernel.inc
+++ b/cosdata_amd/csrc/walk_kernel.inc
@@ -113,8 +113,9 @@
         const u32 out_slot = L - (u32)level;
         u32 nlog = 0;
         const bool tab_level = TABLE_OK && wa.tab != nullptr && (u32)level >= wa.tab_level_min;
-        const float *tabq = wa.tab + (u64)qi * wa.tab_stride + wa.tab_col0[level];
-        const float *tabm = wa.tab_mags + wa.tab_col0[level];
+        const float *tabq = tab_query_row(wa, qi);
+        const float *tabm = wa.tab_mags;
+        const u32 *adj_col = tab_level ? wa.tab_adj_col[level] : nullptr;
 
         if (!exact) {
             vis_clear<64>(sm.vis, M, lane);
@@ -131,7 +132,8 @@
             float s0;
             if (tab_level) {
                 bool bad;
-                s0 = cosine_or_dot(metric, uniform_f32(tabq[entry]), qmag, uniform_f32(tabm[entry]), bad);
+                const u32 ecol = tab_entry_col(wa, adj_col, lv, level, entry);
+                s0 = cosine_or_dot(metric, uniform_f32(tabq[ecol]), qmag, uniform_f32(tabm[ecol]), bad);
                 if (bad) { status = COS_ERR_CALCULATION; break; }
             } else if (!single_distance(erow, s0)) { status = COS_ERR_CALCULATION; break; }
             if (lane == 0) {
@@ -159,7 +161,7 @@
             n_rounds++;
             u32 kwin = npool < (u32)LA ? npool : (u32)LA;
             if (kwin > wa.ef - npop) kwin = wa.ef - npop;
-            u32 wv_[LA], wn_[LA];
+            u32 wv_[LA], wn_[LA], wc_[LA];
             {
                 const u32 slot_l = (u32)lane < slots ? (u32)lane : slots - 1u;
                 auto fetch_stage = [&](auto bothc) {
@@ -171,6 +173,7 @@
                         const u64 off = ((u64)nd << log2M) + slot_l;
                         wv_[i] = lv.adj_vec[off];
                         if constexpr (BOTH) wn_[i] = lv.adj_node[off];
+                        if constexpr (TAB) wc_[i] = adj_col[off];
                         if constexpr (!TAB && AMAG) wm_[i] = lv.adj_mag[(u64)nd * lv.mag_stride + slot_l];
                     });
                     if constexpr (!TAB) {
@@ -186,7 +189,7 @@
                 else fetch_stage(std::false_type{});
             }
             u32 stop = 0;
-            auto consume = [&](u32 wi, u32 nb_vec, u32 nb_node, float nb_mag) __attribute__((always_inline)) {
+            auto consume = [&](u32 wi, u32 nb_vec, u32 nb_node, u32 nb_col, float nb_mag) __attribute__((always_inline)) {
                 if constexpr (R == 1) {
                     const u64 hd = pool.head();
                     res_lo = writelane_dyn(res_lo, (u32)hd, (int)npop);
@@ -298,7 +301,7 @@
                 };
                 if constexpr (TAB) {
                     float simv = 0.0f, magv = 1.0f;
-                    if (win) { simv = tabq[nb_node]; magv = tabm[nb_node]; }
+                    if (win) { simv = tabq[nb_col]; magv = tabm[nb_col]; }
                     bool badl;
                     simv = cosine_or_dot<ENG == ENG_U8>(metric_t, simv, qmag, magv, badl);
                     if (wmask & ballot64(badl)) failed = 1;
@@ -433,11 +436,11 @@
             if constexpr (TAB) {
                 static_for<0, LA>([&](auto ic) __attribute__((always_inline)) {
                     constexpr int i = decltype(ic)::value;
-                    if ((u32)i < kwin && !stop) consume((u32)i, wv_[i], wn_[i], 1.0f);
+                    if ((u32)i < kwin && !stop) consume((u32)i, wv_[i], wn_[i], wc_[i], 1.0f);
                 });
             } else {
                 for (u32 wi = 0; wi < kwin && !stop; wi++)
-                    consume(wi, sm.win_vec[wi * 64 + lane], sm.win_node[wi * 64 + lane], AMAG ? sm.win_mag[wi * 64 + lane] : 1.0f);
+                    consume(wi, sm.win_vec[wi * 64 + lane], sm.win_node[wi * 64 + lane], 0u, AMAG ? sm.win_mag[wi * 64 + lane] : 1.0f);
             }
             if (failed) break;
         }
diff --git a/cosdata_amd/index.py b/cosdata_amd/index.py
--- a/cosdata_amd/index.py
+++ b/cosdata_amd/index.py
@@ -275,6 +275,11 @@
         check(_lib.lib().cos_index_walk_table_info(self._h, C.byref(lv), C.byref(cols)))
         return int(lv.value), int(cols.value)
 
+    def walk_table_phys_cols(self) -> int:
+        cols = C.c_uint32()
+        check(_lib.lib().cos_index_walk_table_phys_cols(self._h, C.byref(cols)))
+        return int(cols.value)
+
     def last_walk_split(self, stream: int = 0) -> CosWalkSplit:
         st = CosWalkSplit()
         st.struct_size = C.sizeof(CosWalkSplit)
diff --git a/include/cosdata_hip.h b/include/cosdata_hip.h
--- a/include/cosdata_hip.h
+++ b/include/cosdata_hip.h
@@ -129,13 +129,14 @@
 #define COS_WALK_TABLE_AUTO 0xFFFFFFFFu
 int32_t cos_index_set_walk_table(cos_index *ix, uint32_t max_cols, uint32_t min_queries);
 int32_t cos_index_walk_table_info(cos_index *ix, uint32_t *out_level_min, uint32_t *out_cols);
+int32_t cos_index_walk_table_phys_cols(cos_index *ix, uint32_t *out_phys_cols);
 typedef struct {
     uint32_t struct_size;
     uint32_t queries;
     uint32_t table_level_min;
     uint32_t table_cols;
     uint32_t cut_after_level;
-    uint32_t reserved;
+    uint32_t table_phys_cols;
     float table_ms;
     float upper_ms, sort_ms, lower_ms;
     double table_int8_ops;
```

Result: slower. 996,800 (-1.8%).
